# intellerce/controlanimate

Measured on AMD Instinct MI355X. Metric: frames_per_sec, higher is better.
Workload: dtype fp16

## Files before the change

controlanimate_amd/_capi.py:

```python
from __future__ import annotations

import ctypes as C
import os

_HERE = os.path.dirname(os.path.abspath(__file__))
LIB_PATH = os.environ.get("CA_HIP_LIB") or os.path.join(_HERE, "csrc", "libcontrolanimate_hip.so")

CA_BF16, CA_F16 = 0, 1
CA_F32 = 2
CA_ACT_NONE, CA_ACT_SILU = 0, 1
CA_ACT_RELU = 4
CA_ACT_RELU6 = 5
CA_MLSD_TOPK = 200
ABI_VERSION = 16


class CAHipUnavailable(RuntimeError):
    pass


class CAHipError(RuntimeError):
    pass


class GemmArgs(C.Structure):
    _fields_ = [
        ("a", C.c_void_p), ("a2", C.c_void_p), ("w", C.c_void_p), ("c", C.c_void_p),
        ("bias", C.c_void_p), ("rowbias", C.c_void_p), ("residual", C.c_void_p),
        ("lda", C.c_int64), ("lda2", C.c_int64), ("ldc", C.c_int64), ("ld_res", C.c_int64),
        ("ld_rowbias", C.c_int64),
        ("m", C.c_int32), ("n", C.c_int32), ("k1", C.c_int32), ("k2", C.c_int32),
        ("rows_per_group", C.c_int32),
        ("alpha", C.c_float), ("post_scale", C.c_float),
        ("act", C.c_int32), ("geglu", C.c_int32), ("out_f32", C.c_int32), ("dtype", C.c_int32),
        ("ln_stats", C.c_void_p), ("ln_colsum", C.c_void_p), ("ln_eps", C.c_float),
        ("workspace", C.c_void_p), ("workspace_bytes", C.c_int64),
        ("row_sums_out", C.c_void_p), ("ln_parts", C.c_int32),
        ("w_frag", C.c_void_p),
    ]


class FfArgs(C.Structure):
    _fields_ = [
        ("x", C.c_void_p), ("w1_frag", C.c_void_p), ("bias1", C.c_void_p), ("colsum1", C.c_void_p), ("ln_stats", C.c_void_p),
        ("w2_frag", C.c_void_p), ("bias2", C.c_void_p), ("residual", C.c_void_p), ("y", C.c_void_p),
        ("lda", C.c_int64), ("ldc", C.c_int64), ("ld_res", C.c_int64),
        ("m", C.c_int32), ("c", C.c_int32), ("inner", C.c_int32), ("ln_eps", C.c_float), ("dtype", C.c_int32),
        ("w_out_frag", C.c_void_p), ("bias_out", C.c_void_p), ("residual_out", C.c_void_p), ("ld_res_out", C.c_int64),
    ]


class TattnArgs(C.Structure):
    _fields_ = [
        ("x", C.c_void_p), ("w_frag", C.c_void_p), ("gamma", C.c_void_p), ("bias_pe", C.c_void_p), ("o", C.c_void_p),
        ("lda", C.c_int64), ("ldo", C.c_int64), ("ld_bias_pe", C.c_int64),
        ("batch", C.c_int32), ("frames", C.c_int32), ("tokens", C.c_int32), ("heads", C.c_int32), ("c", C.c_int32),
        ("ln_eps", C.c_float), ("scale", C.c_float), ("dtype", C.c_int32),
        ("w_out_frag", C.c_void_p), ("bias_out", C.c_void_p), ("residual", C.c_void_p), ("ld_res", C.c_int64),
    ]


ATTN_WOUT_FRAG_ELEMS = 102400
TATTN_W_FRAG_ELEMS = 368640


class XattnArgs(C.Structure):
    _fields_ = [
        ("x", C.c_void_p), ("wq_frag", C.c_void_p), ("bias", C.c_void_p), ("kv_frag", C.c_void_p), ("o", C.c_void_p),
        ("lda", C.c_int64), ("ldo", C.c_int64),
        ("m", C.c_int32), ("tokens", C.c_int32), ("frames_per_kv", C.c_int32), ("kv_mod", C.c_int32), ("kv_batches", C.c_int32),
        ("nk", C.c_int32), ("heads", C.c_int32), ("c", C.c_int32),
        ("ln_eps", C.c_float), ("dtype", C.c_int32),
        ("w_out_frag", C.c_void_p), ("bias_out", C.c_void_p), ("residual", C.c_void_p), ("ld_res", C.c_int64),
        ("kv_frag_ip", C.c_void_p), ("nk_ip", C.c_int32), ("ip_scale", C.c_float),
    ]


XATTN_W_FRAG_ELEMS = 122880
XATTN_KV_FRAG_ELEMS = 7680


class ConvArgs(C.Structure):
    _fields_ = [
        ("x", C.c_void_p), ("x2", C.c_void_p), ("w", C.c_void_p), ("y", C.c_void_p),
        ("bias", C.c_void_p), ("rowbias", C.c_void_p), ("residual", C.c_void_p),
        ("ld_res", C.c_int64), ("ld_rowbias", C.c_int64),
        ("images", C.c_int32), ("hin", C.c_int32), ("win", C.c_int32),
        ("cin1", C.c_int32), ("cin2", C.c_int32), ("cout", C.c_int32),
        ("stride", C.c_int32), ("upsample", C.c_int32), ("rows_per_group", C.c_int32),
        ("alpha", C.c_float), ("post_scale", C.c_float),
        ("act", C.c_int32), ("out_f32", C.c_int32), ("dtype", C.c_int32),
        ("workspace", C.c_void_p), ("workspace_bytes", C.c_int64), ("pad_asym", C.c_int32),
        ("w_wino", C.c_void_p), ("x_is_wino_v", C.c_int32),
    ]


class GroupNormArgs(C.Structure):
    _fields_ = [
        ("x", C.c_void_p), ("x2", C.c_void_p), ("y", C.c_void_p),
        ("gamma", C.c_void_p), ("beta", C.c_void_p), ("partials", C.c_void_p),
        ("images", C.c_int32), ("hw", C.c_int32), ("c1", C.c_int32), ("c2", C.c_int32),
        ("groups", C.c_int32), ("frames_per_stat", C.c_int32),
        ("eps", C.c_float), ("act", C.c_int32), ("dtype", C.c_int32),
        ("wino_v", C.c_void_p), ("wino_h", C.c_int32), ("wino_w", C.c_int32),
    ]


class LayerNormArgs(C.Structure):
    _fields_ = [
        ("x", C.c_void_p), ("y", C.c_void_p), ("gamma", C.c_void_p), ("beta", C.c_void_p),
        ("pos", C.c_void_p),
        ("rows", C.c_int64),
        ("c", C.c_int32), ("rows_per_frame", C.c_int32), ("frames", C.c_int32),
        ("eps", C.c_float), ("dtype", C.c_int32), ("stats", C.c_void_p),
    ]


class AttnArgs(C.Structure):
    _fields_ = [
        ("q", C.c_void_p), ("k", C.c_void_p), ("v", C.c_void_p), ("o", C.c_void_p),
        ("q_outer", C.c_int64), ("q_inner", C.c_int64), ("q_row", C.c_int64),
        ("o_outer", C.c_int64), ("o_inner", C.c_int64), ("o_row", C.c_int64),
# ... 51 lines not shown
    "ca_gemm_wants_finished_stats": (C.c_int, [C.POINTER(GemmArgs)]),
    "ca_ln_finish_sums": (C.c_int, [C.c_void_p, C.c_int, C.c_int64, C.c_int, C.c_float, C.c_void_p, C.c_void_p]),
    "ca_gemm_workspace_bytes": (C.c_int64, [C.POINTER(GemmArgs)]),
    "ca_gemm_row_sums_parts": (C.c_int, [C.POINTER(GemmArgs)]),
    "ca_gemm_plan_name": (C.c_int, [C.POINTER(GemmArgs), C.c_char_p, C.c_int32]),
    "ca_conv3x3_plan_name": (C.c_int, [C.POINTER(ConvArgs), C.c_char_p, C.c_int32]),
    "ca_conv3x3": (C.c_int, [C.POINTER(ConvArgs), C.c_void_p]),
    "ca_pack_w_wino": (C.c_int, [C.c_void_p, C.c_int32, C.c_int32, C.c_int32, C.c_void_p, C.c_void_p]),
    "ca_conv3x3_workspace_bytes": (C.c_int64, [C.POINTER(ConvArgs)]),
    "ca_softmax_rows": (C.c_int, [C.c_void_p, C.c_void_p, C.c_int64, C.c_int32, C.c_int64, C.c_int64, C.c_float, C.c_int32, C.c_void_p]),
    "ca_groupnorm_partials_floats": (C.c_int64, [C.c_int32, C.c_int32, C.c_int32, C.c_int32]),
    "ca_groupnorm_stats": (C.c_int, [C.POINTER(GroupNormArgs), C.c_void_p]),
    "ca_groupnorm_apply": (C.c_int, [C.POINTER(GroupNormArgs), C.c_void_p]),
    "ca_groupnorm": (C.c_int, [C.POINTER(GroupNormArgs), C.c_void_p]),
    "ca_groupnorm_wino_supported": (C.c_int, [C.POINTER(GroupNormArgs)]),
    "ca_layernorm": (C.c_int, [C.POINTER(LayerNormArgs), C.c_void_p]),
    "ca_attention": (C.c_int, [C.POINTER(AttnArgs), C.c_void_p]),
    "ca_attention_plan_name": (C.c_int, [C.POINTER(AttnArgs), C.c_char_p, C.c_int32]),
    "ca_add_bcast": (C.c_int, [C.c_void_p, C.c_void_p, C.c_void_p, C.c_int64, C.c_int64, C.c_int32, C.c_void_p]),
    "ca_repeat": (C.c_int, [C.c_void_p, C.c_void_p, C.c_int64, C.c_int32, C.c_void_p]),
    "ca_silu_f32": (C.c_int, [C.c_void_p, C.c_void_p, C.c_int64, C.c_void_p]),
    "ca_timestep_embedding": (C.c_int, [C.c_void_p, C.c_float, C.c_void_p, C.c_int32, C.c_int32, C.c_int32, C.c_void_p]),
    "ca_latents_to_nhwc": (C.c_int, [C.c_void_p, C.c_void_p, C.c_int32, C.c_int32, C.c_int32, C.c_int32, C.c_int32,
                                      C.c_int32, C.c_int32, C.c_float, C.c_int32, C.c_void_p]),
    "ca_nhwc_to_ncfhw_f32": (C.c_int, [C.c_void_p, C.c_void_p, C.c_int32, C.c_int32, C.c_int32, C.c_int32, C.c_int32,
                                        C.c_int32, C.c_int32, C.c_int32, C.c_void_p]),
    "ca_ncfhw_to_nhwc": (C.c_int, [C.c_void_p, C.c_int32, C.POINTER(C.c_int64), C.c_void_p, C.c_int32, C.c_int32,
                                    C.c_int32, C.c_int32, C.c_int32, C.c_int32, C.c_int32, C.c_void_p]),
    "ca_cfg_scheduler_step": (C.c_int, [C.c_void_p, C.c_int32, C.c_int32, C.c_float, C.c_void_p, C.c_void_p,
                                         C.c_void_p, C.c_void_p, C.c_int32, C.c_int32, C.c_int32, C.c_int32,
                                         C.POINTER(C.c_float), C.c_float, C.c_void_p]),
    "ca_lincomb": (C.c_int, [C.c_void_p, C.POINTER(C.c_void_p), C.POINTER(C.c_float), C.c_int32, C.c_int64, C.c_void_p]),
    "ca_conv3x3_narrow": (C.c_int, [C.POINTER(ConvNarrowArgs), C.c_void_p]),
    "ca_conv3x3_narrow_plan_name": (C.c_int, [C.POINTER(ConvNarrowArgs), C.c_char_p, C.c_int32]),
    "ca_rgb8_to_nhwc": (C.c_int, [C.c_void_p, C.c_void_p, C.c_int32, C.c_int32, C.c_int32, C.c_int32, C.c_void_p]),
    "ca_resize_lanczos4_u8": (C.c_int, [C.c_void_p, C.c_void_p, C.c_int32, C.c_int32, C.c_int32, C.c_int32, C.c_int32,
                                         C.c_void_p, C.c_void_p, C.c_void_p, C.c_void_p, C.c_void_p]),
    "ca_color_match_workspace_bytes": (C.c_int64, [C.c_int32, C.c_int64]),
    "ca_hist_u8x3": (C.c_int, [C.c_void_p, C.c_void_p, C.c_int32, C.c_int64, C.c_void_p]),
    "ca_color_moments_f64": (C.c_int, [C.c_void_p, C.c_void_p, C.c_void_p, C.c_void_p, C.c_int32, C.c_int64, C.c_void_p, C.c_int64, C.c_void_p]),
    "ca_color_transform_f64": (C.c_int, [C.c_void_p, C.c_void_p, C.c_void_p, C.c_void_p, C.c_void_p, C.c_void_p, C.c_int32, C.c_int64, C.c_void_p]),
    "ca_sort_f64_segments": (C.c_int, [C.c_void_p, C.c_void_p, C.c_int32, C.c_int64, C.c_void_p, C.c_int64, C.c_void_p]),
    "ca_color_rank_map_f64": (C.c_int, [C.c_void_p, C.c_void_p, C.c_void_p, C.c_void_p, C.c_void_p, C.c_void_p, C.c_int32, C.c_int64,
                                         C.c_void_p, C.c_int64, C.c_void_p]),
    "ca_color_finish_u8": (C.c_int, [C.c_void_p, C.c_void_p, C.c_int32, C.c_int64, C.c_int32, C.c_void_p, C.c_int64, C.c_void_p]),
    "ca_canny_workspace_bytes": (C.c_int64, [C.c_int32, C.c_int32, C.c_int32]),
    "ca_canny_tile_w": (C.c_int32, []),
    "ca_canny_tile_h": (C.c_int32, []),
    "ca_canny_classify": (C.c_int, [C.c_void_p, C.c_int32, C.c_int32, C.c_int32, C.c_int32, C.c_int32, C.c_int32, C.c_void_p, C.c_int64, C.c_void_p]),
    "ca_canny_link": (C.c_int, [C.c_int32, C.c_int32, C.c_int32, C.c_void_p, C.c_int64, C.c_void_p]),
    "ca_canny_link_stage": (C.c_int, [C.c_int32, C.c_int32, C.c_int32, C.c_void_p, C.c_int64, C.c_int32, C.c_void_p]),
    "ca_canny_emit": (C.c_int, [C.c_int32, C.c_int32, C.c_int32, C.c_void_p, C.c_int64, C.c_void_p, C.c_void_p, C.c_int32, C.c_int32, C.c_void_p]),
    "ca_conv_up2_phase_supported": (C.c_int, [C.POINTER(ConvArgs)]),
    "ca_conv_up2_phase": (C.c_int, [C.POINTER(ConvArgs), C.c_void_p]),
    "ca_conv_up2_phase_plan_name": (C.c_int, [C.POINTER(ConvArgs), C.c_char_p, C.c_int32]),
    "ca_perceiver_attn": (C.c_int, [C.POINTER(PerceiverAttnArgs), C.c_void_p]),
    "ca_hed_prep": (C.c_int, [C.c_void_p, C.c_void_p, C.c_void_p, C.c_int32, C.c_int32, C.c_int32, C.c_int32, C.c_void_p]),
    "ca_hed_pool_side": (C.c_int, [C.c_void_p, C.c_void_p, C.c_void_p, C.c_void_p, C.c_void_p, C.c_int32, C.c_int32, C.c_int32, C.c_int32, C.c_int32, C.c_void_p]),
    "ca_hed_fuse": (C.c_int, [C.c_void_p, C.c_void_p, C.c_void_p, C.c_void_p, C.c_void_p, C.c_int32, C.c_int32, C.c_int32, C.c_void_p, C.c_void_p, C.c_int32, C.c_int32, C.c_void_p]),
    "ca_lineart_conv_in": (C.c_int, [C.c_void_p, C.c_void_p, C.c_void_p, C.c_int32, C.c_int32, C.c_int32, C.c_int32, C.c_void_p]),
    "ca_instnorm_partials_floats": (C.c_int64, [C.c_int32, C.c_int32, C.c_int32, C.c_int32]),
    "ca_instnorm_stats": (C.c_int, [C.c_void_p, C.c_void_p, C.c_int32, C.c_int32, C.c_int32, C.c_int32, C.c_int32, C.c_int32, C.c_void_p]),
    "ca_instnorm_apply": (C.c_int, [C.c_void_p, C.c_void_p, C.c_void_p, C.c_void_p, C.c_int32, C.c_int32, C.c_int32, C.c_int32, C.c_int32, C.c_int32, C.c_int32,
                                    C.c_int32, C.c_float, C.c_int32, C.c_void_p]),
    "ca_convt3x3s2_gather": (C.c_int, [C.c_void_p, C.c_void_p, C.c_int32, C.c_int32, C.c_int32, C.c_int32, C.c_int32, C.c_void_p]),
    "ca_lineart_conv_out": (C.c_int, [C.c_void_p, C.c_void_p, C.c_void_p, C.c_void_p, C.c_int32, C.c_int32, C.c_int32, C.c_int32, C.c_void_p]),
    "ca_lineart_finish": (C.c_int, [C.c_void_p, C.c_int32, C.c_int32, C.c_int32, C.c_void_p, C.c_void_p, C.c_int32, C.c_int32, C.c_void_p]),
    "ca_mlsd_prep": (C.c_int, [C.c_void_p, C.c_void_p, C.c_int32, C.c_int32, C.c_int32, C.c_int32, C.c_void_p]),
    "ca_dwconv3x3": (C.c_int, [C.c_void_p, C.c_void_p, C.c_void_p, C.c_void_p, C.c_int32, C.c_int32, C.c_int32, C.c_int32, C.c_int32, C.c_int32, C.c_int32, C.c_void_p]),
    "ca_upsample2x_bilinear_ac": (C.c_int, [C.c_void_p, C.c_void_p, C.c_int32, C.c_int32, C.c_int32, C.c_int32, C.c_int64, C.c_int32, C.c_int32, C.c_void_p]),
    "ca_conv3x3_dil": (C.c_int, [C.c_void_p, C.c_void_p, C.c_void_p, C.c_void_p, C.c_int32, C.c_int32, C.c_int32, C.c_int32, C.c_int32, C.c_int32, C.c_int32, C.c_void_p]),
    "ca_mlsd_decode_workspace_bytes": (C.c_int64, [C.c_int32, C.c_int32, C.c_int32]),
    "ca_mlsd_decode": (C.c_int, [C.c_void_p, C.c_int32, C.c_int32, C.c_int32, C.c_float, C.c_float, C.c_void_p, C.c_int64, C.c_void_p, C.c_void_p, C.c_void_p]),
    "ca_mlsd_draw": (C.c_int, [C.c_void_p, C.c_void_p, C.c_int32, C.c_int32, C.c_int32, C.c_void_p, C.c_void_p, C.c_int32, C.c_int32, C.c_void_p]),
    "ca_softedge_prep": (C.c_int, [C.c_void_p, C.c_void_p, C.c_int32, C.c_int32, C.c_int32, C.c_int32, C.c_void_p]),
    "ca_relu": (C.c_int, [C.c_void_p, C.c_void_p, C.c_int64, C.c_int32, C.c_void_p]),
    "ca_dwconv_k": (C.c_int, [C.c_void_p, C.c_void_p, C.c_void_p, C.c_int32, C.c_int32, C.c_int32, C.c_int32, C.c_int32, C.c_int32, C.c_int32, C.c_void_p]),
    "ca_maxpool2x2": (C.c_int, [C.c_void_p, C.c_void_p, C.c_int32, C.c_int32, C.c_int32, C.c_int32, C.c_int32, C.c_void_p]),
    "ca_pdc_block_supported": (C.c_int, [C.c_int32, C.c_int32]),
    "ca_pdc_block": (C.c_int, [C.c_void_p, C.c_void_p, C.c_void_p, C.c_void_p, C.c_int32, C.c_int32, C.c_int32, C.c_int32, C.c_int32, C.c_int32, C.c_void_p]),
    "ca_cdcm_dil4": (C.c_int, [C.c_void_p, C.c_void_p, C.c_void_p, C.c_int32, C.c_int32, C.c_int32, C.c_int32, C.c_int32, C.c_void_p]),
    "ca_csam_reduce": (C.c_int, [C.c_void_p] * 9 + [C.c_int32] * 5 + [C.c_void_p]),
    "ca_softedge_fuse": (C.c_int, [C.c_void_p] * 5 + [C.c_int32] * 4 + [C.c_void_p] * 3 + [C.c_int32, C.c_int32, C.c_void_p]),
}

_lib = None


def lib() -> C.CDLL:
    global _lib
    if _lib is not None:
        return _lib
    import torch
    if not os.path.exists(LIB_PATH):
        raise CAHipUnavailable(
            f"{LIB_PATH} is missing: the HIP extension is not built. Run "
            "`python -m controlanimate_amd._build` (needs hipcc); there is no CPU fallback.")
    try:
        handle = C.CDLL(LIB_PATH)
    except OSError as e:
        raise CAHipUnavailable(f"cannot load {LIB_PATH}: {e}") from e
    for name, (res, args) in SYMBOLS.items():
        fn = getattr(handle, name)
        fn.restype = res
        fn.argtypes = args
    if handle.ca_abi_version() != ABI_VERSION:
        raise CAHipUnavailable(f"ABI mismatch: library {handle.ca_abi_version()} vs binding {ABI_VERSION}; rebuild")
    _lib = handle
    return handle


def check(rc: int, what: str) -> None:
    if rc != 0:
        msg = lib().ca_last_error()
        raise CAHipError(f"{what} failed with code {rc}: {msg.decode() if msg else ''}")
```

controlanimate_amd/attention.py:

```python
from __future__ import annotations

from typing import Optional

import torch
from torch import nn

from . import kernels as K
from .attention_processor import Attention, AttnProcessor2_0
from .context import ExecCtx, dispatch
from .layers import HipConv1x1, HipGroupNorm, HipLayerNorm, HipLinear, LnFold, WeightArena, _f32, geglu_interleave, ln_fold_enabled


class GEGLU(nn.Module):
    def __init__(self, dim_in: int, dim_out: int):
        super().__init__()
        self.dim_in, self.dim_out = dim_in, dim_out
        self.proj = HipLinear(dim_in, dim_out * 2)
        self.w = self.b = None

    def pack(self, arena: WeightArena, dtype):
        self.w = arena.add((2 * self.dim_out, self.dim_in), dtype, lambda: geglu_interleave(_f32(self.proj.weight)))
        self.b = arena.add((2 * self.dim_out,), torch.float32, lambda: geglu_interleave(_f32(self.proj.bias)))

    def run(self, x: torch.Tensor) -> torch.Tensor:
        return K.gemm(x, self.w.t, bias=self.b.t, geglu=True)


class FeedForward(nn.Module):
    def __init__(self, dim: int, dim_out: Optional[int] = None, mult: int = 4, dropout: float = 0.0,
                 activation_fn: str = "geglu", final_dropout: bool = False):
        super().__init__()
        if activation_fn != "geglu":
            raise NotImplementedError(activation_fn)
        inner = int(dim * mult)
        self.net = nn.ModuleList([GEGLU(dim, inner), nn.Identity(), HipLinear(inner, dim_out or dim)])

    def pack(self, arena, dtype, fold_ln=None):
        self.fold = None
        if fold_ln is not None and ln_fold_enabled():
            self.fold = LnFold(arena, dtype, fold_ln, [self.net[0].proj], geglu=True)
        else:
            self.net[0].pack(arena, dtype)
        self.net[2].pack(arena, dtype)
        self.w2f = None
        out = self.net[2]
        if self.fold is not None and self.fold.w.frag is not None and (out.out_features, out.in_features) == (320, 1280):
            from .layers import frag_order2
            self.w2f = arena.add((320, 1280), dtype, lambda: frag_order2(out.weight.detach().float()))

    def run_with_proj_out(self, x: torch.Tensor, residual: Optional[torch.Tensor], proj_frag, proj_bias, proj_residual) -> Optional[torch.Tensor]:
        fold = getattr(self, "fold", None)
        if fold is None or getattr(self, "w2f", None) is None or proj_frag is None or not dispatch.attn_out_fused:
            return None
        return K.ff_fused(x, fold.w.frag[0].t, fold.b.t, fold.cs.t, self.w2f.t, None if self.net[2].b is None else self.net[2].b.t,
                          fold.eps, residual=residual, w_out_frag=proj_frag.t, bias_out=None if proj_bias is None else proj_bias.t,
                          residual_out=proj_residual)

    def run(self, x: torch.Tensor, residual: Optional[torch.Tensor] = None, sums=None) -> torch.Tensor:
        fold = getattr(self, "fold", None)
        if fold is not None and getattr(self, "w2f", None) is not None and sums is None:
            y = K.ff_fused(x, fold.w.frag[0].t, fold.b.t, fold.cs.t, self.w2f.t, None if self.net[2].b is None else self.net[2].b.t,
                           fold.eps, residual=residual)
            if y is not None:
                return y
        if fold is not None:
            h = K.gemm(x, fold.w.t, bias=fold.b.t, geglu=True, ln=(K.RowStats(x, fold.eps, sums), fold.cs.t))
        else:
            h = self.net[0].run(x)
        return self.net[2].run(h, residual=residual)


class BasicTransformerBlock(nn.Module):
    def __init__(self, query_dim: int, num_attention_heads: int, attention_head_dim: int, dropout=0.0,
                 cross_attention_dim: Optional[int] = None, activation_fn: str = "geglu", attention_bias: bool = False,
                 upcast_attention: bool = False, unet_use_cross_frame_attention=False, unet_use_temporal_attention=False, **_):
        super().__init__()
        if unet_use_cross_frame_attention or unet_use_temporal_attention:
            raise NotImplementedError("both flags are false in configs/inference/inference-v{1,2}.yaml")
        self.processor = AttnProcessor2_0()
        self.attn1 = Attention(query_dim, heads=num_attention_heads, dim_head=attention_head_dim, bias=attention_bias)
        self.norm1 = HipLayerNorm(query_dim)
        self.attn2 = Attention(query_dim, cross_attention_dim=cross_attention_dim, heads=num_attention_heads,
                               dim_head=attention_head_dim, bias=attention_bias) if cross_attention_dim is not None else None
        self.norm2 = HipLayerNorm(query_dim) if cross_attention_dim is not None else None
        self.ff = FeedForward(query_dim, activation_fn=activation_fn)
        self.norm3 = HipLayerNorm(query_dim)

    def get_processor(self, return_deprecated_lora: bool = False):
        return self.processor

    def set_processor(self, processor, _remove_lora: bool = False):
        if isinstance(getattr(self, "processor", None), nn.Module) and not isinstance(processor, nn.Module):
            self._modules.pop("processor", None)
        self.processor = processor

    def pack(self, arena, dtype):
        self.attn1.pack(arena, dtype, fold_ln=self.norm1)
        self.norm1.pack(arena, dtype)
        if self.attn2 is not None:
            self.attn2.pack(arena, dtype, fold_ln=self.norm2)
            self.norm2.pack(arena, dtype)
        self.ff.pack(arena, dtype, fold_ln=self.norm3)
        self.norm3.pack(arena, dtype)

    def forward(self, x: torch.Tensor, ctx: ExecCtx, proj_out=None) -> torch.Tensor:
        return self.forward_rest(self.forward_self(x), ctx, proj_out=proj_out)

    def forward_self(self, x: torch.Tensor) -> torch.Tensor:
        B, N, C = x.shape
        next_folded = (self.attn2.fold if self.attn2 is not None else self.ff.fold) is not None
        if self.attn1.fold is not None:
            x = self.attn1(x, residual=x, ln=(K.RowStats(x.view(B * N, C), self.norm1.eps, K.row_sums_of(x)), self.attn1.fold),
                           row_sums=next_folded)
        else:
            x = self.attn1(self.norm1.run(x.view(B * N, C)).view(B, N, C), residual=x, row_sums=next_folded)
        return x

    def forward_rest(self, x: torch.Tensor, ctx: ExecCtx, proj_out=None) -> torch.Tensor:
        B, N, C = x.shape
        if self.attn2 is not None:
            kw = dict(encoder_hidden_states=ctx.ehs, residual=x, frames_per_kv=ctx.frames_per_kv, kv_mod=ctx.kv_mod, cache=ctx.cache,
                      row_sums=self.ff.fold is not None)
            if self.attn2.fold is not None:
                x = self.attn2(x, ln=(K.RowStats(x.view(B * N, C), self.norm2.eps, K.row_sums_of(x)), self.attn2.fold), **kw)
            else:
                x = self.attn2(self.norm2.run(x.view(B * N, C)).view(B, N, C), **kw)
        x2 = x.view(B * N, C)
        if self.ff.fold is None:
            return self.ff.run(self.norm3.run(x2), residual=x2).view(B, N, C)
        if proj_out is not None and K.row_sums_of(x) is None:
            y = self.ff.run_with_proj_out(x2, x2, *proj_out)
            if y is not None:
                y = y.view(B, N, C)
                y._proj_out_done = True
                return y
        return self.ff.run(x2, residual=x2, sums=K.row_sums_of(x)).view(B, N, C)


class Transformer3DModel(nn.Module):
    def __init__(self, num_attention_heads: int = 16, attention_head_dim: int = 88, in_channels: Optional[int] = None,
                 num_layers: int = 1, norm_num_groups: int = 32, cross_attention_dim: Optional[int] = None,
                 use_linear_projection: bool = False, **kw):
        super().__init__()
        if use_linear_projection:
            raise NotImplementedError("SD1.5 uses 1x1-conv projections")
        inner = num_attention_heads * attention_head_dim
        self.in_channels = in_channels
        self.norm = HipGroupNorm(norm_num_groups, in_channels, eps=1e-6)
        self.proj_in = HipConv1x1(in_channels, inner)
        self.transformer_blocks = nn.ModuleList([
            BasicTransformerBlock(inner, num_attention_heads, attention_head_dim, cross_attention_dim=cross_attention_dim, **kw)
            for _ in range(num_layers)])
        self.proj_out = HipConv1x1(inner, in_channels)

    def pack(self, arena, dtype):
        self.norm.pack(arena, dtype)
        self.proj_in.pack(arena, dtype)
        for b in self.transformer_blocks:
            b.pack(arena, dtype)
        self.proj_out.pack(arena, dtype)
        self.proj_out_frag = None
        po = self.proj_out
        if tuple(po.weight.shape[:2]) == (320, 320) and getattr(self.transformer_blocks[-1].ff, "w2f", None) is not None:
            from .layers import frag_order_wout
            self.proj_out_frag = arena.add((102400,), dtype, lambda: frag_order_wout(_f32(po.weight).reshape(320, 320)))

    def forward(self, x: torch.Tensor, ctx: ExecCtx, shared_half: bool = False) -> torch.Tensor:
        images, h, w, c = x.shape
        rows = images * h * w
        y = self.norm.run(x)
        y0 = self.proj_in.run(y.view(rows, c), row_sums=self.transformer_blocks[0].attn1.fold is not None)
        y = K.carry_row_sums(y0.view(images, h * w, -1), y0)
        nblk = len(self.transformer_blocks)
        pfrag = getattr(self, "proj_out_frag", None)

        def proj(k, x_rows):
            return (pfrag, self.proj_out.b, x_rows) if (k == nblk - 1 and pfrag is not None) else None
        if shared_half:
            y = self.transformer_blocks[0].forward_self(y)
            y, x = K.repeat_batch(y), K.repeat_batch(x)
            images, rows = 2 * images, 2 * rows
            y = self.transformer_blocks[0].forward_rest(y, ctx, proj_out=proj(0, x.view(rows, c)))
        for k in range(1 if shared_half else 0, nblk):
            y = self.transformer_blocks[k](y, ctx, proj_out=proj(k, x.view(rows, c)))
        if getattr(y, "_proj_out_done", False):
            return y.view(images, h, w, c)
        return self.proj_out.run(y.view(rows, -1), residual=x.view(rows, c)).view(images, h, w, c)
```

controlanimate_amd/context.py:

```python
from __future__ import annotations

from dataclasses import dataclass, field
from typing import Optional

import torch


@dataclass
class ExecCtx:
    b: int
    f: int
    dtype: torch.dtype
    temb: torch.Tensor
    emb_groups: int
    ehs: Optional[torch.Tensor] = None
    frames_per_kv: int = 1
    kv_mod: int = 0
    gn_frames_per_stat: int = 1
    cache: dict = field(default_factory=dict)

    @property
    def images(self) -> int:
        return self.b * self.f

    def rows_per_emb_group(self, h: int, w: int) -> int:
        return self.images // self.emb_groups * h * w


class Dispatch:
    gemm_ar = True
    ff_fused = True
    tattn_fused = True
    xattn_fused = True
    attn_out_fused = True
    xattn_ip_fused = True
    conv_winograd = True
    gn_winograd = True
    conv_up2_phase = True
    ln_row_sums = True
    repeat_kernel = True
    ln_fold = True
    cfg_shared = True
    cn_cfg_dedup = True
    pdc_block_fused = True
    controlnet_streams = 2


dispatch = Dispatch()
```

controlanimate_amd/csrc/ca_gemm.hip:

```cpp

#include "ca_gemm_plan.h"

namespace {
using namespace ca_gemm_detail;
#include "ca_conv_wino.h"

template <int DT, int BM, int BN, int WAVES_M, int WAVES_N, int MODE>
__global__ __launch_bounds__(256) void k_gemm(GemmKParams p) {
  constexpr int TM = BM / WAVES_M / 16;
  constexpr int TN = BN / WAVES_N / 16;
  constexpr int AI = BM / 32;
  constexpr int BI = BN / 32;
  static_assert(2 * (BM + BN) * BK >= BM * (BN + 8), "epilogue staging must fit");
  __shared__ __attribute__((aligned(16))) u16 smem[2 * (BM + BN) * BK];

  const int tid = threadIdx.x;
  const int lane = tid & 63;
  const int wid = tid >> 6;
  const int wm = wid / WAVES_N, wn = wid % WAVES_N;
  const int g = lane >> 4, l15 = lane & 15;

  const int tiles_n = (p.n + BN - 1) / BN;
  const unsigned bid = xcd_remap(blockIdx.x, gridDim.x);
  int tile_m, tile_n;
// ... 329 lines not shown
  if (p.bias) {
#pragma unroll
    for (int k = 0; k < 8; ++k) v[k] += p.bias[n + k];
  }
  if (p.rowbias) {
    const float* rbp = p.rowbias + (m / p.rows_per_group) * p.ld_rowbias + n;
#pragma unroll
    for (int k = 0; k < 8; ++k) v[k] += rbp[k];
  }
#pragma unroll
  for (int k = 0; k < 8; ++k) v[k] *= p.alpha;
  unpack8<DT>(pack8<DT>(v), v);
  if (p.res) {
    float r[8];
    unpack8<DT>(ld16(p.res + m * p.ld_res + n), r);
#pragma unroll
    for (int k = 0; k < 8; ++k) v[k] += r[k];
  }
#pragma unroll
  for (int k = 0; k < 8; ++k) v[k] *= p.post;
  if (p.act != CA_ACT_NONE) {
#pragma unroll
    for (int k = 0; k < 8; ++k) v[k] = act_f(v[k], p.act);
  }
  const int64_t off = m * p.ldc + n;
  if (p.out_f32) {
    float* cp = reinterpret_cast<float*>(p.c) + off;
    *reinterpret_cast<f32x4*>(cp) = (f32x4){v[0], v[1], v[2], v[3]};
    *reinterpret_cast<f32x4*>(cp + 4) = (f32x4){v[4], v[5], v[6], v[7]};
  } else {
    st16(reinterpret_cast<u16*>(p.c) + off, pack8<DT>(v));
  }
}

template <int DT, int MODE>
int launch_gemm(const GemmKParams& p, const GemmPlan& g, hipStream_t st) {
  const dim3 grid(ceil_div_i(p.m, g.bm) * ceil_div_i(p.n, g.bn));
  switch (g.kind) {
    case PK_WRES: return ca_launch_gemm_pp(p, DT, MODE, PK_WRES, 0u, st);
    case PK_AR: return ca_launch_gemm_ar(p, DT, st);
    case PK_PP2:
    case PK_PS:
    case PK_PQ: return ca_launch_gemm_pp(p, DT, MODE, g.kind, g.tiles, st);
    case PK_PP2_SPLITK: {
      GemmKParams q = p;
      q.splits = g.splits;
      const int rc = ca_launch_gemm_pp(q, DT, MODE, PK_PP2, g.tiles * (unsigned)g.splits, st);
      hipLaunchKernelGGL((k_splitk_reduce<DT>), dim3(ceil_div_i((int64_t)q.m * (q.n / 8), 256)), dim3(256), 0, st, q);
      return rc;
    }
    case PK_DMA_SPLITK:
      hipLaunchKernelGGL((k_gemm_dma<DT, 128, 128, 2, 2, MODE, 1>), dim3(g.tiles * (unsigned)p.splits), dim3(256), 0, st, p);
      hipLaunchKernelGGL((k_splitk_reduce<DT>), dim3(ceil_div_i((int64_t)p.m * (p.n / 8), 256)), dim3(256), 0, st, p);
      return CA_OK;
    case PK_DMA:
      if (g.bn == 160 && g.nbuf == 1) hipLaunchKernelGGL((k_gemm_dma<DT, 128, 160, 2, 2, MODE, 1>), grid, dim3(256), 0, st, p);
      else if (g.bn == 128 && g.nbuf == 1) hipLaunchKernelGGL((k_gemm_dma<DT, 128, 128, 2, 2, MODE, 1>), grid, dim3(256), 0, st, p);
      else if (g.bn == 64 && g.nbuf == 1) hipLaunchKernelGGL((k_gemm_dma<DT, 128, 64, 4, 1, MODE, 1>), grid, dim3(256), 0, st, p);
      else if (g.bn == 64 && g.nbuf == 3) hipLaunchKernelGGL((k_gemm_dma<DT, 128, 64, 4, 1, MODE, 3>), grid, dim3(256), 0, st, p);
      else break;
      return CA_OK;
    case PK_REG:
      if (g.bn == 128) hipLaunchKernelGGL((k_gemm<DT, 128, 128, 2, 2, MODE>), grid, dim3(256), 0, st, p);
      else if (g.bn == 64) hipLaunchKernelGGL((k_gemm<DT, 128, 64, 4, 1, MODE>), grid, dim3(256), 0, st, p);
      else break;
      return CA_OK;
  }
  CA_FAIL(CA_ERR_LAUNCH, "ca_gemm: no kernel for plan kind %d, tile %dx%d, %d stages", (int)g.kind, g.bm, g.bn, g.nbuf);
}

}

extern "C" int ca_gemm(const ca_gemm_args* a, void* stream) {
  DenseLaunch d;
  int rc = gemm_prepare(a, d);
  if (rc) return rc;
  hipStream_t st = (hipStream_t)stream;
  rc = a->dtype == CA_BF16 ? launch_gemm<CA_BF16, 0>(d.p, d.plan, st) : launch_gemm<CA_F16, 0>(d.p, d.plan, st);
  if (rc) return rc;
  CA_CHECK_LAUNCH("ca_gemm");
  return CA_OK;
}

extern "C" int64_t ca_gemm_workspace_bytes(const ca_gemm_args* a) {
  DenseLaunch d;
  return gemm_resolve(a, d) == CA_OK ? d.workspace : 0;
}

extern "C" int ca_gemm_row_sums_parts(const ca_gemm_args* a) {
  DenseLaunch d;
  DenseAsk ask{};
  ask.without_row_sums = true;
  return gemm_resolve(a, d, ask) == CA_OK ? row_sums_parts_of(d.p) : 0;
}

extern "C" int ca_gemm_ln_inline_supported(const ca_gemm_args* a) {
  DenseLaunch d;
  return a && a->ln_colsum && gemm_resolve(a, d) == CA_OK && wres_eligible(d.p) ? 1 : 0;
}

extern "C" int ca_gemm_wants_finished_stats(const ca_gemm_args* a) {
  if (!a || !a->ln_colsum || !a->ln_stats || a->ln_parts <= 0 || a->row_sums_out) return 0;
  DenseLaunch d;
  DenseAsk ask{};
  ask.stats_finished = true;
  return gemm_resolve(a, d, ask) == CA_OK && d.plan.kind == PK_PQ ? 1 : 0;
}

extern "C" int64_t ca_conv3x3_workspace_bytes(const ca_conv_args* a) { return conv_workspace_bytes(a); }

static int launch_conv_wino(const ca_conv_args* a, const GemmKParams& cp, hipStream_t st) {
  const int kc = a->cin1 + a->cin2;
  const ConvGeom g = conv_geom(a);
  const int64_t tiles = wino_tiles(a, g);
  WinoParams w{};
  w.x = (const u16*)a->x;
  w.x2 = (const u16*)a->x2;
  w.v = (u16*)a->workspace;
  u16* mm = (u16*)a->workspace + (a->x_is_wino_v ? 0 : 16 * tiles * kc);
  w.mm = mm;
  w.y = (u16*)a->y;
  w.bias = a->bias;
  w.rowbias = a->rowbias;
  w.res = (const u16*)a->residual;
  w.ld_res = a->ld_res;
  w.ld_rowbias = a->ld_rowbias;
  w.images = a->images, w.h = g.hl, w.w = g.wl, w.c1 = a->cin1, w.c2 = a->cin2, w.cout = a->cout;
  w.ups = a->upsample;
  w.rows_per_group = cp.rows_per_group;
  w.alpha = a->alpha, w.post = a->post_scale, w.act = a->act;
  const int64_t in_threads = tiles * (kc / 8), out_threads = tiles * (a->cout / 8);
  if (a->x_is_wino_v) w.v = (u16*)a->x;
  else if (a->dtype == CA_BF16) hipLaunchKernelGGL((k_wino_in<CA_BF16>), dim3((unsigned)((in_threads + 255) / 256)), dim3(256), 0, st, w);
  else hipLaunchKernelGGL((k_wino_in<CA_F16>), dim3((unsigned)((in_threads + 255) / 256)), dim3(256), 0, st, w);
  GemmKParams q{};
  q.a = w.v;
  q.w = (const u16*)a->w_wino;
  q.c = mm;
  q.lda = kc;
  q.ldc = a->cout;
  q.a_bytes = desc_bytes(16 * tiles * kc);
  q.w_bytes = desc_bytes((int64_t)16 * a->cout * kc);
  q.m = (int)(16 * tiles);
  q.n = a->cout;
  q.c1 = kc;
  q.taps = 1;
  q.kc_tiles = kc / BK;
  q.rows_per_group = 1;
  q.alpha = 1.f, q.post = 1.f;
  q.splits = 1;
  q.w_group_rows = (int)tiles;
  q.w_group_stride = (unsigned)((int64_t)a->cout * kc * 2);
  const unsigned gemm_tiles = (unsigned)((q.m / 256) * (q.n / 320));
  int rc = ca_launch_gemm_pp(q, a->dtype, 0, PK_PQ, gemm_tiles, st);
  if (rc) return rc;
  if (a->dtype == CA_BF16) hipLaunchKernelGGL((k_wino_out<CA_BF16>), dim3((unsigned)((out_threads + 255) / 256)), dim3(256), 0, st, w);
  else hipLaunchKernelGGL((k_wino_out<CA_F16>), dim3((unsigned)((out_threads + 255) / 256)), dim3(256), 0, st, w);
  return CA_OK;
}

extern "C" int ca_pack_w_wino(const void* w, int32_t cout, int32_t cin, int32_t dtype, void* dst, void* stream) {
  CA_REQUIRE(w && dst, "ca_pack_w_wino: null operand");
  CA_REQUIRE(cout > 0 && cin > 0 && (dtype == CA_BF16 || dtype == CA_F16), "ca_pack_w_wino: cout=%d cin=%d dtype=%d", cout, cin, dtype);
  const int64_t n = (int64_t)cout * cin;
  if (dtype == CA_BF16) hipLaunchKernelGGL((k_pack_w_wino<CA_BF16>), dim3((unsigned)((n + 255) / 256)), dim3(256), 0, (hipStream_t)stream, (const u16*)w, (u16*)dst, cout, cin);
  else hipLaunchKernelGGL((k_pack_w_wino<CA_F16>), dim3((unsigned)((n + 255) / 256)), dim3(256), 0, (hipStream_t)stream, (const u16*)w, (u16*)dst, cout, cin);
  CA_CHECK_LAUNCH("ca_pack_w_wino");
  return CA_OK;
}

extern "C" int ca_conv3x3(const ca_conv_args* a, void* stream) {
  GemmKParams p{};
  int rc = conv_prepare(a, p);
  if (rc) return rc;
  hipStream_t st = (hipStream_t)stream;
  if (wino_taken(a)) {
    rc = launch_conv_wino(a, p, st);
    if (rc) return rc;
    CA_CHECK_LAUNCH("ca_conv3x3(winograd)");
    return CA_OK;
  }
// ... 54 lines not shown
```

controlanimate_amd/csrc/ca_gemm_core.h:

```cpp
#pragma once
#include "ca_common.h"
#include <stdlib.h>

namespace ca_gemm_detail {


struct GemmKParams {
  const u16* a;
  const u16* a2;
  const u16* w;
  void* c;
  const float* bias;
  const float* rowbias;
  const float* ln_stats;
  const float* ln_colsum;
  const u16* res;
  int64_t lda, lda2, ldc, ld_res, ld_rowbias;
  unsigned a_bytes, a2_bytes, w_bytes;
  int m, n;
  int c1, c2;
  int taps;
  int kc_tiles;
  int hin, win, hout, wout, stride, ups, pad_lo;
  int rows_per_group;
  float alpha, post;
  int act, geglu, out_f32;
  int splits;
  float* partial;
  int dbg;
  int tap_inner;
  float* row_sums;
  int ln_parts;
  int ln_inline;
  float ln_eps;
  const u16* wf;
  int w_group_rows;
  unsigned w_group_stride;
  int up2_rows, up2_tiles;
  unsigned up2_mag_w, up2_mag_h;
};

constexpr int BK = 64;

constexpr int GROUP_M = 8;
__device__ __forceinline__ void tile_coords(unsigned bid, int tiles_m, int tiles_n, int& tile_m, int& tile_n) {
  const unsigned gsz = GROUP_M * tiles_n;
  const unsigned group = bid / gsz, in = bid - group * gsz;
  const int first_m = group * GROUP_M;
  const int gm = tiles_m - first_m < GROUP_M ? tiles_m - first_m : GROUP_M;
  tile_m = first_m + in % gm;
  tile_n = in / gm;
}

__device__ __forceinline__ void k_tile_split(const GemmKParams& p, int t, int kct, int& tap, int& cc) {
  if (p.taps == 1) {
    tap = 0;
    cc = t;
  } else if (p.tap_inner) {
    cc = t / p.taps;
    tap = t - cc * p.taps;
  } else {
    tap = t / kct;
    cc = t - tap * kct;
  }
}

__device__ __forceinline__ int lds_off(int row, int chunk) {
  return row * BK + ((chunk ^ ((row >> 1) & 7)) << 3);
}

template <int DT, int TM, int TN>
__device__ __forceinline__ void gemm_epilogue_direct(const GemmKParams& p, f32x4 (&acc)[TM][TN], int m0, int n0, int wm, int wn,
                                                     int l15, int g) {
#pragma unroll
  for (int i = 0; i < TM; ++i) {
    const int m = m0 + wm * TM * 16 + i * 16 + l15;
    if (m >= p.m) continue;
    const float* rbp = p.rowbias ? p.rowbias + (int64_t)(m / p.rows_per_group) * p.ld_rowbias : nullptr;
#pragma unroll
    for (int j = 0; j < TN; ++j) {
      const int n = n0 + wn * TN * 16 + j * 16 + g * 4;
      if (n >= p.n) continue;
      float v[4];
#pragma unroll
      for (int r = 0; r < 4; ++r) v[r] = acc[i][j][r];
      if (p.bias) {
        f32x4 b = *reinterpret_cast<const f32x4*>(p.bias + n);
#pragma unroll
        for (int r = 0; r < 4; ++r) v[r] += b[r];
      }
      if (rbp) {
        f32x4 b = *reinterpret_cast<const f32x4*>(rbp + n);
#pragma unroll
        for (int r = 0; r < 4; ++r) v[r] += b[r];
      }
#pragma unroll
      for (int r = 0; r < 4; ++r) v[r] *= p.alpha;
      if (p.res) {
        u32x2 rr = *reinterpret_cast<const u32x2*>(p.res + (int64_t)m * p.ld_res + n);
        v[0] += Elem<DT>::to_f((u16)(rr[0] & 0xffffu));
        v[1] += Elem<DT>::to_f((u16)(rr[0] >> 16));
        v[2] += Elem<DT>::to_f((u16)(rr[1] & 0xffffu));
        v[3] += Elem<DT>::to_f((u16)(rr[1] >> 16));
      }
#pragma unroll
      for (int r = 0; r < 4; ++r) v[r] *= p.post;
      if (p.act != CA_ACT_NONE) {
#pragma unroll
        for (int r = 0; r < 4; ++r) v[r] = act_f(v[r], p.act);
      }
      if (p.geglu) {
        const f32x2 gg = gelu_erf_f2((f32x2){v[1], v[3]});
        float o0 = v[0] * gg[0];
        float o1 = v[2] * gg[1];
        const int64_t off = (int64_t)m * p.ldc + (n >> 1);
        if (p.out_f32) {
          float* cp = reinterpret_cast<float*>(p.c) + off;
          cp[0] = o0;
          cp[1] = o1;
        } else {
          *reinterpret_cast<unsigned*>(reinterpret_cast<u16*>(p.c) + off) = pack2<DT>(o0, o1);
        }
// ... 256 lines not shown
```

controlanimate_amd/csrc/ca_gemm_plan.h:

```cpp
#pragma once
#include "ca_gemm_core.h"

namespace ca_gemm_detail {

inline unsigned desc_bytes(int64_t elems) {
  const int64_t b = elems * 2;
  return (b > 0 && b < (int64_t)0xFFFFFF00ll) ? (unsigned)b : 0u;
}

inline bool dma_shape_ok(const GemmKParams& p) { return (p.c1 + p.c2) % BK == 0 && (p.c2 == 0 || p.c1 % BK == 0); }
inline bool dma_sizes_ok(const GemmKParams& p) { return p.a_bytes != 0 && p.w_bytes != 0 && (p.c2 == 0 || p.a2_bytes != 0); }
inline bool dma_capable(const GemmKParams& p) { return dma_shape_ok(p) && dma_sizes_ok(p); }

inline bool wres_eligible(const GemmKParams& p) {
  static const int wres_env = CA_KNOB("CA_GEMM_WRES", -1);
  const int kc = p.c1 + p.c2;
  return wres_env != 0 && kc == 320 && p.taps == 1 && (p.c2 == 0 || p.c1 % 32 == 0) && p.n % 160 == 0 && p.n / 160 <= 32 && !p.out_f32 &&
         p.splits <= 1 && !p.ln_parts && dma_sizes_ok(p) &&
         (!p.rowbias || p.rows_per_group % 32 == 0) &&
         act_out_fit31(p) &&
         (wres_env == 1 || p.m >= 16384);
}

inline bool ar_eligible(const GemmKParams& p, bool scratch) {
// ... 62 lines not shown
      if (s_eff > p.splits) s_eff = p.splits;
      if (s_eff >= 2 && tiles320 * s_eff >= 128 && nt / s_eff >= 12) {
        return GemmPlan{PK_PP2_SPLITK, 128, 320, 0, s_eff, (unsigned)tiles320};
      }
    }
    return GemmPlan{PK_DMA_SPLITK, 128, 128, 1, p.splits, (unsigned)(ceil_div_i(p.m, 128) * (p.n / 128))};
  }
  static const int pp_env = CA_KNOB("CA_GEMM_PP", -1);
  static const int pq_env = CA_KNOB("CA_GEMM_PQ", -1);
  if (pq_env != 0 && pq_capable(p, mode)) {
    const int64_t tiles = (int64_t)ceil_div_i(p.m, 256) * (p.n / 320);
    const bool dflt = mode == 1 ? (tiles >= 256 && (p.n >= 640 || nt >= 64)) : (tiles >= 256 && (tiles % 256 == 0 || tiles >= 1024) && nt >= 8 && !wres_eligible(p));
    const bool epi1 = p.geglu || p.ln_colsum || p.ln_stats;
    const bool dflt2 = dflt && (mode == 1 || p.geglu), dflt3 = dflt && mode == 1, dflt4 = dflt && (mode == 1 || p.geglu || !epi1);
    if ((pq_env < 0 && dflt) || pq_env == 1 || (pq_env == 2 && dflt2) || (pq_env == 3 && dflt3) || (pq_env == 4 && dflt4) || (pq_env == 5 && dflt)) {
      return GemmPlan{PK_PQ, 256, 320, 0, 1, (unsigned)tiles};
    }
  }
  static const int ps_env = CA_KNOB("CA_GEMM_PS", -1);
  if (ps_env != 0 && ps_capable(p)) {
    const int64_t tiles = (int64_t)ceil_div_i(p.m, 128) * (p.n / 320);
    const bool dflt = mode == 0 && !wres_eligible(p) && nt <= 20 && tiles >= 256 && (p.geglu || p.n <= 1280);
    if ((ps_env < 0 && dflt) || ps_env == 1 || (ps_env == 2 && !(mode == 0 && wres_eligible(p)))) {
      return GemmPlan{PK_PS, 128, 320, 0, 1, (unsigned)tiles};
    }
  }
  if (mode == 0 && dma && ar_eligible(p, p.partial != nullptr)) return GemmPlan{PK_AR, 128, 64, 0, 1, 0u};
  if (mode == 0 && dma && wres_eligible(p)) return GemmPlan{PK_WRES, 256, 160, 0, 1, 0u};
  if (dma && pp_env != 0 && nt >= 2 && p.n % 320 == 0 && p.splits <= 1) {
    const int64_t tiles = (int64_t)ceil_div_i(p.m, 128) * (p.n / 320);
    if (p.row_sums || pp_env == 2 || (pp_env < 0 && tiles >= 128 && nt >= 10 && (tiles <= 256 || (tiles <= 512 && mode == 0)))) {
      return GemmPlan{PK_PP2, 128, 320, 0, 1, (unsigned)tiles};
    }
  }
  const bool wide = p.n % 128 == 0 && (int64_t)ceil_div_i(p.m, 128) * ceil_div_i(p.n, 128) >= 512;
  const int64_t blocks = (int64_t)ceil_div_i(p.m, 128) * ceil_div_i(p.n, wide ? 128 : 64);
  const int nbuf = blocks >= 512 ? 1 : 3;
  if (dma && !wide && p.n % 160 == 0 && (int64_t)ceil_div_i(p.m, 128) * (p.n / 160) >= 512) return GemmPlan{PK_DMA, 128, 160, 1, 1, 0u};
  return GemmPlan{dma ? PK_DMA : PK_REG, 128, wide ? 128 : 64, dma ? nbuf : 2, 1, 0u};
}

inline int row_sums_parts_of(GemmKParams p) {
  p.row_sums = nullptr;
  if (p.geglu || p.out_f32) return 0;
  const PlanKind k = plan_gemm(p, 0).kind;
  if (k == PK_PP2 || k == PK_PS) return p.n / 320;
  if (k == PK_PQ && !p.ln_colsum && !p.ln_stats) return 4 * (p.n / 320);
  return 0;
}
inline bool row_sums_capable(const GemmKParams& p) { return row_sums_parts_of(p) > 0; }

inline void plan_label(const GemmPlan& g, char* buf, int len) {
  switch (g.kind) {
    case PK_WRES: snprintf(buf, len, "wres160"); break;
    case PK_AR: snprintf(buf, len, "ar128x64"); break;
    case PK_PP2: snprintf(buf, len, "pp128x320"); break;
    case PK_PS: snprintf(buf, len, "ps128x320"); break;
    case PK_PQ: snprintf(buf, len, "pq256x320"); break;
    case PK_PP2_SPLITK: snprintf(buf, len, "pp128x320_splitk%d", g.splits); break;
    case PK_DMA: snprintf(buf, len, "%dx%d%s", g.bm, g.bn, g.nbuf == 3 ? "_r3" : ""); break;
    case PK_DMA_SPLITK: snprintf(buf, len, "128x128_splitk%d", g.splits); break;
    case PK_REG: snprintf(buf, len, "reg_%dx%d", g.bm, g.bn); break;
  }
}

inline int check_epilogue(const char* who, int n, int geglu, int64_t ldc, int64_t ld_res, const void* res) {
  CA_REQUIRE(n == 4 || (n >= 8 && n % 8 == 0), "%s: N=%d must be 4 or a multiple of 8", who, n);
  CA_REQUIRE(!geglu || n % 8 == 0, "%s: geglu needs N %% 8 == 0", who);
  if (n >= 8) {
    CA_REQUIRE(ldc % (geglu ? 4 : 8) == 0, "%s: ldc=%lld must be a multiple of %d", who, (long long)ldc, geglu ? 4 : 8);
    CA_REQUIRE(!res || ld_res % 8 == 0, "%s: ld_res=%lld must be a multiple of 8", who, (long long)ld_res);
  } else {
    CA_REQUIRE(ldc % 4 == 0, "%s: ldc=%lld misaligned", who, (long long)ldc);
    CA_REQUIRE(!res || ld_res % 4 == 0, "%s: ld_res=%lld misaligned", who, (long long)ld_res);
  }
  return CA_OK;
}

struct DenseAsk {
  bool without_row_sums;
  bool stats_finished;
};

inline int gemm_fill(const ca_gemm_args* a, GemmKParams& p, const DenseAsk& ask) {
  CA_REQUIRE(a != nullptr, "ca_gemm: null args");
  CA_REQUIRE(a->a && a->w && a->c, "ca_gemm: null operand");
  CA_REQUIRE(a->m > 0 && a->k1 > 0 && a->k2 >= 0, "ca_gemm: bad sizes m=%d k1=%d k2=%d", a->m, a->k1, a->k2);
  CA_REQUIRE(a->k1 % 8 == 0 && a->k2 % 8 == 0, "ca_gemm: k1=%d k2=%d must be multiples of 8", a->k1, a->k2);
  CA_REQUIRE(a->lda % 8 == 0 && (a->k2 == 0 || (a->a2 && a->lda2 % 8 == 0)), "ca_gemm: lda/lda2 misaligned or a2 missing");
  CA_REQUIRE(a->dtype == CA_BF16 || a->dtype == CA_F16, "ca_gemm: dtype %d", a->dtype);
  CA_REQUIRE(!a->rowbias || a->rows_per_group > 0, "ca_gemm: rows_per_group");
  CA_REQUIRE(!a->rowbias || a->ld_rowbias % 4 == 0, "ca_gemm: ld_rowbias misaligned");
  int rc = check_epilogue("ca_gemm", a->n, a->geglu, a->ldc, a->ld_res, a->residual);
  if (rc) return rc;
  p.a = (const u16*)a->a, p.a2 = (const u16*)a->a2, p.w = (const u16*)a->w, p.c = a->c;
  p.bias = a->bias, p.rowbias = a->rowbias, p.ln_stats = a->ln_stats, p.ln_colsum = a->ln_colsum;
  p.row_sums = ask.without_row_sums ? nullptr : a->row_sums_out;
  p.ln_parts = ask.stats_finished ? 0 : a->ln_parts;
  CA_REQUIRE(p.ln_parts >= 0 && p.ln_parts <= 16, "ca_gemm: ln_parts=%d", p.ln_parts);
  CA_REQUIRE(p.ln_parts == 0 || (a->ln_stats && a->ln_colsum && a->ln_eps > 0.f), "ca_gemm: ln_parts needs ln_stats (the partial sums), ln_colsum and ln_eps > 0");
  p.ln_inline = (a->ln_colsum && !a->ln_stats) ? 1 : 0;
  p.ln_eps = a->ln_eps;
  p.wf = (const u16*)a->w_frag;
  CA_REQUIRE(!a->ln_stats || a->ln_colsum, "ca_gemm: ln_stats without ln_colsum");
  CA_REQUIRE(!p.ln_inline || a->ln_eps > 0.f, "ca_gemm: ln_colsum without ln_stats asks for in-kernel statistics and needs ln_eps > 0");
  CA_REQUIRE(!a->ln_colsum || (a->n >= 8 && a->k2 == 0), "ca_gemm: the folded LayerNorm needs N >= 8 and a single A source");
  p.res = (const u16*)a->residual;
  p.lda = a->lda, p.lda2 = a->lda2, p.ldc = a->ldc, p.ld_res = a->ld_res, p.ld_rowbias = a->ld_rowbias;
  p.a_bytes = desc_bytes((int64_t)(a->m - 1) * a->lda + a->k1);
  p.a2_bytes = a->k2 ? desc_bytes((int64_t)(a->m - 1) * a->lda2 + a->k2) : 0u;
  p.w_bytes = desc_bytes((int64_t)a->n * (a->k1 + a->k2));
  p.m = a->m, p.n = a->n, p.c1 = a->k1, p.c2 = a->k2;
  p.taps = 1;
  p.kc_tiles = ceil_div_i(a->k1 + a->k2, BK);
  p.rows_per_group = a->rows_per_group > 0 ? a->rows_per_group : 1;
  p.alpha = a->alpha, p.post = a->post_scale, p.act = a->act, p.geglu = a->geglu, p.out_f32 = a->out_f32;
  p.splits = 1;
  return CA_OK;
}

struct DenseLaunch {
  GemmKParams p;
  GemmPlan plan;
  int64_t workspace;
};
inline int gemm_resolve(const ca_gemm_args* a, DenseLaunch& d, const DenseAsk& ask = DenseAsk{}) {
  d = DenseLaunch{};
  GemmKParams& p = d.p;
  int rc = gemm_fill(a, p, ask);
  if (rc) return rc;
  const SplitK k = splitk_decide(p, 0);
  splitk_apply(k, a->workspace, a->workspace_bytes, p);
  d.workspace = k.bytes;
  if (p.ln_inline && p.wf) {
    if (ar_eligible(p, true)) d.workspace = (int64_t)p.m * 8;
    if (a->workspace && a->workspace_bytes >= (int64_t)p.m * 8) p.partial = reinterpret_cast<float*>(a->workspace);
  }
  d.plan = plan_gemm(p, 0);
  return CA_OK;
}

inline int gemm_prepare(const ca_gemm_args* a, DenseLaunch& d) {
  int rc = gemm_resolve(a, d);
  if (rc) return rc;
  CA_REQUIRE(!d.p.row_sums || row_sums_capable(d.p), "ca_gemm: row_sums_out is not available for this launch: ask ca_gemm_row_sums_parts() first");
  CA_REQUIRE(!d.p.ln_inline || wres_eligible(d.p), "ca_gemm: in-kernel LayerNorm statistics (ln_stats NULL) are not available for this launch: "
             "ask ca_gemm_ln_inline_supported() first and pass ln_stats otherwise");
  return CA_OK;
}

struct ConvGeom { int hl, wl, hout, wout; int64_t m; };
inline ConvGeom conv_geom(const ca_conv_args* a) {
  ConvGeom g;
  g.hl = a->hin << a->upsample, g.wl = a->win << a->upsample;
  const int pad = a->pad_asym ? 1 : 2;
  g.hout = (g.hl + pad - 3) / a->stride + 1;
  g.wout = (g.wl + pad - 3) / a->stride + 1;
  g.m = (int64_t)a->images * g.hout * g.wout;
  return g;
}
inline int64_t wino_tiles(const ca_conv_args* a, const ConvGeom& g) { return (int64_t)a->images * (g.hl / 2) * (g.wl / 2); }

inline int64_t wino_workspace_bytes(const ca_conv_args* a) {
  if (!a || !a->w_wino || (a->dtype != CA_F16 && a->dtype != CA_BF16) || a->stride != 1 || a->pad_asym || a->out_f32) return 0;
  if (a->upsample != 0 && a->upsample != 1) return 0;
  if (a->x_is_wino_v && (a->cin2 != 0 || a->upsample)) return 0;
  const ConvGeom g = conv_geom(a);
  if (a->images <= 0 || g.hl < 2 || g.wl < 2 || (g.hl & 1) || (g.wl & 1)) return 0;
  const int kc = a->cin1 + a->cin2;
  static const int min_cin = CA_KNOB("CA_WINO_MIN_CIN", 1280);
  if (kc < 640 || kc % BK != 0 || a->cin1 % 8 != 0 || a->cin2 % 8 != 0 || a->cout % 320 != 0) return 0;
  const int64_t tiles = wino_tiles(a, g);
  if (kc < min_cin && !(min_cin == 1280 && tiles <= 4096)) return 0;
  static const int max_tiles = CA_KNOB("CA_WINO_MAX_TILES", 16384);
  if (tiles % 256 != 0 || tiles > max_tiles) return 0;
  if (16 * tiles * (int64_t)(kc > a->cout ? kc : a->cout) * 2 >= 0x7FFFFF00ll) return 0;
  return 16 * tiles * (int64_t)((a->x_is_wino_v ? 0 : kc) + a->cout) * 2;
}

inline bool wino_taken(const ca_conv_args* a) {
  const int64_t wb = wino_workspace_bytes(a);
  return wb > 0 && a->workspace && a->workspace_bytes >= wb && (((uintptr_t)a->workspace | (uintptr_t)a->w_wino) & 15) == 0;
}

inline void conv_fill_sizes(const ca_conv_args* a, const ConvGeom& g, GemmKParams& p) {
  p.a_bytes = desc_bytes((int64_t)a->images * a->hin * a->win * a->cin1);
  p.a2_bytes = a->cin2 ? desc_bytes((int64_t)a->images * a->hin * a->win * a->cin2) : 0u;
  p.w_bytes = desc_bytes((int64_t)a->cout * 9 * (a->cin1 + a->cin2));
  p.m = (int)g.m, p.n = a->cout, p.c1 = a->cin1, p.c2 = a->cin2;
  p.taps = 9;
  static const int tap_inner_env = CA_KNOB("CA_CONV_TAP_INNER", 1);
  p.tap_inner = tap_inner_env;
  p.kc_tiles = ceil_div_i(a->cin1 + a->cin2, BK);
  p.hin = a->hin, p.win = a->win, p.hout = g.hout, p.wout = g.wout;
  p.stride = a->stride, p.ups = a->upsample, p.pad_lo = a->pad_asym ? 0 : 1;
  p.geglu = 0, p.out_f32 = a->out_f32;
  p.splits = 1;
}

inline int conv_prepare(const ca_conv_args* a, GemmKParams& p) {
  CA_REQUIRE(a != nullptr, "ca_conv3x3: null args");
  CA_REQUIRE(a->x && a->w && a->y, "ca_conv3x3: null operand");
  CA_REQUIRE(a->images > 0 && a->hin > 0 && a->win > 0, "ca_conv3x3: bad geometry");
  CA_REQUIRE(a->cin1 > 0 && a->cin1 % 8 == 0 && a->cin2 >= 0 && a->cin2 % 8 == 0,
             "ca_conv3x3: cin1=%d cin2=%d must be multiples of 8", a->cin1, a->cin2);
  CA_REQUIRE(a->cin2 == 0 || a->x2, "ca_conv3x3: x2 missing");
  CA_REQUIRE(a->stride == 1 || a->stride == 2, "ca_conv3x3: stride %d", a->stride);
  CA_REQUIRE(a->upsample == 0 || a->upsample == 1, "ca_conv3x3: upsample %d", a->upsample);
  CA_REQUIRE(a->dtype == CA_BF16 || a->dtype == CA_F16, "ca_conv3x3: dtype %d", a->dtype);
  CA_REQUIRE(!a->rowbias || a->rows_per_group > 0, "ca_conv3x3: rows_per_group");
  int rc = check_epilogue("ca_conv3x3", a->cout, 0, a->cout, a->ld_res, a->residual);
  if (rc) return rc;
  CA_REQUIRE(a->pad_asym == 0 || a->pad_asym == 1, "ca_conv3x3: pad_asym %d", a->pad_asym);
  const ConvGeom g = conv_geom(a);
  CA_REQUIRE(g.m < (1ll << 31), "ca_conv3x3: too many output pixels");
  conv_fill_sizes(a, g, p);
  p.a = (const u16*)a->x, p.a2 = (const u16*)a->x2, p.w = (const u16*)a->w, p.c = a->y;
  p.bias = a->bias, p.rowbias = a->rowbias, p.res = (const u16*)a->residual;
  p.ldc = a->cout, p.ld_res = a->ld_res, p.ld_rowbias = a->ld_rowbias;
  p.rows_per_group = a->rows_per_group > 0 ? a->rows_per_group : 1;
  p.alpha = a->alpha, p.post = a->post_scale, p.act = a->act;
  splitk_apply(splitk_decide(p, 1), a->workspace, a->workspace_bytes, p);
  return CA_OK;
}

inline int64_t conv_workspace_bytes(const ca_conv_args* a) {
  if (!a || a->images <= 0 || a->hin <= 0 || a->win <= 0 || (a->stride != 1 && a->stride != 2)) return 0;
  const int64_t wb = wino_workspace_bytes(a);
  if (wb > 0) return wb;
  const ConvGeom g = conv_geom(a);
// ... 51 lines not shown
```

controlanimate_amd/csrc/ca_gemm_pp.hip:

```cpp
#include "ca_gemm_core.h"
#include <type_traits>

namespace {
using namespace ca_gemm_detail;
#include "ca_gemm_pp2.h"
#include "ca_gemm_wres.h"
#include "ca_gemm_ps.h"
#include "ca_gemm_pq.h"

int cu_count() {
  static int n = 0;
  if (!n) {
    int dev = 0;
    hipDeviceProp_t prop;
    if (hipGetDevice(&dev) == hipSuccess && hipGetDeviceProperties(&prop, dev) == hipSuccess) n = prop.multiProcessorCount;
    if (n <= 0) n = 256;
  }
  return n;
}

template <class Launch>
int launch_stamped(const GemmKParams& p, hipStream_t st, const char* label, unsigned sep, unsigned eol, Launch launch) {
  static unsigned long long* dbuf = nullptr;
  if (!dbuf && hipMalloc(&dbuf, 4096 * 8) != hipSuccess) return CA_ERR_LAUNCH;
  (void)hipMemsetAsync(dbuf, 0, 4096 * 8, st);
  GemmKParams q = p;
  q.partial = reinterpret_cast<float*>(dbuf);
  launch(q);
  (void)hipStreamSynchronize(st);
  static int printed = 0;
  if (printed++ < 1) {
    static unsigned long long host[4096];
    (void)hipMemcpy(host, dbuf, sizeof(host), hipMemcpyDeviceToHost);
    for (int g = 0; g < 2; ++g) {
      fprintf(stderr, "[%s stamps group %d, %dx%dx%d] tag:delta_cycles ...\n", label, g, p.m, p.n, (p.c1 + p.c2) * p.taps);
      unsigned long long prev = host[g * 2048];
      for (int i = 0; i < 1000 && host[g * 2048 + 2 * i]; ++i) {
        fprintf(stderr, "%llu:%llu ", host[g * 2048 + 2 * i + 1], host[g * 2048 + 2 * i] - prev);
        prev = host[g * 2048 + 2 * i];
        if (host[g * 2048 + 2 * i + 1] == sep) fprintf(stderr, "| ");
        if (host[g * 2048 + 2 * i + 1] == eol) fprintf(stderr, "\n");
      }
      fprintf(stderr, "\n");
    }
  }
  return CA_OK;
}

template <int DT, int MODE>
int launch_pp(const GemmKParams& p, PlanKind kind, unsigned tiles, hipStream_t st) {
  const unsigned c_bytes = (unsigned)c_extent_bytes(p), res_bytes = (unsigned)res_extent_bytes(p);
  const unsigned grid = tiles < (unsigned)cu_count() ? tiles : (unsigned)cu_count();
  switch (kind) {
    case PK_PQ: {
      auto launch = [&](const GemmKParams& q) {
        if (MODE == 0 && (q.geglu || q.ln_colsum || q.ln_stats)) hipLaunchKernelGGL((k_gemm_pq<DT, 0, 1>), dim3(grid), dim3(512), 0, st, q, (int)tiles, c_bytes, 0u);
        else if (MODE == 0 && q.row_sums) hipLaunchKernelGGL((k_gemm_pq<DT, 0, 2>), dim3(grid), dim3(512), 0, st, q, (int)tiles, c_bytes, res_bytes);
        else hipLaunchKernelGGL((k_gemm_pq<DT, MODE>), dim3(grid), dim3(512), 0, st, q, (int)tiles, c_bytes, res_bytes);
      };
#ifdef CA_STAMPS
      if (p.dbg == 9) return launch_stamped(p, st, "pq", 8, 10, launch);
#endif
      launch(p);
      return CA_OK;
    }
    case PK_PS: {
      auto launch = [&](const GemmKParams& q) { hipLaunchKernelGGL((k_gemm_ps<DT, MODE>), dim3(grid), dim3(512), 0, st, q, (int)tiles, c_bytes, res_bytes); };
#ifdef CA_STAMPS
      if (p.dbg == 9) return launch_stamped(p, st, "ps", 8, 10, launch);
#endif
      launch(p);
      return CA_OK;
    }
    case PK_WRES: {
      if (MODE != 0) return CA_ERR_LAUNCH;
      const int panels = p.n / 160;
      const int chunks = (p.m + 255) / 256;
      int per = (cu_count() / 8) / panels;
      if (per * 8 > chunks) per = chunks / 8;
      if (per < 1) per = 1;
      const unsigned rb_bytes = p.rowbias ? (unsigned)(((int64_t)((p.m - 1) / p.rows_per_group) * p.ld_rowbias + p.n) * 4) : 16u;
      hipLaunchKernelGGL((k_gemm_wres<DT>), dim3(8 * per * panels), dim3(512), 0, st, p, panels, 8 * per, chunks, rb_bytes, c_bytes, res_bytes);
      return CA_OK;
    }
    case PK_PP2:
      hipLaunchKernelGGL((k_gemm_pp2<DT, MODE>), dim3(tiles), dim3(512), 0, st, p);
      return CA_OK;
    default: return CA_ERR_LAUNCH;
  }
}

template <int DT>
int launch_up2(const GemmKParams& p, PlanKind kind, unsigned tiles, hipStream_t st) {
  if (kind != PK_PQ) return CA_ERR_LAUNCH;
  const unsigned grid = tiles < (unsigned)cu_count() ? tiles : (unsigned)cu_count();
  hipLaunchKernelGGL((k_gemm_pq<DT, 2>), dim3(grid), dim3(512), 0, st, p, (int)tiles, (unsigned)c_extent_bytes(p), (unsigned)res_extent_bytes(p));
  return CA_OK;
}
}

int ca_launch_gemm_pp(const ca_gemm_detail::GemmKParams& p0, int dtype, int mode, ca_gemm_detail::PlanKind kind, unsigned tiles, hipStream_t st) {
  static const int dbg = CA_KNOB("CA_PP_DBG", 0);
  ca_gemm_detail::GemmKParams p = p0;
  p.dbg = dbg;
  if (mode == 2) return dtype == CA_BF16 ? launch_up2<CA_BF16>(p, kind, tiles, st) : launch_up2<CA_F16>(p, kind, tiles, st);
  if (dtype == CA_BF16) return mode ? launch_pp<CA_BF16, 1>(p, kind, tiles, st) : launch_pp<CA_BF16, 0>(p, kind, tiles, st);
  return mode ? launch_pp<CA_F16, 1>(p, kind, tiles, st) : launch_pp<CA_F16, 0>(p, kind, tiles, st);
}
```

controlanimate_amd/csrc/ca_gemm_wres.h:

```cpp
#include "ca_gemm_seq.h"

__device__ __forceinline__ int ca_wres_col(int j, int i, bool geglu) {
  if (geglu) return 16 * j + i;
  return 32 * (j >> 1) + 8 * (i >> 2) + 4 * (j & 1) + (i & 3);
}

template <int DT>
__global__ __launch_bounds__(512, 1) void k_gemm_wres(GemmKParams p, int panels, int lanes, int chunks, unsigned rb_bytes, unsigned c_bytes, unsigned res_bytes) {
  constexpr int K = 320, PN = 160, TN = 10, KQ = 10;
  constexpr int WLD_B = 656;
  constexpr int W_BYTES = PN * WLD_B;
  constexpr int SLOT = 2048, RING = 3 * SLOT;
  constexpr int OFF_PAR = W_BYTES + 8 * RING;
  constexpr int OFF_RB = OFF_PAR + 1280;
  constexpr int OFF_FLAG = OFF_RB + 8 * 1024;
  __shared__ __attribute__((aligned(16))) unsigned char smem[OFF_FLAG + 8 * 16];
  static_assert(OFF_FLAG + 8 * 16 <= 160 * 1024, "LDS");

  const int tid = threadIdx.x;
  const int lane = tid & 63;
  const int wid = __builtin_amdgcn_readfirstlane(tid >> 6);
  const int g = lane >> 4, l15 = lane & 15;

  const int slot_b = blockIdx.x >> 3;
  const int panel = slot_b % panels;
  const int my_lane = (blockIdx.x & 7) + 8 * (slot_b / panels);
  if (my_lane >= lanes) return;
  const int n0 = panel * PN;

  const bool geglu = p.geglu != 0;
  for (int q = tid; q < PN * (K / 8); q += 512) {
    const int row = q / (K / 8), c = q - row * (K / 8);
    *reinterpret_cast<u32x4*>(smem + row * WLD_B + c * 16) = ld16(p.w + (int64_t)(n0 + ca_wres_col(row >> 4, row & 15, geglu)) * K + c * 8);
  }
  if (tid < 2 * PN) {
    const float* src = tid < PN ? p.bias : p.ln_colsum;
    const int n = tid < PN ? tid : tid - PN;
    reinterpret_cast<float*>(smem + OFF_PAR)[tid] = src ? src[n0 + n] : 0.f;
  }
  __syncthreads();

  const __amdgpu_buffer_rsrc_t rs_rb = __builtin_amdgcn_make_buffer_rsrc((void*)(p.rowbias ? (const void*)p.rowbias : (const void*)p.w), 0, rb_bytes, 0x00020000);
  unsigned char* rb_patch = smem + OFF_RB + wid * 1024;
  const __amdgpu_buffer_rsrc_t rs_c = __builtin_amdgcn_make_buffer_rsrc(p.c, 0, c_bytes, 0x00020000);
  const __amdgpu_buffer_rsrc_t rs_res = __builtin_amdgcn_make_buffer_rsrc((void*)(p.res ? (const void*)p.res : (const void*)p.c), 0, p.res ? res_bytes : 0u, 0x00020000);
  const __amdgpu_buffer_rsrc_t rs_a = __builtin_amdgcn_make_buffer_rsrc((void*)p.a, 0, p.a_bytes, 0x00020000);
  const __amdgpu_buffer_rsrc_t rs_a2 = __builtin_amdgcn_make_buffer_rsrc((void*)(p.a2 ? p.a2 : p.a), 0, p.a2 ? p.a2_bytes : p.a_bytes, 0x00020000);
  unsigned char* ring = smem + W_BYTES + wid * RING;
  const __amdgpu_buffer_rsrc_t rs_seq = __builtin_amdgcn_make_buffer_rsrc((void*)ca_seq_table.v, 0, 4096u, 0x00020000);
  unsigned char* const my_flags = smem + OFF_FLAG + wid * 16;
  const unsigned flag_addr0 = (unsigned)(size_t)(__attribute__((address_space(3))) unsigned char*)my_flags;
  if (lane < 4) {
    asm volatile("ds_write_b32 %0, %1\n\ts_waitcnt lgkmcnt(0)" ::"v"(flag_addr0 + (unsigned)lane * 4u), "v"(0xFFFFFFFFu) : "memory");
  }

  int d_c = my_lane, d_k = 0, d_s = 0;
  int d_n = 0;
  unsigned d_v1[2], d_v2[2];
  auto head_slab = [&]() {
    int lane_o = lane;
    asm volatile("" : "+v"(lane_o));
#pragma unroll
    for (int h = 0; h < 2; ++h) {
      const int m = d_c * 256 + wid * 32 + h * 16 + (lane_o >> 2);
      const bool ok = m < p.m;
      d_v1[h] = ok ? (unsigned)m * (unsigned)p.lda * 2u + (unsigned)(lane_o & 3) * 16u : DMA_OOB;
      d_v2[h] = ok ? (unsigned)m * (unsigned)p.lda2 * 2u + (unsigned)(lane_o & 3) * 16u : DMA_OOB;
    }
  };
  auto issue = [&]() {
    const int k0 = d_k * 32;
    unsigned char* dst = ring + d_s * SLOT;
    if (k0 >= p.c1) {
      const unsigned so = (unsigned)(k0 - p.c1) * 2u;
      __builtin_amdgcn_raw_ptr_buffer_load_lds(rs_a2, (__attribute__((address_space(3))) void*)dst, 16, d_v2[0], so, 0, 0);
      __builtin_amdgcn_raw_ptr_buffer_load_lds(rs_a2, (__attribute__((address_space(3))) void*)(dst + 1024), 16, d_v2[1], so, 0, 0);
    } else {
      const unsigned so = (unsigned)k0 * 2u;
      __builtin_amdgcn_raw_ptr_buffer_load_lds(rs_a, (__attribute__((address_space(3))) void*)dst, 16, d_v1[0], so, 0, 0);
      __builtin_amdgcn_raw_ptr_buffer_load_lds(rs_a, (__attribute__((address_space(3))) void*)(dst + 1024), 16, d_v1[1], so, 0, 0);
    }
    {
      int lane_f = lane;
      asm volatile("" : "+v"(lane_f));
      if (lane_f == 0)
        __builtin_amdgcn_raw_ptr_buffer_load_lds(rs_seq, (__attribute__((address_space(3))) void*)(my_flags + d_s * 4), 4, 0u, (unsigned)(d_n & 1023) * 4u, 0, 0);
    }
    ++d_n;
    d_s = d_s == 2 ? 0 : d_s + 1;
    if (++d_k == KQ) {
      d_k = 0;
      d_c += lanes;
      head_slab();
    }
  };

  auto chunk_wait = [&](int n, unsigned have) __attribute__((always_inline)) {
    const unsigned want = (unsigned)(n & 1023);
    if ((unsigned)__builtin_amdgcn_readfirstlane(have) == want) return;
    const unsigned addr = flag_addr0 + (unsigned)(n % 3) * 4u;
    for (unsigned spins = 0; spins < (1u << 22); ++spins) {
      unsigned v;
      asm volatile("ds_read_b32 %0, %1\n\ts_waitcnt lgkmcnt(0)" : "=v"(v) : "v"(addr) : "memory");
      if ((unsigned)__builtin_amdgcn_readfirstlane(v) == want) return;
      __builtin_amdgcn_s_sleep(1);
    }
    asm volatile("s_waitcnt vmcnt(0)" ::: "memory");
  };
  int r_n = 0;

  head_slab();
  issue();
  issue();
  chunk_wait(0, 0xFFFFFFFEu);

  const int fa_lane = l15 * 64 + g * 16;
  const unsigned char* wb = smem + l15 * WLD_B + g * 16;
  int r_s = 0;

  for (int c = my_lane; c < chunks; c += lanes) {
    const int m0 = c * 256 + wid * 32;
    f32x4 acc[2][TN];
#pragma unroll
    for (int i = 0; i < 2; ++i)
#pragma unroll
      for (int j = 0; j < TN; ++j) acc[i][j] = (f32x4){0.f, 0.f, 0.f, 0.f};

    float2 st[2] = {make_float2(0.f, 0.f), make_float2(0.f, 0.f)};
    float ln_s[2] = {0.f, 0.f}, ln_ss[2] = {0.f, 0.f};
    if (p.ln_stats) {
#pragma unroll
      for (int i = 0; i < 2; ++i) {
        const int m = m0 + i * 16 + l15;
        if (m < p.m) st[i] = *reinterpret_cast<const float2*>(p.ln_stats + (int64_t)m * 2);
      }
    }
    if (p.rowbias) {
      int lane_o = lane;
      asm volatile("" : "+v"(lane_o));
      const unsigned off = (lane_o < PN / 4 && m0 < p.m) ? ((unsigned)(m0 / p.rows_per_group) * (unsigned)p.ld_rowbias + (unsigned)n0) * 4u + (unsigned)lane_o * 16u : DMA_OOB;
      __builtin_amdgcn_raw_ptr_buffer_load_lds(rs_rb, (__attribute__((address_space(3))) void*)rb_patch, 16, off, 0, 0, 0);
    }
#pragma unroll
    for (int kq = 0; kq < KQ; ++kq) {
      issue();
      const unsigned char* as = ring + r_s * SLOT + fa_lane;
      __builtin_amdgcn_sched_barrier(0);
      const u32x4 fa0 = *reinterpret_cast<const u32x4*>(as);
      const u32x4 fa1 = *reinterpret_cast<const u32x4*>(as + 1024);
      u32x4 fb[TN];
#pragma unroll
      for (int j = 0; j < TN; ++j) {
        __builtin_amdgcn_sched_barrier(0);
        fb[j] = *reinterpret_cast<const u32x4*>(wb + j * 16 * WLD_B + kq * 64);
      }
      __builtin_amdgcn_sched_barrier(0);
#define CA_WRES_PAIR(J, CNT)                                        \
  asm volatile("s_waitcnt lgkmcnt(" #CNT ")" ::: "memory");         \
  __builtin_amdgcn_sched_barrier(0);                                \
  acc[0][J] = Elem<DT>::mfma(fb[J], fa0, acc[0][J]);                \
  acc[1][J] = Elem<DT>::mfma(fb[J], fa1, acc[1][J]);                \
  __builtin_amdgcn_sched_barrier(0);
      CA_WRES_PAIR(0, 9)
      if (p.ln_inline) {
#pragma unroll
        for (int q = 0; q < 4; ++q) {
          const float a0 = Elem<DT>::to_f((u16)(fa0[q] & 0xffffu)), a1 = Elem<DT>::to_f((u16)(fa0[q] >> 16));
          const float b0 = Elem<DT>::to_f((u16)(fa1[q] & 0xffffu)), b1 = Elem<DT>::to_f((u16)(fa1[q] >> 16));
          ln_s[0] += a0 + a1;
          ln_ss[0] = fmaf(a0, a0, fmaf(a1, a1, ln_ss[0]));
          ln_s[1] += b0 + b1;
          ln_ss[1] = fmaf(b0, b0, fmaf(b1, b1, ln_ss[1]));
        }
      }
      CA_WRES_PAIR(1, 8) CA_WRES_PAIR(2, 7) CA_WRES_PAIR(3, 6) CA_WRES_PAIR(4, 5)
      unsigned flag_next;
      asm volatile("ds_read_b32 %0, %1" : "=v"(flag_next) : "v"(flag_addr0 + (unsigned)((r_n + 1) % 3) * 4u) : "memory");
      __builtin_amdgcn_sched_barrier(0);
      CA_WRES_PAIR(5, 5) CA_WRES_PAIR(6, 4) CA_WRES_PAIR(7, 3) CA_WRES_PAIR(8, 2) CA_WRES_PAIR(9, 1)
#undef CA_WRES_PAIR
      asm volatile("s_waitcnt lgkmcnt(0)" : "+v"(flag_next)::"memory");
      r_s = r_s == 2 ? 0 : r_s + 1;
      ++r_n;
      chunk_wait(r_n, flag_next);
    }

    if (p.ln_inline) {
#pragma unroll
      for (int i = 0; i < 2; ++i) {
        float a = ln_s[i], b = ln_ss[i];
        a += __shfl_xor(a, 16);
        b += __shfl_xor(b, 16);
        a += __shfl_xor(a, 32);
        b += __shfl_xor(b, 32);
        const float mean = a * (1.f / K);
        st[i] = make_float2(mean, rsqrtf(fmaxf(b * (1.f / K) - mean * mean, 0.f) + p.ln_eps));
      }
    }
    if (p.dbg == 1) {
      if (acc[0][0][0] == 12345.678f) *reinterpret_cast<float*>(p.c) = acc[1][TN - 1][1];
      continue;
    }
    int lane_e = lane;
    asm volatile("" : "+v"(lane_e));
    const int g = lane_e >> 4, l15 = lane_e & 15;
    u32x4 rr[2][TN / 2];
    if (p.res) {
#pragma unroll
      for (int i = 0; i < 2; ++i)
#pragma unroll
        for (int q = 0; q < TN / 2; ++q) {
          const int m = m0 + i * 16 + l15;
          const unsigned off = m < p.m ? ((unsigned)m * (unsigned)p.ld_res + (unsigned)(n0 + g * 8)) * 2u : 0x80000000u;
          rr[i][q] = __builtin_bit_cast(u32x4, __builtin_amdgcn_raw_buffer_load_b128(rs_res, off, q * 64, 0));
        }
    }
    if (p.alpha == 1.f && p.post == 1.f && p.act == CA_ACT_NONE && !p.geglu) {
      unsigned off[2];
#pragma unroll
      for (int i = 0; i < 2; ++i) {
        const int m = m0 + i * 16 + l15;
        off[i] = m < p.m ? ((unsigned)m * (unsigned)p.ldc + (unsigned)(n0 + g * 8)) * 2u : 0x80000000u;
      }
#pragma unroll
      for (int q = 0; q < TN / 2; ++q) {
        f32x4 bb[2], cs[2];
#pragma unroll
        for (int u = 0; u < 2; ++u) {
          const int col = 32 * q + 8 * g + 4 * u;
          bb[u] = *reinterpret_cast<const f32x4*>(smem + OFF_PAR + col * 4);
          cs[u] = (f32x4){0.f, 0.f, 0.f, 0.f};
          if (p.ln_colsum) cs[u] = *reinterpret_cast<const f32x4*>(smem + OFF_PAR + (PN + col) * 4);
          if (p.rowbias) {
            const f32x4 rb = *reinterpret_cast<const f32x4*>(rb_patch + col * 4);
#pragma unroll
            for (int r = 0; r < 4; ++r) bb[u][r] += rb[r];
          }
        }
#pragma unroll
        for (int i = 0; i < 2; ++i) {
          u32x4 w;
#pragma unroll
          for (int u = 0; u < 2; ++u) {
            f32x4 v = acc[i][2 * q + u];
            if (p.ln_colsum) {
#pragma unroll
              for (int r = 0; r < 4; ++r) v[r] = st[i].y * (v[r] - st[i].x * cs[u][r]);
            }
            w[2 * u] = pack2<DT>(v[0] + bb[u][0], v[1] + bb[u][1]);
            w[2 * u + 1] = pack2<DT>(v[2] + bb[u][2], v[3] + bb[u][3]);
          }
          if (p.res) {
#pragma unroll
            for (int k = 0; k < 4; ++k) {
              if (DT == CA_F16) {
                unsigned s_;
                asm("v_pk_add_f16 %0, %1, %2" : "=v"(s_) : "v"(w[k]), "v"(rr[i][q][k]));
                w[k] = s_;
              } else {
                w[k] = pack2<DT>(Elem<DT>::to_f((u16)(w[k] & 0xffffu)) + Elem<DT>::to_f((u16)(rr[i][q][k] & 0xffffu)),
                                 Elem<DT>::to_f((u16)(w[k] >> 16)) + Elem<DT>::to_f((u16)(rr[i][q][k] >> 16)));
              }
            }
          }
          __builtin_amdgcn_raw_buffer_store_b128(w, rs_c, off[i] + (unsigned)(q * 64), 0, 0);
        }
      }
      continue;
    }
    if (p.geglu && !p.rowbias && !p.res && p.alpha == 1.f && p.post == 1.f && p.act == CA_ACT_NONE) {
      unsigned off[2];
#pragma unroll
      for (int i = 0; i < 2; ++i) {
        const int m = m0 + i * 16 + l15;
        off[i] = m < p.m ? ((unsigned)m * (unsigned)p.ldc + (unsigned)((n0 >> 1) + g * 2)) * 2u : DMA_OOB;
      }
#pragma unroll
      for (int j = 0; j < TN; ++j) {
        const f32x4 bi = *reinterpret_cast<const f32x4*>(smem + OFF_PAR + (j * 16 + g * 4) * 4);
        f32x4 cs = {0.f, 0.f, 0.f, 0.f};
        if (p.ln_colsum) cs = *reinterpret_cast<const f32x4*>(smem + OFF_PAR + (PN + j * 16 + g * 4) * 4);
#pragma unroll
        for (int i = 0; i < 2; ++i) {
          f32x4 v = acc[i][j];
          if (p.ln_colsum) {
#pragma unroll
            for (int r = 0; r < 4; ++r) v[r] = st[i].y * (v[r] - st[i].x * cs[r]);
          }
          float h[4];
#pragma unroll
          for (int r = 0; r < 4; ++r) h[r] = Elem<DT>::to_f(Elem<DT>::from_f(v[r] + bi[r]));
          const f32x2 gg = gelu_erf_f2((f32x2){h[1], h[3]});
          __builtin_amdgcn_raw_buffer_store_b32(pack2<DT>(h[0] * gg[0], h[2] * gg[1]), rs_c, off[i], j * 16, 0);
        }
      }
      continue;
    }
#pragma unroll
    for (int j = 0; j < TN; ++j) {
      const int nl = ca_wres_col(j, 4 * g, geglu);
      const f32x4 bi = *reinterpret_cast<const f32x4*>(smem + OFF_PAR + nl * 4);
      f32x4 cs = {0.f, 0.f, 0.f, 0.f}, rb = {0.f, 0.f, 0.f, 0.f};
      if (p.ln_colsum) cs = *reinterpret_cast<const f32x4*>(smem + OFF_PAR + (PN + nl) * 4);
      if (p.rowbias) rb = *reinterpret_cast<const f32x4*>(rb_patch + nl * 4);
#pragma unroll
      for (int i = 0; i < 2; ++i) {
        const int m = m0 + i * 16 + l15;
        float v[4];
#pragma unroll
        for (int r = 0; r < 4; ++r) v[r] = acc[i][j][r];
        if (p.ln_colsum) {
#pragma unroll
          for (int r = 0; r < 4; ++r) v[r] = st[i].y * (v[r] - st[i].x * cs[r]);
        }
#pragma unroll
        for (int r = 0; r < 4; ++r) v[r] = Elem<DT>::to_f(Elem<DT>::from_f((v[r] + bi[r] + rb[r]) * p.alpha));
        if (p.res) {
          const unsigned r0 = rr[i][j >> 1][2 * (j & 1)], r1 = rr[i][j >> 1][2 * (j & 1) + 1];
          v[0] += Elem<DT>::to_f((u16)(r0 & 0xffffu));
          v[1] += Elem<DT>::to_f((u16)(r0 >> 16));
          v[2] += Elem<DT>::to_f((u16)(r1 & 0xffffu));
          v[3] += Elem<DT>::to_f((u16)(r1 >> 16));
        }
#pragma unroll
        for (int r = 0; r < 4; ++r) v[r] *= p.post;
        if (p.act != CA_ACT_NONE) {
#pragma unroll
          for (int r = 0; r < 4; ++r) v[r] = act_f(v[r], p.act);
        }
        if (p.geglu) {
          const f32x2 gg = gelu_erf_f2((f32x2){v[1], v[3]});
          const unsigned w = pack2<DT>(v[0] * gg[0], v[2] * gg[1]);
          const unsigned off = m < p.m ? ((unsigned)m * (unsigned)p.ldc + (unsigned)((n0 >> 1) + (nl >> 1))) * 2u : 0x80000000u;
          __builtin_amdgcn_raw_buffer_store_b32(w, rs_c, off, 0, 0);
        } else {
          u32x2 w;
          w[0] = pack2<DT>(v[0], v[1]);
          w[1] = pack2<DT>(v[2], v[3]);
          const unsigned off = m < p.m ? ((unsigned)m * (unsigned)p.ldc + (unsigned)(n0 + nl)) * 2u : 0x80000000u;
          __builtin_amdgcn_raw_buffer_store_b64(w, rs_c, off, 0, 0);
        }
      }
    }
    asm volatile("s_waitcnt lgkmcnt(0)" ::: "memory");
  }
  asm volatile("s_waitcnt vmcnt(0)" ::: "memory");
}
```

controlanimate_amd/csrc/ca_norm.hip:

```cpp
#include "ca_common.h"
#include <stdlib.h>

namespace {

constexpr int GN_MAX_SLOTS = 5;
constexpr int GN_MAX_C = 64 * 8 * GN_MAX_SLOTS;

inline int gn_chunks_rows(int64_t rows_per_stat, int rows_per_chunk) {
  int64_t n = (rows_per_stat + rows_per_chunk - 1) / rows_per_chunk;
  if (n < 16) n = (rows_per_stat + 3) / 4 < 16 ? (rows_per_stat + 3) / 4 : 16;
  if (n < 1) n = 1;
  if (n > 256) n = 256;
  return (int)n;
}
inline int gn_chunks_host(int64_t rows_per_stat) { return gn_chunks_rows(rows_per_stat, 256); }

struct GnParams {
  const u16* x;
  const u16* x2;
  u16* y;
  const float* gamma;
  const float* beta;
  float* partials;
  int c1, c2, groups;
// ... 180 lines not shown
  {
    const int S = p.groups <= 32 ? 8 : 4;
    const int g = threadIdx.x % (256 / S), slot = threadIdx.x / (256 / S);
    if (g < p.groups) {
      double a = 0.0, b = 0.0;
      const float* part = p.partials + ((int64_t)sg * p.nchunks * p.groups + g) * 2;
      for (int k = slot; k < p.nchunks; k += S) {
        const float2 v = *reinterpret_cast<const float2*>(part + (int64_t)k * p.groups * 2);
        a += (double)v.x;
        b += (double)v.y;
      }
      red[slot][g][0] = a;
      red[slot][g][1] = b;
    }
    __syncthreads();
    if (threadIdx.x < p.groups) {
      double a = 0.0, b = 0.0;
      for (int q = 0; q < S; ++q) {
        a += red[q][threadIdx.x][0];
        b += red[q][threadIdx.x][1];
      }
      const double cnt = (double)p.rows_per_stat * (double)cpg;
      const double mean = a / cnt;
      double var = b / cnt - mean * mean;
      if (var < 0.0) var = 0.0;
      gm[threadIdx.x] = (float)mean;
      gr[threadIdx.x] = (float)(1.0 / sqrt(var + (double)p.eps));
    }
    __syncthreads();
  }
  float rs[SLOTS][8], rh[SLOTS][8];
#pragma unroll
  for (int k = 0; k < SLOTS; ++k) {
    const int c8 = tx + (k << txlog);
    if (c8 < C8) {
      const f32x4 g0 = *reinterpret_cast<const f32x4*>(p.gamma + (c8 << 3)), g1 = *reinterpret_cast<const f32x4*>(p.gamma + (c8 << 3) + 4);
      const f32x4 b0 = *reinterpret_cast<const f32x4*>(p.beta + (c8 << 3)), b1 = *reinterpret_cast<const f32x4*>(p.beta + (c8 << 3) + 4);
#pragma unroll
      for (int j = 0; j < 8; ++j) {
        const int gi = ((c8 << 3) + j) / cpg;
        const float scale = gr[gi] * (j < 4 ? g0[j & 3] : g1[j & 3]);
        rs[k][j] = scale;
        rh[k][j] = (j < 4 ? b0[j & 3] : b1[j & 3]) - gm[gi] * scale;
      }
    }
  }
  const int64_t r0 = (int64_t)chunk * p.rows_per_chunk;
  int64_t r1 = r0 + p.rows_per_chunk;
  if (r1 > p.rows_per_stat) r1 = p.rows_per_stat;
  const int64_t base_row = (int64_t)sg * p.rows_per_stat;
  for (int64_t piece = chunk;; piece += 2 * (int64_t)gridDim.x) {
    const int64_t ra = piece * TY + ty, rb = (piece + gridDim.x) * TY + ty;
    if (piece * TY >= p.rows_per_stat) break;
    const bool ok[2] = {ra < p.rows_per_stat, rb < p.rows_per_stat};
    const int64_t rows2[2] = {base_row + ra, base_row + rb};
    u32x4 raw[2][SLOTS];
#pragma unroll
    for (int h = 0; h < 2; ++h)
#pragma unroll
      for (int k = 0; k < SLOTS; ++k) {
        const int c8 = tx + (k << txlog);
        if (c8 < C8 && ok[h]) {
          const int ch = c8 << 3;
          const int64_t rr = rows2[h];
          raw[h][k] = ld16(ch < p.c1 ? p.x + rr * p.c1 + ch : p.x2 + rr * p.c2 + (ch - p.c1));
        }
      }
#pragma unroll
    for (int h = 0; h < 2; ++h)
#pragma unroll
      for (int k = 0; k < SLOTS; ++k) {
        const int c8 = tx + (k << txlog);
        if (c8 < C8 && ok[h]) {
          float f[8];
          unpack8<DT>(raw[h][k], f);
#pragma unroll
          for (int j = 0; j < 8; ++j) {
            const float v = f[j] * rs[k][j] + rh[k][j];
            f[j] = p.act == CA_ACT_SILU ? silu_f(v) : v;
          }
          st16(p.y + rows2[h] * C + (c8 << 3), pack8<DT>(f));
        }
      }
  }
}

constexpr int GNS_MAX = 12;
template <int DT, int NCH = GNS_MAX>
__global__ __launch_bounds__(256) void k_gn_small(GnParams p) {
  __shared__ double red[4][2];
  __shared__ float mr[2];
  const int C = p.c1 + p.c2;
  const int cpg = C / p.groups, q = cpg >> 3;
  const int g = blockIdx.x, sg = blockIdx.y;
  const int total = (int)p.rows_per_stat * q;
  const int64_t base_row = (int64_t)sg * p.rows_per_stat;
  const int lane = threadIdx.x & 63, wave = threadIdx.x >> 6;
  u32x4 raw[NCH];
  float s = 0.f, ss = 0.f;
#pragma unroll
  for (int k = 0; k < NCH; ++k) {
    const int id = threadIdx.x + k * 256;
    if (id < total) {
      const int row = id / q, ch = g * cpg + (id - row * q) * 8;
      const int64_t rr = base_row + row;
      raw[k] = ld16(ch < p.c1 ? p.x + rr * p.c1 + ch : p.x2 + rr * p.c2 + (ch - p.c1));
    }
  }
#pragma unroll
  for (int k = 0; k < NCH; ++k) {
    if (threadIdx.x + k * 256 < total) {
      float f[8];
      unpack8<DT>(raw[k], f);
#pragma unroll
      for (int j = 0; j < 8; ++j) {
        s += f[j];
        ss += f[j] * f[j];
      }
    }
  }
#pragma unroll
  for (int off = 1; off < 64; off <<= 1) {
    s += __shfl_xor(s, off);
    ss += __shfl_xor(ss, off);
  }
  if (lane == 0) {
    red[wave][0] = (double)s;
    red[wave][1] = (double)ss;
  }
  __syncthreads();
  if (threadIdx.x == 0) {
    const double a = red[0][0] + red[1][0] + red[2][0] + red[3][0], b = red[0][1] + red[1][1] + red[2][1] + red[3][1];
    const double cnt = (double)p.rows_per_stat * (double)cpg;
    const double mean = a / cnt;
    double var = b / cnt - mean * mean;
    if (var < 0.0) var = 0.0;
    mr[0] = (float)mean;
    mr[1] = (float)(1.0 / sqrt(var + (double)p.eps));
  }
  __syncthreads();
  const float mean = mr[0], rstd = mr[1];
#pragma unroll
  for (int k = 0; k < NCH; ++k) {
    const int id = threadIdx.x + k * 256;
    if (id < total) {
      const int row = id / q, ch = g * cpg + (id - row * q) * 8;
      const f32x4 g0 = *reinterpret_cast<const f32x4*>(p.gamma + ch), g1 = *reinterpret_cast<const f32x4*>(p.gamma + ch + 4);
      const f32x4 b0 = *reinterpret_cast<const f32x4*>(p.beta + ch), b1 = *reinterpret_cast<const f32x4*>(p.beta + ch + 4);
      float f[8];
      unpack8<DT>(raw[k], f);
#pragma unroll
      for (int j = 0; j < 8; ++j) {
        const float scale = rstd * (j < 4 ? g0[j & 3] : g1[j & 3]);
        const float v = f[j] * scale + ((j < 4 ? b0[j & 3] : b1[j & 3]) - mean * scale);
        f[j] = p.act == CA_ACT_SILU ? silu_f(v) : v;
      }
      st16(p.y + (base_row + row) * C + ch, pack8<DT>(f));
    }
  }
}

__device__ __forceinline__ unsigned gnw_pk_add(unsigned a, unsigned b) {
  unsigned r;
  asm("v_pk_add_f16 %0, %1, %2" : "=v"(r) : "v"(a), "v"(b));
  return r;
}
// ... 452 lines not shown
    const int txlog = gn_txlog(p.c >> 3);
    const int ty = 256 >> txlog;
    int64_t blocks = (p.rows + 2 * ty - 1) / (2 * ty);
    if (blocks > 8192) blocks = 8192;
    dim3 grid((unsigned)blocks), block(256);
    switch (txlog) {
      case 3: hipLaunchKernelGGL((k_ln_stats<DT, 3>), grid, block, 0, st, p); break;
      case 4: hipLaunchKernelGGL((k_ln_stats<DT, 4>), grid, block, 0, st, p); break;
      case 5: hipLaunchKernelGGL((k_ln_stats<DT, 5>), grid, block, 0, st, p); break;
      default: hipLaunchKernelGGL((k_ln_stats<DT, 6>), grid, block, 0, st, p); break;
    }
    return;
  }
  int64_t waves = (p.rows + LN_RPW - 1) / LN_RPW;
  int64_t blocks = (waves + 3) / 4;
  if (blocks > 16384) blocks = 16384;
  const int slots = (p.c / 8 + 63) / 64;
  dim3 grid((unsigned)blocks), block(256);
  switch (slots) {
    case 1: hipLaunchKernelGGL((k_layernorm<DT, 1>), grid, block, 0, st, p); break;
    case 2: hipLaunchKernelGGL((k_layernorm<DT, 2>), grid, block, 0, st, p); break;
    case 3: hipLaunchKernelGGL((k_layernorm<DT, 3>), grid, block, 0, st, p); break;
    default: hipLaunchKernelGGL((k_layernorm<DT, 4>), grid, block, 0, st, p); break;
  }
}

}

extern "C" int64_t ca_groupnorm_partials_floats(int32_t images, int32_t hw, int32_t frames_per_stat, int32_t groups) {
  if (images <= 0 || hw <= 0 || frames_per_stat <= 0 || groups <= 0) return 0;
  const int64_t nstat = images / frames_per_stat;
  return nstat * gn_chunks_host((int64_t)frames_per_stat * hw) * groups * 2;
}

template <int DT, int L>
void launch_gn_l(bool apply, int slots, const GnParams& p, dim3 grid, hipStream_t st) {
  if (slots <= 2) {
    if (apply) hipLaunchKernelGGL((k_gn_apply<DT, L, 2>), grid, dim3(256), 0, st, p);
    else hipLaunchKernelGGL((k_gn_stats<DT, L, 2>), grid, dim3(256), 0, st, p);
  } else if (slots <= 4) {
    if (apply) hipLaunchKernelGGL((k_gn_apply<DT, L, 4>), grid, dim3(256), 0, st, p);
    else hipLaunchKernelGGL((k_gn_stats<DT, L, 4>), grid, dim3(256), 0, st, p);
  } else {
    if (apply) hipLaunchKernelGGL((k_gn_apply<DT, L, 5>), grid, dim3(256), 0, st, p);
    else hipLaunchKernelGGL((k_gn_stats<DT, L, 5>), grid, dim3(256), 0, st, p);
  }
}

template <int DT>
void launch_gn(bool apply, const GnParams& p, dim3 grid, hipStream_t st) {
  const int c8 = (p.c1 + p.c2) >> 3;
  const int txlog = gn_txlog(c8);
  const int slots = (c8 + (1 << txlog) - 1) >> txlog;
  switch (txlog) {
    case 3: launch_gn_l<DT, 3>(apply, slots, p, grid, st); break;
    case 4: launch_gn_l<DT, 4>(apply, slots, p, grid, st); break;
    case 5: launch_gn_l<DT, 5>(apply, slots, p, grid, st); break;
    default: launch_gn_l<DT, 6>(apply, slots, p, grid, st);
  }
}

extern "C" int ca_groupnorm_stats(const ca_groupnorm_args* a, void* stream) {
  GnParams p{};
  int rc = gn_fill(a, p, "ca_groupnorm_stats");
  if (rc) return rc;
  dim3 grid(p.nchunks, a->images / a->frames_per_stat);
  if (a->dtype == CA_BF16) launch_gn<CA_BF16>(false, p, grid, (hipStream_t)stream);
  else launch_gn<CA_F16>(false, p, grid, (hipStream_t)stream);
  CA_CHECK_LAUNCH("ca_groupnorm_stats");
  return CA_OK;
}

extern "C" int ca_groupnorm_apply(const ca_groupnorm_args* a, void* stream) {
  GnParams p{};
  int rc = gn_fill(a, p, "ca_groupnorm_apply");
  if (rc) return rc;
  CA_REQUIRE(a->y && a->gamma && a->beta, "ca_groupnorm_apply: null operand");
  const int achunks = gn_chunks_rows(p.rows_per_stat, p.rows_per_stat >= 2048 ? 128 : 64);
  p.rows_per_chunk = (p.rows_per_stat + achunks - 1) / achunks;
  dim3 grid(achunks, a->images / a->frames_per_stat);
  if (a->dtype == CA_BF16) launch_gn<CA_BF16>(true, p, grid, (hipStream_t)stream);
  else launch_gn<CA_F16>(true, p, grid, (hipStream_t)stream);
  CA_CHECK_LAUNCH("ca_groupnorm_apply");
  return CA_OK;
}

extern "C" int ca_groupnorm_wino_supported(const ca_groupnorm_args* a) {
  if (!a || !a->x || !a->gamma || !a->beta || !a->wino_v || a->dtype != CA_F16 || a->frames_per_stat != 1) return 0;
  if (a->images <= 0 || a->c1 <= 0 || a->c1 % 8 || a->c2 < 0 || a->c2 % 8 || (a->c2 && !a->x2) || a->groups <= 0) return 0;
  const int C = a->c1 + a->c2;
  if (C % a->groups) return 0;
  const int cpg = C / a->groups;
  if (cpg % 8 || cpg > GNW_MAX_CPG || (a->c2 != 0 && a->c1 % cpg != 0)) return 0;
  if (a->wino_h < 2 || a->wino_w < 2 || (a->wino_h & 1) || (a->wino_w & 1) || a->wino_h * a->wino_w != a->hw || a->hw > GNW_MAX_ROWS) return 0;
  if ((int64_t)a->hw * (cpg >> 3) > 256 * GNS_MAX) return 0;
  if ((((uintptr_t)a->wino_v | (uintptr_t)a->x | (uintptr_t)a->x2) & 15) != 0) return 0;
  return 1;
}

extern "C" int ca_groupnorm(const ca_groupnorm_args* a, void* stream) {
  GnParams p{};
  if (a && a->wino_v) {
    CA_REQUIRE(ca_groupnorm_wino_supported(a), "ca_groupnorm: wino_v with arguments outside the fused form (fp16, per-image statistics, even image of <= 256 pixels, "
                                                "<= 80 channels per group in whole 8-channel chunks): ask ca_groupnorm_wino_supported() first");
    p.x = (const u16*)a->x;
    p.x2 = (const u16*)a->x2;
    p.gamma = a->gamma;
    p.beta = a->beta;
    p.c1 = a->c1, p.c2 = a->c2, p.groups = a->groups;
    p.rows_per_stat = a->hw;
    p.eps = a->eps;
    p.act = a->act;
    p.wino_v = (u16*)a->wino_v;
    p.wino_h = a->wino_h, p.wino_w = a->wino_w;
    {
      const int cpg_w = (a->c1 + a->c2) / a->groups;
      const int64_t per_thread = ((int64_t)a->hw * (cpg_w >> 3) + 255) / 256;
      const dim3 grid_w(a->groups, a->images);
      hipStream_t st_w = (hipStream_t)stream;
#define CA_GNW_CASE(N)                                                                                  \
  if (cpg_w <= 40) hipLaunchKernelGGL((k_gn_small_wino<N, 40>), grid_w, dim3(256), 0, st_w, p);         \
  else hipLaunchKernelGGL((k_gn_small_wino<N, GNW_MAX_CPG>), grid_w, dim3(256), 0, st_w, p);
      if (per_thread <= 2) { CA_GNW_CASE(2) }
      else if (per_thread <= 5) { CA_GNW_CASE(5) }
      else { CA_GNW_CASE(GNS_MAX) }
#undef CA_GNW_CASE
    }
    CA_CHECK_LAUNCH("ca_groupnorm(wino)");
    return CA_OK;
  }
  int rc = gn_fill(a, p, "ca_groupnorm");
  if (rc) return rc;
  CA_REQUIRE(a->y && a->gamma && a->beta, "ca_groupnorm: null operand");
  if (gn_small_ok(p)) {
    const dim3 grid(p.groups, a->images / a->frames_per_stat);
    const int64_t per_thread = (p.rows_per_stat * ((p.c1 + p.c2) / p.groups >> 3) + 255) / 256;
#define CA_GNS_CASE(N)                                                                                                     \
  if (a->dtype == CA_BF16) hipLaunchKernelGGL((k_gn_small<CA_BF16, N>), grid, dim3(256), 0, (hipStream_t)stream, p);       \
  else hipLaunchKernelGGL((k_gn_small<CA_F16, N>), grid, dim3(256), 0, (hipStream_t)stream, p);
    if (per_thread <= 2) { CA_GNS_CASE(2) }
    else if (per_thread <= 5) { CA_GNS_CASE(5) }
    else { CA_GNS_CASE(GNS_MAX) }
#undef CA_GNS_CASE
    CA_CHECK_LAUNCH("ca_groupnorm");
    return CA_OK;
  }
  if (const int uc = gn_unit_channels(p)) {
    const int units = (p.c1 + p.c2) / uc;
    const dim3 grid(units * (a->images / a->frames_per_stat));
    static const int gnu_small = CA_KNOB("CA_GN_UNIT_SMALL", 1);
    const bool few = gnu_small && (int64_t)p.rows_per_stat * (uc >> 3) <= 1024 * 5;
    if (a->dtype == CA_BF16) {
      if (few) hipLaunchKernelGGL((k_gn_unit<CA_BF16, 5>), grid, dim3(1024), 0, (hipStream_t)stream, p, uc, units);
      else hipLaunchKernelGGL((k_gn_unit<CA_BF16, GNU_MAX>), grid, dim3(1024), 0, (hipStream_t)stream, p, uc, units);
    } else {
      if (few) hipLaunchKernelGGL((k_gn_unit<CA_F16, 5>), grid, dim3(1024), 0, (hipStream_t)stream, p, uc, units);
      else hipLaunchKernelGGL((k_gn_unit<CA_F16, GNU_MAX>), grid, dim3(1024), 0, (hipStream_t)stream, p, uc, units);
    }
    CA_CHECK_LAUNCH("ca_groupnorm");
    return CA_OK;
  }
  rc = ca_groupnorm_stats(a, stream);
  if (rc) return rc;
  return ca_groupnorm_apply(a, stream);
}

// ... 49 lines not shown
```

controlanimate_amd/kernels.py:

```python
from __future__ import annotations

import ctypes as C
from typing import Optional

import torch

from . import _capi
from .context import dispatch
from ._capi import (AttnArgs, ConvArgs, ConvNarrowArgs, FfArgs, PerceiverAttnArgs, TattnArgs, XattnArgs, GemmArgs, GroupNormArgs, LayerNormArgs, CA_ACT_NONE,
                    CA_ACT_SILU, CA_BF16, CA_F16, check, lib)

ACT_NONE, ACT_SILU = CA_ACT_NONE, CA_ACT_SILU
ACT_QUICK_GELU, ACT_GELU = 2, 3
ACT_RELU = _capi.CA_ACT_RELU
ACT_RELU6 = _capi.CA_ACT_RELU6


def dt_code(dtype: torch.dtype) -> int:
    if dtype == torch.bfloat16:
        return CA_BF16
    if dtype == torch.float16:
        return CA_F16
    raise TypeError(f"activations must be bf16 or fp16, got {dtype}")


def _stream() -> int:
    return torch.cuda.current_stream().cuda_stream


def _p(t: Optional[torch.Tensor]) -> Optional[int]:
    return None if t is None else t.data_ptr()


def _req_cuda(*ts):
    for t in ts:
        if t is not None and not t.is_cuda:
            raise _capi.CAHipError("HIP kernels need device tensors (no CPU fallback)")


_plan_sink = None


def _record_plan(query, args) -> None:
    if _plan_sink is not None:
        buf = C.create_string_buffer(64)
        _plan_sink.append(buf.value.decode() if query(C.byref(args), buf, 64) == 0 else "?")


def gemm(a: torch.Tensor, w: torch.Tensor, *, a2: Optional[torch.Tensor] = None,
         bias: Optional[torch.Tensor] = None, rowbias: Optional[torch.Tensor] = None,
         rows_per_group: int = 0, residual: Optional[torch.Tensor] = None, alpha: float = 1.0,
         post_scale: float = 1.0, act: int = ACT_NONE, geglu: bool = False, out_f32: bool = False,
         out: Optional[torch.Tensor] = None, ln=None, row_sums: bool = False) -> torch.Tensor:
    _req_cuda(a, w, a2, bias, rowbias, residual, out)
    assert a.dim() == 2 and a.stride(1) == 1 and w.dim() == 2 and w.is_contiguous()
    m, k1 = a.shape
    k2 = 0
    if a2 is not None:
        assert a2.dim() == 2 and a2.stride(1) == 1 and a2.shape[0] == m and a2.dtype == a.dtype
        k2 = a2.shape[1]
    n = w.shape[0]
    assert w.shape[1] == k1 + k2 and w.dtype == a.dtype
    ncols = n // 2 if geglu else n
    if out is None:
        out = torch.empty((m, ncols), device=a.device, dtype=torch.float32 if out_f32 else a.dtype)
    assert out.shape == (m, ncols) and out.stride(1) == 1
    if residual is not None:
        assert residual.shape == (m, n) and residual.stride(1) == 1 and residual.dtype == a.dtype
    if bias is not None:
        assert bias.dtype == torch.float32 and bias.numel() == n
    if rowbias is not None:
        assert rowbias.dtype == torch.float32 and rowbias.dim() == 2 and rowbias.shape[1] == n and rows_per_group > 0
    args = GemmArgs(a=_p(a), a2=_p(a2), w=_p(w), c=_p(out), bias=_p(bias), rowbias=_p(rowbias),
                    residual=_p(residual), lda=a.stride(0), lda2=a2.stride(0) if a2 is not None else 0,
                    ldc=out.stride(0), ld_res=residual.stride(0) if residual is not None else 0,
                    ld_rowbias=rowbias.stride(0) if rowbias is not None else 0,
                    m=m, n=n, k1=k1, k2=k2, rows_per_group=rows_per_group, alpha=alpha,
                    post_scale=post_scale, act=act, geglu=int(geglu), out_f32=int(out_f32),
                    dtype=dt_code(a.dtype))
    frag = getattr(w, "_frag", None)
    if frag is not None and frag[1] == bool(geglu) and dispatch.gemm_ar:
        args.w_frag = _p(frag[0])
    if ln is not None:
        st, cs = ln
        assert cs.dtype == torch.float32 and cs.numel() == n
        args.ln_colsum = _p(cs)
        if isinstance(st, RowStats):
            assert st.x.data_ptr() == a.data_ptr() and st.x.shape == a.shape, "RowStats belongs to another tensor"
            args.ln_eps = st.eps
            if lib().ca_gemm_ln_inline_supported(C.byref(args)):
                pass
            elif st.sums is not None:
                rs, parts = st.sums
                assert rs.shape == (m, parts, 2) and rs.dtype == torch.float32 and rs.is_contiguous()
                args.ln_stats, args.ln_parts = _p(rs), min(parts, 4)
                if parts > 4 or lib().ca_gemm_wants_finished_stats(C.byref(args)):
                    fin = getattr(st, "_finished", None)
                    if fin is None:
                        fin = torch.empty((m, 2), device=a.device, dtype=torch.float32)
                        check(lib().ca_ln_finish_sums(_p(rs), parts, m, k1 + k2, st.eps, _p(fin), _stream()), "ca_ln_finish_sums")
                        st._finished = fin
                    args.ln_stats, args.ln_parts = _p(fin), 0
            else:
                st = st.tensor()
        if not isinstance(st, RowStats):
            assert st.dtype == torch.float32 and st.shape == (m, 2) and st.is_contiguous()
            args.ln_stats = _p(st)
    if hasattr(out, "_row_sums"):
        del out._row_sums
    if row_sums and dispatch.ln_row_sums and not geglu and not out_f32:
        parts = int(lib().ca_gemm_row_sums_parts(C.byref(args)))
        if parts > 0:
            rs = torch.empty((m, parts, 2), device=a.device, dtype=torch.float32)
            args.row_sums_out = _p(rs)
            out._row_sums = (rs, parts)
    wbytes = 0 if args.row_sums_out else int(lib().ca_gemm_workspace_bytes(C.byref(args)))
    if wbytes > 0:
        ws = torch.empty((wbytes,), device=a.device, dtype=torch.uint8)
        args.workspace, args.workspace_bytes = _p(ws), wbytes
    _record_plan(lib().ca_gemm_plan_name, args)
    check(lib().ca_gemm(C.byref(args), _stream()), "ca_gemm")
    return out


def attach_w_frag(w: torch.Tensor, geglu: bool = False) -> torch.Tensor:
    _req_cuda(w)
    if w.dim() != 2 or w.shape[1] != 320 or w.shape[0] % 320 != 0 or not w.is_contiguous() or w.dtype not in (torch.float16, torch.bfloat16):
        return w
    dst = torch.empty_like(w)
    check(lib().ca_pack_w_frag(w.data_ptr(), w.shape[0], w.shape[1], int(bool(geglu)), dst.data_ptr(), _stream()), "ca_pack_w_frag")
    w._frag = (dst, bool(geglu))
    return w


def ff_fused(x: torch.Tensor, w1_frag: torch.Tensor, bias1: torch.Tensor, colsum1: torch.Tensor, w2_frag: torch.Tensor,
             bias2: Optional[torch.Tensor], ln_eps: float, residual: Optional[torch.Tensor] = None,
             ln_stats: Optional[torch.Tensor] = None, *, w_out_frag: Optional[torch.Tensor] = None, bias_out: Optional[torch.Tensor] = None,
             residual_out: Optional[torch.Tensor] = None) -> Optional[torch.Tensor]:
    if not dispatch.ff_fused:
        return None
    _req_cuda(x, w1_frag, bias1, colsum1, w2_frag, bias2, residual, ln_stats, w_out_frag, bias_out, residual_out)
    if x.dim() != 2 or x.stride(1) != 1 or (residual is not None and (residual.shape != x.shape or residual.stride(1) != 1 or residual.dtype != x.dtype)):
        return None
    if w_out_frag is None and (bias_out is not None or residual_out is not None):
        return None
    if residual_out is not None and (residual_out.shape != x.shape or residual_out.stride(1) != 1 or residual_out.dtype != x.dtype):
        return None
    m, c = x.shape
    inner = w2_frag.shape[1]
    y = torch.empty((m, c), device=x.device, dtype=x.dtype)
    args = FfArgs(x=_p(x), w1_frag=_p(w1_frag), bias1=_p(bias1), colsum1=_p(colsum1), ln_stats=_p(ln_stats), w2_frag=_p(w2_frag),
                  bias2=_p(bias2), residual=_p(residual), y=_p(y), lda=x.stride(0), ldc=y.stride(0),
                  ld_res=residual.stride(0) if residual is not None else 0, m=m, c=c, inner=inner, ln_eps=float(ln_eps), dtype=dt_code(x.dtype),
                  w_out_frag=_p(w_out_frag), bias_out=_p(bias_out), residual_out=_p(residual_out),
                  ld_res_out=residual_out.stride(0) if residual_out is not None else 0)
    if not lib().ca_ff_fused_supported(C.byref(args)):
        return None
    if _plan_sink is not None:
        _plan_sink.append("ff_out128" if w_out_frag is not None else "ff_fused128")
    check(lib().ca_ff_fused(C.byref(args), _stream()), "ca_ff_fused")
    return y


def tattn_fused(x: torch.Tensor, w_frag: torch.Tensor, gamma: torch.Tensor, bias_pe: torch.Tensor, b: int, frames: int, tokens: int,
                heads: int, ln_eps: float, scale: float, *, w_out_frag: Optional[torch.Tensor] = None, bias_out: Optional[torch.Tensor] = None,
                residual: Optional[torch.Tensor] = None) -> Optional[torch.Tensor]:
    if not dispatch.tattn_fused:
        return None
    _req_cuda(x, w_frag, gamma, bias_pe, w_out_frag, bias_out, residual)
    if x.dim() != 2 or x.stride(1) != 1 or x.shape[0] != b * frames * tokens or bias_pe.shape[0] < frames or bias_pe.stride(1) != 1:
        return None
    if w_out_frag is None and (bias_out is not None or residual is not None):
        return None
    if residual is not None and (residual.shape != x.shape or residual.stride(1) != 1 or residual.dtype != x.dtype):
        return None
    c = x.shape[1]
    o = torch.empty((x.shape[0], c), device=x.device, dtype=x.dtype)
    args = TattnArgs(x=_p(x), w_frag=_p(w_frag), gamma=_p(gamma), bias_pe=_p(bias_pe), o=_p(o), lda=x.stride(0), ldo=o.stride(0),
                     ld_bias_pe=bias_pe.stride(0), batch=b, frames=frames, tokens=tokens, heads=heads, c=c, ln_eps=float(ln_eps),
                     scale=float(scale), dtype=dt_code(x.dtype), w_out_frag=_p(w_out_frag), bias_out=_p(bias_out), residual=_p(residual),
                     ld_res=residual.stride(0) if residual is not None else 0)
    if not lib().ca_tattn_fused_supported(C.byref(args)):
        return None
    if _plan_sink is not None:
        _plan_sink.append("tattn_out128" if w_out_frag is not None else "tattn_fused128")
    check(lib().ca_tattn_fused(C.byref(args), _stream()), "ca_tattn_fused")
    return o


def xattn_pack_kv(kv: torch.Tensor, kv_batches: int, rows_per_batch: int, nk: int, scale: float, row_offset: int = 0,
                  out: Optional[torch.Tensor] = None) -> Optional[torch.Tensor]:
    if (not dispatch.xattn_fused or kv.dim() != 2 or kv.shape[1] != 640 or kv.stride(1) != 1 or not (64 < nk <= 80 or 1 <= nk <= 16)
            or kv.dtype not in (torch.float16, torch.bfloat16)):
        return None
    _req_cuda(kv)
    dst = out if out is not None else torch.empty((kv_batches, 8, _capi.XATTN_KV_FRAG_ELEMS), device=kv.device, dtype=kv.dtype)
    assert dst.shape == (kv_batches, 8, _capi.XATTN_KV_FRAG_ELEMS) and dst.dtype == kv.dtype and dst.is_contiguous()
    check(lib().ca_xattn_pack_kv(kv.data_ptr(), kv.stride(0), kv_batches, rows_per_batch, row_offset, nk, float(scale), dt_code(kv.dtype),
                                 dst.data_ptr(), _stream()), "ca_xattn_pack_kv")
    return dst


def xattn_fused(x: torch.Tensor, wq_frag: torch.Tensor, bias: Optional[torch.Tensor], kv_frag: torch.Tensor, images: int, tokens: int,
                frames_per_kv: int, kv_mod: int, nk: int, ln_eps: float, *, w_out_frag: Optional[torch.Tensor] = None,
                bias_out: Optional[torch.Tensor] = None, residual: Optional[torch.Tensor] = None, kv_frag_ip: Optional[torch.Tensor] = None,
# ... 121 lines not shown
    cout = w_phase.shape[1]
    assert tuple(w_phase.shape) == (4, cout, 2, 2, cin)
    y = torch.empty((images, 2 * hin, 2 * win, cout), device=x.device, dtype=x.dtype)
    if residual is not None:
        assert residual.dtype == x.dtype and residual.is_contiguous() and residual.numel() == y.numel()
    if bias is not None:
        assert bias.dtype == torch.float32 and bias.numel() == cout
    args = _up2_args(x, w_phase, bias, residual, alpha, y)
    _record_plan(lib().ca_conv_up2_phase_plan_name, args)
    check(lib().ca_conv_up2_phase(C.byref(args), _stream()), "ca_conv_up2_phase")
    return y


_gn_wino_declined: dict = {}


def group_norm_conv3x3_wino(x: torch.Tensor, gamma: torch.Tensor, beta: torch.Tensor, w: torch.Tensor, w_wino: torch.Tensor, *,
                            x2: Optional[torch.Tensor] = None, groups: int = 32, eps: float = 1e-5, act: int = ACT_NONE,
                            bias: Optional[torch.Tensor] = None, rowbias: Optional[torch.Tensor] = None, rows_per_group: int = 0,
                            residual: Optional[torch.Tensor] = None, post_scale: float = 1.0) -> Optional[torch.Tensor]:
    if not (dispatch.conv_winograd and dispatch.gn_winograd):
        return None
    _req_cuda(x, gamma, beta, w, w_wino, x2, bias, rowbias, residual)
    if x.dim() != 4 or not x.is_contiguous() or x.dtype != torch.float16 or (x2 is not None and (not x2.is_contiguous() or x2.shape[:3] != x.shape[:3])):
        return None
    images, h, w_, c1 = x.shape
    c2 = 0 if x2 is None else x2.shape[3]
    c, cout = c1 + c2, w.shape[0]
    tiles = images * (h // 2) * (w_ // 2)
    key = (images, h, w_, c1, c2, cout, groups, act, rowbias is not None, residual is not None, rows_per_group)
    if _gn_wino_declined.get(key):
        return None
    cargs = ConvArgs(x=_p(x), x2=None, w=_p(w), y=_p(x), bias=_p(bias), rowbias=_p(rowbias), residual=_p(residual),
                     ld_res=cout if residual is not None else 0, ld_rowbias=rowbias.stride(0) if rowbias is not None else 0, images=images, hin=h,
                     win=w_, cin1=c, cin2=0, cout=cout, stride=1, upsample=0, rows_per_group=rows_per_group, alpha=1.0, post_scale=post_scale,
                     act=ACT_NONE, out_f32=0, dtype=dt_code(x.dtype), pad_asym=0, w_wino=_p(w_wino), x_is_wino_v=1)
    cargs.workspace, cargs.workspace_bytes = _p(x), 1 << 60
    buf = C.create_string_buffer(64)
    if lib().ca_conv3x3_plan_name(C.byref(cargs), buf, 64) != 0 or not buf.value.decode().startswith("wino"):
        _gn_wino_declined[key] = True
        return None
    wbytes = int(lib().ca_conv3x3_workspace_bytes(C.byref(cargs)))
    gargs = GroupNormArgs(x=_p(x), x2=_p(x2), y=None, gamma=_p(gamma), beta=_p(beta), partials=None, images=images, hw=h * w_, c1=c1, c2=c2,
                          groups=groups, frames_per_stat=1, eps=eps, act=act, dtype=dt_code(x.dtype), wino_v=_p(x), wino_h=h, wino_w=w_)
    if wbytes <= 0 or not lib().ca_groupnorm_wino_supported(C.byref(gargs)):
        _gn_wino_declined[key] = True
        return None
    y = torch.empty((images, h, w_, cout), device=x.device, dtype=x.dtype)
    v = torch.empty((16, tiles, c), device=x.device, dtype=x.dtype)
    if residual is not None:
        assert residual.dtype == x.dtype and residual.is_contiguous() and residual.numel() == y.numel()
    ws = torch.empty((wbytes,), device=x.device, dtype=torch.uint8)
    cargs.x, cargs.y, gargs.wino_v = _p(v), _p(y), _p(v)
    cargs.workspace, cargs.workspace_bytes = _p(ws), wbytes
    if _plan_sink is not None:
        buf = C.create_string_buffer(64)
        _plan_sink.append("gn_" + (buf.value.decode() if lib().ca_conv3x3_plan_name(C.byref(cargs), buf, 64) == 0 else "?"))
    check(lib().ca_groupnorm(C.byref(gargs), _stream()), "ca_groupnorm(wino)")
    check(lib().ca_conv3x3(C.byref(cargs), _stream()), "ca_conv3x3(wino, V given)")
    return y


def group_norm(x: torch.Tensor, gamma: torch.Tensor, beta: torch.Tensor, *, x2: Optional[torch.Tensor] = None,
               groups: int = 32, frames_per_stat: int = 1, eps: float = 1e-5, act: int = ACT_NONE) -> torch.Tensor:
    _req_cuda(x, gamma, beta, x2)
    assert x.dim() == 4 and x.is_contiguous()
    images, h, w_, c1 = x.shape
    c2 = 0
    if x2 is not None:
        assert x2.is_contiguous() and x2.shape[:3] == x.shape[:3] and x2.dtype == x.dtype
        c2 = x2.shape[3]
    c = c1 + c2
    assert gamma.dtype == torch.float32 and beta.dtype == torch.float32 and gamma.numel() == c and beta.numel() == c
    y = torch.empty((images, h, w_, c), device=x.device, dtype=x.dtype)
    nfl = lib().ca_groupnorm_partials_floats(images, h * w_, frames_per_stat, groups)
    partials = torch.empty((max(int(nfl), 1),), device=x.device, dtype=torch.float32)
    args = GroupNormArgs(x=_p(x), x2=_p(x2), y=_p(y), gamma=_p(gamma), beta=_p(beta), partials=_p(partials),
                         images=images, hw=h * w_, c1=c1, c2=c2, groups=groups,
                         frames_per_stat=frames_per_stat, eps=eps, act=act, dtype=dt_code(x.dtype))
    check(lib().ca_groupnorm(C.byref(args), _stream()), "ca_groupnorm")
    return y


def layer_norm(x: torch.Tensor, gamma: torch.Tensor, beta: torch.Tensor, *, pos: Optional[torch.Tensor] = None,
               rows_per_frame: int = 1, frames: int = 1, eps: float = 1e-5) -> torch.Tensor:
    _req_cuda(x, gamma, beta, pos)
    assert x.dim() == 2 and x.is_contiguous()
    rows, c = x.shape
    assert gamma.dtype == torch.float32 and beta.dtype == torch.float32
    if pos is not None:
        assert pos.dtype == torch.float32 and pos.is_contiguous() and pos.shape == (frames, c)
    y = torch.empty_like(x)
    args = LayerNormArgs(x=_p(x), y=_p(y), gamma=_p(gamma), beta=_p(beta), pos=_p(pos), rows=rows, c=c,
                         rows_per_frame=rows_per_frame, frames=frames, eps=eps, dtype=dt_code(x.dtype))
    check(lib().ca_layernorm(C.byref(args), _stream()), "ca_layernorm")
    return y


def row_stats(x: torch.Tensor, eps: float = 1e-5) -> torch.Tensor:
    _req_cuda(x)
    assert x.dim() == 2 and x.is_contiguous()
    rows, c = x.shape
    st = torch.empty((rows, 2), device=x.device, dtype=torch.float32)
    args = LayerNormArgs(x=_p(x), y=None, gamma=None, beta=None, pos=None, rows=rows, c=c, rows_per_frame=1, frames=1,
                         eps=eps, dtype=dt_code(x.dtype), stats=_p(st))
    check(lib().ca_layernorm(C.byref(args), _stream()), "ca_layernorm(stats)")
    return st


def attention_raw(q: torch.Tensor, k: torch.Tensor, v: torch.Tensor, o: torch.Tensor, *, q_off: int, k_off: int,
                  v_off: int, o_off: int, q_strides, o_strides, k_strides, inner_count: int, kv_inner_count: int,
                  kv_div: int, batches: int, heads: int, head_dim: int, nq: int, nk: int, scale: float,
                  out_scale: float = 1.0, accumulate: bool = False, kv_mod: int = 0, causal: bool = False,
                  key_mask: Optional[torch.Tensor] = None) -> None:
    _req_cuda(q, k, v, o, key_mask)
    if key_mask is not None:
        assert key_mask.dtype == torch.uint8 and key_mask.dim() == 2 and key_mask.shape == (batches, nk) and key_mask.stride(1) == 1
    es = q.element_size()
    args = AttnArgs(q=q.data_ptr() + q_off * es, k=k.data_ptr() + k_off * es, v=v.data_ptr() + v_off * es,
                    o=o.data_ptr() + o_off * es,
                    q_outer=q_strides[0], q_inner=q_strides[1], q_row=q_strides[2],
                    o_outer=o_strides[0], o_inner=o_strides[1], o_row=o_strides[2],
                    k_outer=k_strides[0], k_inner=k_strides[1], k_row=k_strides[2],
                    inner_count=inner_count, kv_inner_count=kv_inner_count, kv_div=kv_div,
                    kv_mod=kv_mod if kv_mod > 0 else batches, batches=batches, heads=heads, head_dim=head_dim, nq=nq, nk=nk, scale=scale, out_scale=out_scale,
                    accumulate=int(accumulate), dtype=dt_code(q.dtype), causal=int(causal),
                    key_mask=_p(key_mask), key_mask_stride=key_mask.stride(0) if key_mask is not None else 0)
    _record_plan(lib().ca_attention_plan_name, args)
    check(lib().ca_attention(C.byref(args), _stream()), "ca_attention")


def attention_spatial(qkv: torch.Tensor, images: int, tokens: int, heads: int, causal: bool = False,
                      key_mask: Optional[torch.Tensor] = None) -> torch.Tensor:
    c = qkv.shape[1] // 3
    d = c // heads
    o = torch.empty((images * tokens, c), device=qkv.device, dtype=qkv.dtype)
    ld = qkv.stride(0)
    attention_raw(qkv, qkv, qkv, o, q_off=0, k_off=c, v_off=2 * c, o_off=0,
                  q_strides=(tokens * ld, 0, ld), o_strides=(tokens * c, 0, c), k_strides=(tokens * ld, 0, ld),
                  inner_count=1, kv_inner_count=1, kv_div=1, batches=images, heads=heads, head_dim=d,
                  nq=tokens, nk=tokens, scale=d ** -0.5, causal=causal, key_mask=key_mask)
    return o


def attention_cross(q: torch.Tensor, kv: torch.Tensor, images: int, tokens: int, heads: int, kv_tokens: int,
                    kv_rows_per_batch: int, frames_per_kv: int, *, out: Optional[torch.Tensor] = None,
                    out_scale: float = 1.0, accumulate: bool = False, kv_row_offset: int = 0,
                    kv_mod: int = 0, key_mask: Optional[torch.Tensor] = None) -> torch.Tensor:
    c = q.shape[1]
    d = c // heads
    if out is None:
        out = torch.empty_like(q)
    ldk = kv.stride(0)
    attention_raw(q, kv, kv, out, q_off=0, k_off=kv_row_offset * ldk, v_off=kv_row_offset * ldk + c, o_off=0,
                  q_strides=(tokens * q.stride(0), 0, q.stride(0)), o_strides=(tokens * out.stride(0), 0, out.stride(0)),
                  k_strides=(kv_rows_per_batch * ldk, 0, ldk), inner_count=1, kv_inner_count=1,
                  kv_div=frames_per_kv, batches=images, heads=heads, head_dim=d, nq=tokens, nk=kv_tokens,
                  scale=d ** -0.5, out_scale=out_scale, accumulate=accumulate, kv_mod=kv_mod, key_mask=key_mask)
    return out


def attention_temporal(qkv: torch.Tensor, b: int, frames: int, tokens: int, heads: int) -> torch.Tensor:
    c = qkv.shape[1] // 3
    d = c // heads
    o = torch.empty((b * frames * tokens, c), device=qkv.device, dtype=qkv.dtype)
    ld = qkv.stride(0)
# ... 664 lines not shown
```

controlanimate_amd/layers.py:

```python
from __future__ import annotations

from typing import Callable, List, Optional, Sequence, Tuple

import torch
from torch import nn

from . import kernels as K
from .context import dispatch

ALIGN = 256


class Packed:

    __slots__ = ("shape", "dtype", "fill", "offset", "t", "frag")

    def __init__(self, shape, dtype, fill):
        self.shape = tuple(int(s) for s in shape)
        self.dtype = dtype
        self.fill = fill
        self.offset = -1
        self.t: Optional[torch.Tensor] = None
        self.frag = None

# ... 120 lines not shown
        super().__init__()
        self.in_channels, self.out_channels = in_channels, out_channels
        self.weight = nn.Parameter(torch.empty(out_channels, in_channels, 1, 1))
        self.bias = nn.Parameter(torch.zeros(out_channels))
        nn.init.normal_(self.weight, std=in_channels ** -0.5)
        self.w = self.b = None

    def pack(self, arena: WeightArena, dtype):
        self.w = arena.add((self.out_channels, self.in_channels), dtype, lambda: _f32(self.weight).reshape(self.out_channels, self.in_channels))
        self.b = arena.add((self.out_channels,), torch.float32, lambda: _f32(self.bias))

    def run(self, a: torch.Tensor, **kw) -> torch.Tensor:
        return K.gemm(a, self.w.t, bias=self.b.t, **kw)


def phase_weights(w: torch.Tensor) -> torch.Tensor:
    sel = torch.tensor([[[1.0, 0.0, 0.0], [0.0, 1.0, 1.0]], [[1.0, 1.0, 0.0], [0.0, 0.0, 1.0]]], dtype=w.dtype, device=w.device)
    wp = torch.einsum("ydk,xel,oikl->yxodei", sel, sel, w)
    return wp.reshape(4, w.shape[0], 2, 2, w.shape[1]).contiguous()


class HipConv3x3(nn.Module):

    def __init__(self, in_channels: int, out_channels: int, stride: int = 1):
        super().__init__()
        self.in_channels, self.out_channels, self.stride = in_channels, out_channels, stride
        self.cin_pad = (in_channels + 7) // 8 * 8
        self.weight = nn.Parameter(torch.empty(out_channels, in_channels, 3, 3))
        self.bias = nn.Parameter(torch.zeros(out_channels))
        nn.init.normal_(self.weight, std=(9 * in_channels) ** -0.5)
        self.w = self.b = None
        self.winograd = True
        self.up2_phase = False

    def _packed_weight(self) -> torch.Tensor:
        w = _f32(self.weight).permute(0, 2, 3, 1)
        if self.cin_pad != self.in_channels:
            w = torch.nn.functional.pad(w, (0, self.cin_pad - self.in_channels))
        return w.contiguous()

    def _winograd_weight(self) -> torch.Tensor:
        g = torch.tensor([[1.0, 0.0, 0.0], [0.5, 0.5, 0.5], [0.5, -0.5, 0.5], [0.0, 0.0, 1.0]], dtype=torch.float32, device=self.weight.device)
        u = torch.einsum("xk,oikl,yl->xyoi", g, _f32(self.weight), g)
        return u.reshape(16, self.out_channels, self.in_channels).contiguous()

    def pack(self, arena: WeightArena, dtype):
        self.w = arena.add((self.out_channels, 3, 3, self.cin_pad), dtype, self._packed_weight)
        self.b = arena.add((self.out_channels,), torch.float32, lambda: _f32(self.bias))
        self.u = None
        if (dispatch.conv_winograd and self.stride == 1 and self.winograd and self.in_channels >= 640 and self.in_channels % 64 == 0
                and self.out_channels % 320 == 0):
            self.u = arena.add((16, self.out_channels, self.in_channels), dtype, self._winograd_weight)
        self.wp = None
        if dispatch.conv_up2_phase and self.up2_phase and self.stride == 1 and self.in_channels % 64 == 0 and self.out_channels % 320 == 0:
            self.wp = arena.add((4, self.out_channels, 2, 2, self.in_channels), dtype, lambda: phase_weights(_f32(self.weight)))

    def run(self, x: torch.Tensor, **kw) -> torch.Tensor:
        wp = getattr(self, "wp", None)
        if wp is not None and dispatch.conv_up2_phase and kw.get("upsample") and set(kw) <= {"upsample", "residual", "alpha"}:
            ph = {k: v for k, v in kw.items() if k != "upsample"}
            if K.conv_up2_phase_supported(x, wp.t, bias=self.b.t, **ph):
                return K.conv_up2_phase(x, wp.t, bias=self.b.t, **ph)
        u = getattr(self, "u", None)
        return K.conv3x3(x, self.w.t, bias=self.b.t, stride=self.stride, w_wino=None if u is None else u.t, **kw)


class HipGroupNorm(nn.Module):
    def __init__(self, num_groups: int, num_channels: int, eps: float = 1e-5):
        super().__init__()
        self.num_groups, self.num_channels, self.eps = num_groups, num_channels, eps
        self.weight = nn.Parameter(torch.ones(num_channels))
        self.bias = nn.Parameter(torch.zeros(num_channels))
        self.g = self.b = None

    def pack(self, arena: WeightArena, dtype):
        self.g = arena.add((self.num_channels,), torch.float32, lambda: _f32(self.weight))
        self.b = arena.add((self.num_channels,), torch.float32, lambda: _f32(self.bias))

    def run(self, x: torch.Tensor, *, x2: Optional[torch.Tensor] = None, frames_per_stat: int = 1, act: int = K.ACT_NONE):
        return K.group_norm(x, self.g.t, self.b.t, x2=x2, groups=self.num_groups, frames_per_stat=frames_per_stat,
                            eps=self.eps, act=act)


class HipLayerNorm(nn.Module):
    def __init__(self, dim: int, eps: float = 1e-5):
        super().__init__()
        self.dim, self.eps = dim, eps
        self.weight = nn.Parameter(torch.ones(dim))
        self.bias = nn.Parameter(torch.zeros(dim))
        self.g = self.b = None

    def pack(self, arena: WeightArena, dtype):
        self.g = arena.add((self.dim,), torch.float32, lambda: _f32(self.weight))
        self.b = arena.add((self.dim,), torch.float32, lambda: _f32(self.bias))

    def run(self, x: torch.Tensor, *, pos: Optional[torch.Tensor] = None, rows_per_frame: int = 1, frames: int = 1):
        return K.layer_norm(x, self.g.t, self.b.t, pos=pos, rows_per_frame=rows_per_frame, frames=frames, eps=self.eps)


def pack_concat_rows(arena: WeightArena, dtype, mods: Sequence[nn.Module]) -> Packed:
    n = sum(m.weight.shape[0] for m in mods)
    k = mods[0].weight.shape[1]
    return arena.add((n, k), dtype, lambda: torch.cat([_f32(m.weight).reshape(m.weight.shape[0], -1) for m in mods], 0))


def pack_concat_bias(arena: WeightArena, mods: Sequence[nn.Module]) -> Packed:
    n = sum(m.weight.shape[0] for m in mods)
    return arena.add((n,), torch.float32, lambda: torch.cat([_f32(m.bias) for m in mods], 0))


def ln_fold_enabled() -> bool:
    from .context import dispatch
    return bool(dispatch.ln_fold)


class LnFold:

    def __init__(self, arena: WeightArena, dtype, ln: "HipLayerNorm", mods: Sequence[nn.Module], geglu: bool = False, pe=None):
        n = sum(m.weight.shape[0] for m in mods)
        k = mods[0].weight.shape[1]
        self.eps = ln.eps

        def w_cat():
            return torch.cat([_f32(m.weight).reshape(m.weight.shape[0], -1) for m in mods], 0)

        def w_fold():
            w = w_cat() * _f32(ln.weight)[None, :]
            return geglu_interleave(w) if geglu else w

        def bias():
            b = w_cat() @ _f32(ln.bias)
            b = b + torch.cat([_f32(m.bias) if getattr(m, "bias", None) is not None else torch.zeros(m.weight.shape[0], device=m.weight.device) for m in mods], 0)
            return geglu_interleave(b) if geglu else b

        self.w = arena.add((n, k), dtype, w_fold)
        self.w_fold = w_fold
        if frag_wanted(n, k):
            self.w.frag = (arena.add((n, k), dtype, lambda: frag_order(w_fold(), geglu)), geglu)
        self.cs = arena.add((n,), torch.float32, lambda: w_fold().to(dtype).float().sum(1))
        self.b = arena.add((n,), torch.float32, bias)
        self.pe = None
        if pe is not None:
            self.pe = arena.add((pe.shape[-2], n), torch.float32, lambda: _f32(pe).reshape(pe.shape[-2], k).to(mods[0].weight.device) @ w_cat().to(dtype).float().t())
        self._rb_cache = {}

    def rowbias(self, b: int, f: int) -> torch.Tensor:
        if f > self.pe.t.shape[0]:
            raise ValueError(f"video_length {f} exceeds temporal_position_encoding_max_len {self.pe.t.shape[0]}")
        key = (b, f, self.pe.t.data_ptr())
        rb = self._rb_cache.get(key)
        if rb is None:
            rb = self._rb_cache[key] = self.pe.t[:f].repeat(b, 1).contiguous()
        return rb


def geglu_interleave(w: torch.Tensor) -> torch.Tensor:
    d = w.shape[0] // 2
    return torch.stack([w[:d], w[d:]], dim=1).reshape(w.shape)
```

controlanimate_amd/motion_module.py:

```python
from __future__ import annotations

import math

import torch
from torch import nn

from . import kernels as K
from .attention import FeedForward
from .attention_processor import Attention
from .context import ExecCtx
from .layers import HipGroupNorm, HipLayerNorm, HipLinear, WeightArena, _f32


def get_motion_module(in_channels, motion_module_type: str, motion_module_kwargs: dict):
    if motion_module_type == "Vanilla":
        return VanillaTemporalModule(in_channels=in_channels, **motion_module_kwargs)
    raise ValueError(motion_module_type)


class PositionalEncoding(nn.Module):
    def __init__(self, d_model, dropout=0.0, max_len=24):
        super().__init__()
        position = torch.arange(max_len).unsqueeze(1)
        div_term = torch.exp(torch.arange(0, d_model, 2) * (-math.log(10000.0) / d_model))
        pe = torch.zeros(1, max_len, d_model)
        pe[0, :, 0::2] = torch.sin(position * div_term)
        pe[0, :, 1::2] = torch.cos(position * div_term)
        self.register_buffer("pe", pe)
        self.max_len = max_len
        self.table = None

    def pack(self, arena: WeightArena, dtype):
        self.table = arena.add((self.pe.shape[1], self.pe.shape[2]), torch.float32, lambda: _f32(self.pe)[0])


class VersatileAttention(Attention):
    def __init__(self, attention_mode=None, cross_frame_attention_mode=None, temporal_position_encoding=False,
                 temporal_position_encoding_max_len=24, *args, **kwargs):
        super().__init__(*args, **kwargs)
        assert attention_mode == "Temporal"
        self.attention_mode = attention_mode
        self.is_cross_attention = kwargs.get("cross_attention_dim") is not None
        if self.is_cross_attention:
            raise NotImplementedError("Temporal_Cross is not used by inference-v{1,2}.yaml")
        self.pos_encoder = PositionalEncoding(kwargs["query_dim"], max_len=temporal_position_encoding_max_len) \
            if temporal_position_encoding else None

    def pack(self, arena, dtype, fold_ln=None):
        pe = self.pos_encoder.pe if (fold_ln is not None and self.pos_encoder is not None) else None
        super().pack(arena, dtype, fold_ln=fold_ln, pe=pe)
        if self.pos_encoder is not None:
            self.pos_encoder.pack(arena, dtype)
        self.tfrag = self.tgamma = self.tbias_pe = None
        no_bias = all(getattr(m, "bias", None) is None for m in (self.to_q, self.to_k, self.to_v))
        if self.fold is not None and pe is not None and no_bias and (self.heads, self.inner_dim, self.query_dim) == (8, 320, 320):
            from .layers import _f32, frag_order_tattn
            self.tfrag = arena.add((368640,), dtype, lambda: frag_order_tattn(torch.cat([_f32(m.weight) for m in (self.to_q, self.to_k, self.to_v)], 0)))
            self.tgamma = arena.add((320,), torch.float32, lambda: _f32(fold_ln.weight))
            self.tbias_pe = arena.add((pe.shape[-2], 320), torch.float32,
                                      lambda: _f32(pe).reshape(pe.shape[-2], 320).to(fold_ln.bias.device) + _f32(fold_ln.bias)[None, :])
            self.tln_eps = fold_ln.eps

    def pos_table(self, frames: int):
        if self.pos_encoder is None:
            return None
        if frames > self.pos_encoder.max_len:
            raise ValueError(f"video_length {frames} exceeds temporal_position_encoding_max_len {self.pos_encoder.max_len}")
        return self.pos_encoder.table.t[:frames]


class TemporalTransformerBlock(nn.Module):
    def __init__(self, dim, num_attention_heads, attention_head_dim, attention_block_types=("Temporal_Self", "Temporal_Self"),
                 dropout=0.0, cross_attention_dim=768, activation_fn="geglu", attention_bias=False, upcast_attention=False,
                 cross_frame_attention_mode=None, temporal_position_encoding=False, temporal_position_encoding_max_len=24, **_):
        super().__init__()
        self.attention_blocks = nn.ModuleList([
            VersatileAttention(attention_mode=name.split("_")[0],
                               cross_attention_dim=cross_attention_dim if name.endswith("_Cross") else None,
                               query_dim=dim, heads=num_attention_heads, dim_head=attention_head_dim, bias=attention_bias,
                               temporal_position_encoding=temporal_position_encoding,
                               temporal_position_encoding_max_len=temporal_position_encoding_max_len)
            for name in attention_block_types])
        self.norms = nn.ModuleList([HipLayerNorm(dim) for _ in attention_block_types])
        self.ff = FeedForward(dim, activation_fn=activation_fn)
        self.ff_norm = HipLayerNorm(dim)

    def pack(self, arena, dtype):
        for attn, norm in zip(self.attention_blocks, self.norms):
            attn.pack(arena, dtype, fold_ln=norm)
            norm.pack(arena, dtype)
        self.ff.pack(arena, dtype, fold_ln=self.ff_norm)
        self.ff_norm.pack(arena, dtype)

    def forward(self, x: torch.Tensor, ctx: ExecCtx, tokens: int, proj_out=None) -> torch.Tensor:
        rows, C = x.shape
        nblk = len(self.attention_blocks)
        for i, (attn, norm) in enumerate(zip(self.attention_blocks, self.norms)):
            nxt = (self.attention_blocks[i + 1].fold if i + 1 < nblk else self.ff.fold) is not None
            if attn.fold is not None:
                o = attn(x.view(1, rows, C), residual=x.view(1, rows, C), temporal=(ctx.b, ctx.f, tokens),
                         ln=(K.RowStats(x, norm.eps, K.row_sums_of(x)), attn.fold), row_sums=nxt)
            else:
                n = norm.run(x, pos=attn.pos_table(ctx.f), rows_per_frame=tokens, frames=ctx.f)
                o = attn(n.view(1, rows, C), residual=x.view(1, rows, C), temporal=(ctx.b, ctx.f, tokens), row_sums=nxt)
            x = K.carry_row_sums(o.view(rows, C), o)
        if self.ff.fold is None:
            return self.ff.run(self.ff_norm.run(x), residual=x)
        if proj_out is not None and K.row_sums_of(x) is None:
            y = self.ff.run_with_proj_out(x, x, *proj_out)
            if y is not None:
                y._proj_out_done = True
                return y
        return self.ff.run(x, residual=x, sums=K.row_sums_of(x))


class TemporalTransformer3DModel(nn.Module):
    def __init__(self, in_channels, num_attention_heads, attention_head_dim, num_layers, norm_num_groups=32, **kw):
        super().__init__()
        inner = num_attention_heads * attention_head_dim
        self.norm = HipGroupNorm(norm_num_groups, in_channels, eps=1e-6)
        self.proj_in = HipLinear(in_channels, inner)
        self.transformer_blocks = nn.ModuleList([
            TemporalTransformerBlock(dim=inner, num_attention_heads=num_attention_heads,
                                     attention_head_dim=attention_head_dim, **kw) for _ in range(num_layers)])
        self.proj_out = HipLinear(inner, in_channels)

    def pack(self, arena, dtype):
        self.norm.pack(arena, dtype)
        self.proj_in.pack(arena, dtype)
        for b in self.transformer_blocks:
            b.pack(arena, dtype)
        self.proj_out.pack(arena, dtype)
        self.proj_out_frag = None
        po = self.proj_out
        if tuple(po.weight.shape) == (320, 320) and getattr(self.transformer_blocks[-1].ff, "w2f", None) is not None:
            from .layers import frag_order_wout
            self.proj_out_frag = arena.add((102400,), dtype, lambda: frag_order_wout(_f32(po.weight)))

    def forward(self, x: torch.Tensor, ctx: ExecCtx) -> torch.Tensor:
        images, h, w, c = x.shape
        rows = images * h * w
        y = self.norm.run(x)
        y = self.proj_in.run(y.view(rows, c), row_sums=self.transformer_blocks[0].attention_blocks[0].fold is not None)
        pfrag = getattr(self, "proj_out_frag", None)
        last = len(self.transformer_blocks) - 1
        for k, blk in enumerate(self.transformer_blocks):
            y = blk(y, ctx, h * w, proj_out=(pfrag, self.proj_out.b, x.view(rows, c)) if (k == last and pfrag is not None) else None)
        if getattr(y, "_proj_out_done", False):
            return y.view(images, h, w, c)
        return self.proj_out.run(y, residual=x.view(rows, c)).view(images, h, w, c)


class VanillaTemporalModule(nn.Module):
    def __init__(self, in_channels, num_attention_heads=8, num_transformer_block=2,
                 attention_block_types=("Temporal_Self", "Temporal_Self"), cross_frame_attention_mode=None,
                 temporal_position_encoding=False, temporal_position_encoding_max_len=24, temporal_attention_dim_div=1,
                 zero_initialize=True):
        super().__init__()
        self.temporal_transformer = TemporalTransformer3DModel(
            in_channels=in_channels, num_attention_heads=num_attention_heads,
            attention_head_dim=in_channels // num_attention_heads // temporal_attention_dim_div,
            num_layers=num_transformer_block, attention_block_types=attention_block_types,
            cross_frame_attention_mode=cross_frame_attention_mode, temporal_position_encoding=temporal_position_encoding,
            temporal_position_encoding_max_len=temporal_position_encoding_max_len)
        if zero_initialize:
            nn.init.zeros_(self.temporal_transformer.proj_out.weight)
            nn.init.zeros_(self.temporal_transformer.proj_out.bias)

    def pack(self, arena, dtype):
        self.temporal_transformer.pack(arena, dtype)

    def forward(self, x: torch.Tensor, ctx: ExecCtx) -> torch.Tensor:
        return self.temporal_transformer(x, ctx)
```

include/controlanimate_hip.h:

```cpp
#ifndef CONTROLANIMATE_HIP_H
#define CONTROLANIMATE_HIP_H

#include <stdint.h>

#ifdef __cplusplus
extern "C" {
#endif

#define CA_ABI_VERSION 16

#define CA_BF16 0
#define CA_F16 1
#define CA_F32 2

#define CA_OK 0
#define CA_ERR_INVALID_ARG (-1)
#define CA_ERR_UNSUPPORTED (-2)
#define CA_ERR_LAUNCH (-3)

#define CA_ACT_NONE 0
#define CA_ACT_SILU 1
#define CA_ACT_QUICK_GELU 2
#define CA_ACT_GELU 3
#define CA_ACT_RELU 4
// ... 20 lines not shown
  int32_t dtype;
  const float* ln_stats;
  const float* ln_colsum;
  float ln_eps;
  void* workspace;
  int64_t workspace_bytes;
  float* row_sums_out;
  int32_t ln_parts;
  const void* w_frag;
} ca_gemm_args;
int ca_gemm(const ca_gemm_args* args, void* stream);
int ca_pack_w_frag(const void* w, int32_t n, int32_t k, int32_t geglu, void* dst, void* stream);
typedef struct ca_ff_args {
  const void* x;
  const void* w1_frag;
  const float* bias1;
  const float* colsum1;
  const float* ln_stats;
  const void* w2_frag;
  const float* bias2;
  const void* residual;
  void* y;
  int64_t lda, ldc, ld_res;
  int32_t m, c, inner;
  float ln_eps;
  int32_t dtype;
  const void* w_out_frag;
  const float* bias_out;
  const void* residual_out;
  int64_t ld_res_out;
} ca_ff_args;
int ca_ff_fused(const ca_ff_args* args, void* stream);
int ca_ff_fused_supported(const ca_ff_args* args);
int ca_pack_w2_frag(const void* w, int32_t n, int32_t k, void* dst, void* stream);
#define CA_TATTN_W_FRAG_ELEMS 368640
typedef struct ca_tattn_args {
  const void* x;
  const void* w_frag;
  const float* gamma;
  const float* bias_pe;
  void* o;
  int64_t lda, ldo, ld_bias_pe;
  int32_t batch, frames, tokens, heads, c;
  float ln_eps, scale;
  int32_t dtype;
  const void* w_out_frag;
  const float* bias_out;
  const void* residual;
  int64_t ld_res;
} ca_tattn_args;
int ca_tattn_fused(const ca_tattn_args* args, void* stream);
int ca_tattn_fused_supported(const ca_tattn_args* args);
#define CA_ATTN_WOUT_FRAG_ELEMS 102400
int ca_pack_w_out(const void* w, int32_t n, int32_t k, void* dst, void* stream);
int ca_pack_w_tattn(const void* w, int32_t n, int32_t k, void* dst, void* stream);
#define CA_XATTN_W_FRAG_ELEMS 122880
#define CA_XATTN_KV_FRAG_ELEMS 7680
typedef struct ca_xattn_args {
  const void* x;
  const void* wq_frag;
  const float* bias;
  const void* kv_frag;
  void* o;
  int64_t lda, ldo;
  int32_t m, tokens, frames_per_kv, kv_mod, kv_batches, nk, heads, c;
  float ln_eps;
  int32_t dtype;
  const void* w_out_frag;
  const float* bias_out;
  const void* residual;
  int64_t ld_res;
  const void* kv_frag_ip;
  int32_t nk_ip;
  float ip_scale;
} ca_xattn_args;
int ca_xattn_fused(const ca_xattn_args* args, void* stream);
int ca_xattn_fused_supported(const ca_xattn_args* args);
int ca_xattn_pack_w(const void* w, int32_t n, int32_t k, void* dst, void* stream);
int ca_xattn_pack_kv(const void* kv, int64_t ld, int32_t kv_batches, int32_t rows_per_batch, int32_t row_offset, int32_t nk, float scale, int32_t dtype,
                     void* dst, void* stream);
int64_t ca_gemm_workspace_bytes(const ca_gemm_args* args);
int ca_gemm_row_sums_parts(const ca_gemm_args* args);
int ca_gemm_ln_inline_supported(const ca_gemm_args* args);
int ca_gemm_wants_finished_stats(const ca_gemm_args* args);
int ca_ln_finish_sums(const float* sums, int parts, int64_t rows, int k, float eps, float* mean_rstd, void* stream);
int ca_gemm_plan_name(const ca_gemm_args* args, char* buf, int32_t len);

typedef struct ca_conv_args {
  const void* x;
  const void* x2;
  const void* w;
  void* y;
  const float* bias;
  const float* rowbias;
  const void* residual;
  int64_t ld_res, ld_rowbias;
  int32_t images, hin, win, cin1, cin2, cout;
  int32_t stride;
  int32_t upsample;
  int32_t rows_per_group;
  float alpha, post_scale;
  int32_t act;
  int32_t out_f32;
  int32_t dtype;
  void* workspace;
  int64_t workspace_bytes;
  int32_t pad_asym;
  const void* w_wino;
  int32_t x_is_wino_v;
} ca_conv_args;
int ca_pack_w_wino(const void* w, int32_t cout, int32_t cin, int32_t dtype, void* dst, void* stream);
int64_t ca_conv3x3_workspace_bytes(const ca_conv_args* args);
int ca_conv3x3(const ca_conv_args* args, void* stream);
int ca_conv3x3_plan_name(const ca_conv_args* args, char* buf, int32_t len);
int ca_conv_up2_phase_supported(const ca_conv_args* args);
int ca_conv_up2_phase(const ca_conv_args* args, void* stream);
int ca_conv_up2_phase_plan_name(const ca_conv_args* args, char* buf, int32_t len);

typedef struct ca_groupnorm_args {
  const void* x;
  const void* x2;
  void* y;
  const float* gamma;
  const float* beta;
  float* partials;
  int32_t images, hw, c1, c2;
  int32_t groups;
  int32_t frames_per_stat;
  float eps;
  int32_t act;
  int32_t dtype;
  void* wino_v;
  int32_t wino_h, wino_w;
} ca_groupnorm_args;
int ca_groupnorm_wino_supported(const ca_groupnorm_args* args);
int64_t ca_groupnorm_partials_floats(int32_t images, int32_t hw, int32_t frames_per_stat, int32_t groups);
int ca_groupnorm_stats(const ca_groupnorm_args* args, void* stream);
int ca_groupnorm_apply(const ca_groupnorm_args* args, void* stream);
int ca_groupnorm(const ca_groupnorm_args* args, void* stream);

typedef struct ca_layernorm_args {
  const void* x; void* y;
  const float* gamma; const float* beta;
  const float* pos;
  int64_t rows;
  int32_t c;
  int32_t rows_per_frame, frames;
  float eps;
  int32_t dtype;
  float* stats;
} ca_layernorm_args;
int ca_layernorm(const ca_layernorm_args* args, void* stream);

typedef struct ca_attn_args {
  const void* q; const void* k; const void* v; void* o;
  int64_t q_outer, q_inner, q_row;
  int64_t o_outer, o_inner, o_row;
  int64_t k_outer, k_inner, k_row;
  int32_t inner_count, kv_inner_count, kv_div, kv_mod;
  int32_t batches, heads, head_dim;
  int32_t nq, nk;
  float scale;
  float out_scale;
  int32_t accumulate;
  int32_t dtype;
  int32_t causal;
  const uint8_t* key_mask;
  int64_t key_mask_stride;
} ca_attn_args;
int ca_attention(const ca_attn_args* args, void* stream);
int ca_attention_plan_name(const ca_attn_args* args, char* buf, int32_t len);


int ca_add_bcast(const void* a, const void* b, void* out, int64_t n, int64_t b_period,
                 int32_t dtype, void* stream);
int ca_repeat(const void* src, void* dst, int64_t bytes, int32_t times, void* stream);

int ca_softmax_rows(const float* x, void* y, int64_t rows, int32_t cols, int64_t ldx, int64_t ldy,
                    float scale, int32_t dtype, void* stream);

int ca_silu_f32(const float* x, float* y, int64_t n, void* stream);

int ca_timestep_embedding(const float* t_dev, float t_host, void* out, int32_t batch,
                          int32_t dim, int32_t dtype, void* stream);

int ca_latents_to_nhwc(const float* latents, void* out, int32_t b0, int32_t c, int32_t f,
                       int32_t h, int32_t w, int32_t cpad, int32_t rep, float in_scale,
                       int32_t dtype, void* stream);

int ca_nhwc_to_ncfhw_f32(const void* x, float* out, int32_t b, int32_t c, int32_t f, int32_t h,
                         int32_t w, int32_t ldx, int32_t x_is_f32, int32_t dtype, void* stream);

int ca_ncfhw_to_nhwc(const void* x, int32_t x_kind , const int64_t strides[5],
                     void* out, int32_t b, int32_t c, int32_t f, int32_t h, int32_t w, int32_t cpad,
                     int32_t dtype, void* stream);

int ca_cfg_scheduler_step(const float* eps, int32_t ld_eps, int32_t rep, float guidance,
                          const float* latents, const float* noise, float* prev, float* denoised,
                          int32_t c, int32_t f, int32_t h, int32_t w, const float coef[7],
                          float clip, void* stream);

int ca_lincomb(float* out, const float* const* x, const float* coef, int32_t n_terms, int64_t n, void* stream);

typedef struct ca_conv3x3_narrow_args {
  const void* x;
  const void* w;
  void* y;
  const float* bias;
  const void* r1;
  const void* r2;
  int64_t ldx, ldy, ld_r1, ld_r2;
  int32_t images, hin, win, cin, cout;
  int32_t channel_offset;
  int32_t upsample;
  int32_t leaky_relu;
  float s0, s1, s2;
  int32_t out_u8;
  int32_t dtype;
} ca_conv3x3_narrow_args;
int ca_conv3x3_narrow(const ca_conv3x3_narrow_args* args, void* stream);
int ca_conv3x3_narrow_plan_name(const ca_conv3x3_narrow_args* args, char* buf, int32_t len);

// ... 130 lines not shown
```

Before: 15.96.

## Fuse GroupNorm apply into proj_in GEMM using precomputed per-image moments

Adds a GroupNorm-moments kernel and a GEMM variant that normalizes A fragments in registers with per-channel scale/shift derived from the moments, gamma and beta. The transformer and motion module proj_in paths use it when shapes qualify (K=320, 10 channels per group). This removes the separate GroupNorm apply pass and the write and re-read of the normalized activation. The cost is extra VALU work interleaved with the MFMAs in the GEMM inner loop, plus added complexity.

Result: no change. 16.05, median of 6 (+0.6%).

```diff
diff --git a/controlanimate_amd/_capi.py b/controlanimate_amd/_capi.py
--- a/controlanimate_amd/_capi.py
+++ b/controlanimate_amd/_capi.py
@@ -38,6 +38,10 @@
         ("row_sums_out", C.c_void_p), ("ln_parts", C.c_int32),
         ("w_frag", C.c_void_p),
     ]
+
+
+class GemmGnArgs(C.Structure):
+    _fields_ = [("moments", C.c_void_p), ("gamma", C.c_void_p), ("beta", C.c_void_p), ("groups", C.c_int32), ("rows_per_image", C.c_int32)]
 
 
 class FfArgs(C.Structure):
@@ -255,6 +259,10 @@
     "ca_cdcm_dil4": (C.c_int, [C.c_void_p, C.c_void_p, C.c_void_p, C.c_int32, C.c_int32, C.c_int32, C.c_int32, C.c_int32, C.c_void_p]),
     "ca_csam_reduce": (C.c_int, [C.c_void_p] * 9 + [C.c_int32] * 5 + [C.c_void_p]),
     "ca_softedge_fuse": (C.c_int, [C.c_void_p] * 5 + [C.c_int32] * 4 + [C.c_void_p] * 3 + [C.c_int32, C.c_int32, C.c_void_p]),
+    "ca_gemm_gn_inline_supported": (C.c_int, [C.POINTER(GemmArgs), C.POINTER(GemmGnArgs)]),
+    "ca_gemm_gn": (C.c_int, [C.POINTER(GemmArgs), C.POINTER(GemmGnArgs), C.c_void_p]),
+    "ca_groupnorm_moments_partials_floats": (C.c_int64, [C.c_int32, C.c_int32, C.c_int32]),
+    "ca_groupnorm_moments": (C.c_int, [C.POINTER(GroupNormArgs), C.c_void_p, C.c_void_p]),
 }
 
 _lib = None
diff --git a/controlanimate_amd/attention.py b/controlanimate_amd/attention.py
--- a/controlanimate_amd/attention.py
+++ b/controlanimate_amd/attention.py
@@ -8,7 +8,7 @@
 from . import kernels as K
 from .attention_processor import Attention, AttnProcessor2_0
 from .context import ExecCtx, dispatch
-from .layers import HipConv1x1, HipGroupNorm, HipLayerNorm, HipLinear, LnFold, WeightArena, _f32, geglu_interleave, ln_fold_enabled
+from .layers import HipConv1x1, HipGroupNorm, HipLayerNorm, HipLinear, LnFold, WeightArena, _f32, geglu_interleave, group_norm_proj, ln_fold_enabled
 
 
 class GEGLU(nn.Module):
@@ -168,8 +168,7 @@
     def forward(self, x: torch.Tensor, ctx: ExecCtx, shared_half: bool = False) -> torch.Tensor:
         images, h, w, c = x.shape
         rows = images * h * w
-        y = self.norm.run(x)
-        y0 = self.proj_in.run(y.view(rows, c), row_sums=self.transformer_blocks[0].attn1.fold is not None)
+        y0 = group_norm_proj(self.norm, self.proj_in, x, row_sums=self.transformer_blocks[0].attn1.fold is not None)
         y = K.carry_row_sums(y0.view(images, h * w, -1), y0)
         nblk = len(self.transformer_blocks)
         pfrag = getattr(self, "proj_out_frag", None)
diff --git a/controlanimate_amd/context.py b/controlanimate_amd/context.py
--- a/controlanimate_amd/context.py
+++ b/controlanimate_amd/context.py
@@ -37,6 +37,7 @@
     conv_winograd = True
     gn_winograd = True
     conv_up2_phase = True
+    gn_proj_in = True
     ln_row_sums = True
     repeat_kernel = True
     ln_fold = True
diff --git a/controlanimate_amd/csrc/ca_gemm.hip b/controlanimate_amd/csrc/ca_gemm.hip
--- a/controlanimate_amd/csrc/ca_gemm.hip
+++ b/controlanimate_amd/csrc/ca_gemm.hip
@@ -435,6 +435,18 @@
   return CA_OK;
 }
 
+extern "C" int ca_gemm_gn(const ca_gemm_args* a, const ca_gemm_gn_args* gn, void* stream) {
+  CA_REQUIRE(gn != nullptr, "ca_gemm_gn: null gn args");
+  DenseLaunch d;
+  int rc = gemm_prepare(a, d, gn);
+  if (rc) return rc;
+  hipStream_t st = (hipStream_t)stream;
+  rc = a->dtype == CA_BF16 ? launch_gemm<CA_BF16, 0>(d.p, d.plan, st) : launch_gemm<CA_F16, 0>(d.p, d.plan, st);
+  if (rc) return rc;
+  CA_CHECK_LAUNCH("ca_gemm_gn");
+  return CA_OK;
+}
+
 extern "C" int64_t ca_gemm_workspace_bytes(const ca_gemm_args* a) {
   DenseLaunch d;
   return gemm_resolve(a, d) == CA_OK ? d.workspace : 0;
@@ -450,6 +462,11 @@
 extern "C" int ca_gemm_ln_inline_supported(const ca_gemm_args* a) {
   DenseLaunch d;
   return a && a->ln_colsum && gemm_resolve(a, d) == CA_OK && wres_eligible(d.p) ? 1 : 0;
+}
+
+extern "C" int ca_gemm_gn_inline_supported(const ca_gemm_args* a, const ca_gemm_gn_args* gn) {
+  DenseLaunch d;
+  return a && gn && gemm_resolve(a, d, DenseAsk{}, gn) == CA_OK && gn_inline_ok(d.p, d.plan) ? 1 : 0;
 }
 
 extern "C" int ca_gemm_wants_finished_stats(const ca_gemm_args* a) {
diff --git a/controlanimate_amd/csrc/ca_gemm_core.h b/controlanimate_amd/csrc/ca_gemm_core.h
--- a/controlanimate_amd/csrc/ca_gemm_core.h
+++ b/controlanimate_amd/csrc/ca_gemm_core.h
@@ -38,6 +38,10 @@
   unsigned w_group_stride;
   int up2_rows, up2_tiles;
   unsigned up2_mag_w, up2_mag_h;
+  const float* gn_moments;
+  const float* gn_gamma;
+  const float* gn_beta;
+  int gn_groups, gn_rows_per_image;
 };
 
 constexpr int BK = 64;
diff --git a/controlanimate_amd/csrc/ca_gemm_plan.h b/controlanimate_amd/csrc/ca_gemm_plan.h
--- a/controlanimate_amd/csrc/ca_gemm_plan.h
+++ b/controlanimate_amd/csrc/ca_gemm_plan.h
@@ -168,7 +168,7 @@
   bool stats_finished;
 };
 
-inline int gemm_fill(const ca_gemm_args* a, GemmKParams& p, const DenseAsk& ask) {
+inline int gemm_fill(const ca_gemm_args* a, GemmKParams& p, const DenseAsk& ask, const ca_gemm_gn_args* gn = nullptr) {
   CA_REQUIRE(a != nullptr, "ca_gemm: null args");
   CA_REQUIRE(a->a && a->w && a->c, "ca_gemm: null operand");
   CA_REQUIRE(a->m > 0 && a->k1 > 0 && a->k2 >= 0, "ca_gemm: bad sizes m=%d k1=%d k2=%d", a->m, a->k1, a->k2);
@@ -202,7 +202,19 @@
   p.rows_per_group = a->rows_per_group > 0 ? a->rows_per_group : 1;
   p.alpha = a->alpha, p.post = a->post_scale, p.act = a->act, p.geglu = a->geglu, p.out_f32 = a->out_f32;
   p.splits = 1;
-  return CA_OK;
+  if (gn) {
+    CA_REQUIRE(gn->moments && gn->gamma && gn->beta && gn->groups > 0 && gn->rows_per_image > 0, "ca_gemm_gn: null operand or bad sizes");
+    p.gn_moments = gn->moments, p.gn_gamma = gn->gamma, p.gn_beta = gn->beta;
+    p.gn_groups = gn->groups, p.gn_rows_per_image = gn->rows_per_image;
+  }
+  return CA_OK;
+}
+
+inline bool gn_inline_ok(const GemmKParams& p, const GemmPlan& plan) {
+  return plan.kind == PK_WRES && p.gn_moments && p.c2 == 0 && !p.ln_colsum && !p.ln_stats && !p.ln_inline && !p.rowbias && !p.geglu &&
+         p.alpha == 1.f && p.post == 1.f && p.act == CA_ACT_NONE &&
+         p.gn_rows_per_image % 256 == 0 && p.m % p.gn_rows_per_image == 0 && p.gn_groups > 0 && (p.c1 + p.c2) / p.gn_groups == 10 &&
+         (p.c1 + p.c2) % p.gn_groups == 0;
 }
 
 struct DenseLaunch {
@@ -210,10 +222,10 @@
   GemmPlan plan;
   int64_t workspace;
 };
-inline int gemm_resolve(const ca_gemm_args* a, DenseLaunch& d, const DenseAsk& ask = DenseAsk{}) {
+inline int gemm_resolve(const ca_gemm_args* a, DenseLaunch& d, const DenseAsk& ask = DenseAsk{}, const ca_gemm_gn_args* gn = nullptr) {
   d = DenseLaunch{};
   GemmKParams& p = d.p;
-  int rc = gemm_fill(a, p, ask);
+  int rc = gemm_fill(a, p, ask, gn);
   if (rc) return rc;
   const SplitK k = splitk_decide(p, 0);
   splitk_apply(k, a->workspace, a->workspace_bytes, p);
@@ -226,12 +238,14 @@
   return CA_OK;
 }
 
-inline int gemm_prepare(const ca_gemm_args* a, DenseLaunch& d) {
-  int rc = gemm_resolve(a, d);
+inline int gemm_prepare(const ca_gemm_args* a, DenseLaunch& d, const ca_gemm_gn_args* gn = nullptr) {
+  int rc = gemm_resolve(a, d, DenseAsk{}, gn);
   if (rc) return rc;
   CA_REQUIRE(!d.p.row_sums || row_sums_capable(d.p), "ca_gemm: row_sums_out is not available for this launch: ask ca_gemm_row_sums_parts() first");
   CA_REQUIRE(!d.p.ln_inline || wres_eligible(d.p), "ca_gemm: in-kernel LayerNorm statistics (ln_stats NULL) are not available for this launch: "
              "ask ca_gemm_ln_inline_supported() first and pass ln_stats otherwise");
+  CA_REQUIRE(!gn || gn_inline_ok(d.p, d.plan), "ca_gemm_gn: GroupNorm inside the GEMM is not available for this launch: "
+             "ask ca_gemm_gn_inline_supported() first and run ca_groupnorm + ca_gemm otherwise");
   return CA_OK;
 }
 
diff --git a/controlanimate_amd/csrc/ca_gemm_pp.hip b/controlanimate_amd/csrc/ca_gemm_pp.hip
--- a/controlanimate_amd/csrc/ca_gemm_pp.hip
+++ b/controlanimate_amd/csrc/ca_gemm_pp.hip
@@ -80,6 +80,11 @@
       if (per * 8 > chunks) per = chunks / 8;
       if (per < 1) per = 1;
       const unsigned rb_bytes = p.rowbias ? (unsigned)(((int64_t)((p.m - 1) / p.rows_per_group) * p.ld_rowbias + p.n) * 4) : 16u;
+      if (p.gn_moments) {
+        const unsigned mom_bytes = (unsigned)(p.m / p.gn_rows_per_image) * 256u;
+        hipLaunchKernelGGL((k_gemm_wres_gn<DT>), dim3(8 * per * panels), dim3(512), 0, st, p, panels, 8 * per, chunks, mom_bytes, c_bytes, res_bytes);
+        return CA_OK;
+      }
       hipLaunchKernelGGL((k_gemm_wres<DT>), dim3(8 * per * panels), dim3(512), 0, st, p, panels, 8 * per, chunks, rb_bytes, c_bytes, res_bytes);
       return CA_OK;
     }
diff --git a/controlanimate_amd/csrc/ca_gemm_wres.h b/controlanimate_amd/csrc/ca_gemm_wres.h
--- a/controlanimate_amd/csrc/ca_gemm_wres.h
+++ b/controlanimate_amd/csrc/ca_gemm_wres.h
@@ -5,8 +5,8 @@
   return 32 * (j >> 1) + 8 * (i >> 2) + 4 * (j & 1) + (i & 3);
 }
 
-template <int DT>
-__global__ __launch_bounds__(512, 1) void k_gemm_wres(GemmKParams p, int panels, int lanes, int chunks, unsigned rb_bytes, unsigned c_bytes, unsigned res_bytes) {
+template <int DT, bool GN>
+__device__ __forceinline__ void gemm_wres_body(const GemmKParams& p, int panels, int lanes, int chunks, unsigned rb_bytes, unsigned c_bytes, unsigned res_bytes) {
   constexpr int K = 320, PN = 160, TN = 10, KQ = 10;
   constexpr int WLD_B = 656;
   constexpr int W_BYTES = PN * WLD_B;
@@ -28,7 +28,8 @@
   if (my_lane >= lanes) return;
   const int n0 = panel * PN;
 
-  const bool geglu = p.geglu != 0;
+  const bool geglu = !GN && p.geglu != 0;
+  const bool ln_fold = !GN && p.ln_colsum != nullptr;
   for (int q = tid; q < PN * (K / 8); q += 512) {
     const int row = q / (K / 8), c = q - row * (K / 8);
     *reinterpret_cast<u32x4*>(smem + row * WLD_B + c * 16) = ld16(p.w + (int64_t)(n0 + ca_wres_col(row >> 4, row & 15, geglu)) * K + c * 8);
@@ -38,10 +39,13 @@
     const int n = tid < PN ? tid : tid - PN;
     reinterpret_cast<float*>(smem + OFF_PAR)[tid] = src ? src[n0 + n] : 0.f;
   }
+  if (GN) {
+    for (int q = tid; q < 2 * K; q += 512) reinterpret_cast<float*>(smem + OFF_RB)[q] = q < K ? p.gn_gamma[q] : p.gn_beta[q - K];
+  }
   __syncthreads();
 
-  const __amdgpu_buffer_rsrc_t rs_rb = __builtin_amdgcn_make_buffer_rsrc((void*)(p.rowbias ? (const void*)p.rowbias : (const void*)p.w), 0, rb_bytes, 0x00020000);
-  unsigned char* rb_patch = smem + OFF_RB + wid * 1024;
+  const __amdgpu_buffer_rsrc_t rs_rb = __builtin_amdgcn_make_buffer_rsrc((void*)(GN ? (const void*)p.gn_moments : p.rowbias ? (const void*)p.rowbias : (const void*)p.w), 0, rb_bytes, 0x00020000);
+  unsigned char* rb_patch = GN ? smem + OFF_RB + 4096 + wid * 512 : smem + OFF_RB + wid * 1024;
   const __amdgpu_buffer_rsrc_t rs_c = __builtin_amdgcn_make_buffer_rsrc(p.c, 0, c_bytes, 0x00020000);
   const __amdgpu_buffer_rsrc_t rs_res = __builtin_amdgcn_make_buffer_rsrc((void*)(p.res ? (const void*)p.res : (const void*)p.c), 0, p.res ? res_bytes : 0u, 0x00020000);
   const __amdgpu_buffer_rsrc_t rs_a = __builtin_amdgcn_make_buffer_rsrc((void*)p.a, 0, p.a_bytes, 0x00020000);
@@ -57,9 +61,16 @@
   int d_c = my_lane, d_k = 0, d_s = 0;
   int d_n = 0;
   unsigned d_v1[2], d_v2[2];
+  int d_i = 0;
   auto head_slab = [&]() {
     int lane_o = lane;
     asm volatile("" : "+v"(lane_o));
+    if (GN) {
+      const int m_first = d_c * 256;
+      const unsigned off = m_first < p.m ? (unsigned)(m_first / p.gn_rows_per_image) * 256u + (unsigned)lane_o * 4u : DMA_OOB;
+      __builtin_amdgcn_raw_ptr_buffer_load_lds(rs_rb, (__attribute__((address_space(3))) void*)(rb_patch + d_i * 256), 4, off, 0, 0, 0);
+      d_i ^= 1;
+    }
 #pragma unroll
     for (int h = 0; h < 2; ++h) {
       const int m = d_c * 256 + wid * 32 + h * 16 + (lane_o >> 2);
@@ -109,14 +120,31 @@
   };
   int r_n = 0;
 
+  float sc[8], sh[8];
+  auto gn_coeffs = [&](const unsigned char* mo, int kq) __attribute__((always_inline)) {
+    const int c0 = kq * 32 + (lane >> 4) * 8, ga = c0 / 10, na = (ga + 1) * 10 - c0;
+    const float2 mo_a = *reinterpret_cast<const float2*>(mo + ga * 8);
+    const float2 mo_b = *reinterpret_cast<const float2*>(mo + (ga < 31 ? ga + 1 : 31) * 8);
+    const f32x4 gm0 = *reinterpret_cast<const f32x4*>(smem + OFF_RB + c0 * 4), gm1 = *reinterpret_cast<const f32x4*>(smem + OFF_RB + c0 * 4 + 16);
+    const f32x4 bt0 = *reinterpret_cast<const f32x4*>(smem + OFF_RB + (K + c0) * 4), bt1 = *reinterpret_cast<const f32x4*>(smem + OFF_RB + (K + c0) * 4 + 16);
+#pragma unroll
+    for (int j = 0; j < 8; ++j) {
+      const float scale = (j < na ? mo_a.y : mo_b.y) * (j < 4 ? gm0[j & 3] : gm1[j & 3]);
+      sc[j] = scale;
+      sh[j] = (j < 4 ? bt0[j & 3] : bt1[j & 3]) - (j < na ? mo_a.x : mo_b.x) * scale;
+    }
+  };
+
   head_slab();
   issue();
   issue();
   chunk_wait(0, 0xFFFFFFFEu);
+  if (GN) gn_coeffs(rb_patch, 0);
 
   const int fa_lane = l15 * 64 + g * 16;
   const unsigned char* wb = smem + l15 * WLD_B + g * 16;
   int r_s = 0;
+  int r_i = 0;
 
   for (int c = my_lane; c < chunks; c += lanes) {
     const int m0 = c * 256 + wid * 32;
@@ -128,14 +156,16 @@
 
     float2 st[2] = {make_float2(0.f, 0.f), make_float2(0.f, 0.f)};
     float ln_s[2] = {0.f, 0.f}, ln_ss[2] = {0.f, 0.f};
-    if (p.ln_stats) {
+    if (!GN && p.ln_stats) {
 #pragma unroll
       for (int i = 0; i < 2; ++i) {
         const int m = m0 + i * 16 + l15;
         if (m < p.m) st[i] = *reinterpret_cast<const float2*>(p.ln_stats + (int64_t)m * 2);
       }
     }
-    if (p.rowbias) {
+    const unsigned char* const mom = rb_patch + r_i * 256;
+    r_i ^= 1;
+    if (!GN && p.rowbias) {
       int lane_o = lane;
       asm volatile("" : "+v"(lane_o));
       const unsigned off = (lane_o < PN / 4 && m0 < p.m) ? ((unsigned)(m0 / p.rows_per_group) * (unsigned)p.ld_rowbias + (unsigned)n0) * 4u + (unsigned)lane_o * 16u : DMA_OOB;
@@ -146,8 +176,8 @@
       issue();
       const unsigned char* as = ring + r_s * SLOT + fa_lane;
       __builtin_amdgcn_sched_barrier(0);
-      const u32x4 fa0 = *reinterpret_cast<const u32x4*>(as);
-      const u32x4 fa1 = *reinterpret_cast<const u32x4*>(as + 1024);
+      u32x4 fa0 = *reinterpret_cast<const u32x4*>(as);
+      u32x4 fa1 = *reinterpret_cast<const u32x4*>(as + 1024);
       u32x4 fb[TN];
 #pragma unroll
       for (int j = 0; j < TN; ++j) {
@@ -161,8 +191,43 @@
   acc[0][J] = Elem<DT>::mfma(fb[J], fa0, acc[0][J]);                \
   acc[1][J] = Elem<DT>::mfma(fb[J], fa1, acc[1][J]);                \
   __builtin_amdgcn_sched_barrier(0);
+      unsigned flag_next;
+      if (GN) {
+        float f0[8], f1[8];
+        unpack8<DT>(fa0, f0);
+#pragma unroll
+        for (int j = 0; j < 8; ++j) f0[j] = fmaf(f0[j], sc[j], sh[j]);
+        fa0 = pack8<DT>(f0);
+        __builtin_amdgcn_sched_barrier(0);
+#define CA_WRES_ROW0(J, CNT)                                        \
+  asm volatile("s_waitcnt lgkmcnt(" #CNT ")" ::: "memory");         \
+  __builtin_amdgcn_sched_barrier(0);                                \
+  acc[0][J] = Elem<DT>::mfma(fb[J], fa0, acc[0][J]);                \
+  __builtin_amdgcn_sched_barrier(0);
+#define CA_WRES_ELEM(J)                                                                                                       \
+  f1[J] = fmaf(Elem<DT>::to_f((u16)((J) & 1 ? fa1[(J) >> 1] >> 16 : fa1[(J) >> 1] & 0xffffu)), sc[J], sh[J]);                  \
+  __builtin_amdgcn_sched_barrier(0);
+        CA_WRES_ROW0(0, 9) CA_WRES_ELEM(0) CA_WRES_ROW0(1, 8) CA_WRES_ELEM(1) CA_WRES_ROW0(2, 7) CA_WRES_ELEM(2)
+        CA_WRES_ROW0(3, 6) CA_WRES_ELEM(3) CA_WRES_ROW0(4, 5) CA_WRES_ELEM(4)
+        asm volatile("ds_read_b32 %0, %1" : "=v"(flag_next) : "v"(flag_addr0 + (unsigned)((r_n + 1) % 3) * 4u) : "memory");
+        __builtin_amdgcn_sched_barrier(0);
+        CA_WRES_ROW0(5, 5) CA_WRES_ELEM(5) CA_WRES_ROW0(6, 4) CA_WRES_ELEM(6) CA_WRES_ROW0(7, 3) CA_WRES_ELEM(7)
+        CA_WRES_ROW0(8, 2)
+        fa1[0] = pack2<DT>(f1[0], f1[1]);
+        fa1[1] = pack2<DT>(f1[2], f1[3]);
+        __builtin_amdgcn_sched_barrier(0);
+        CA_WRES_ROW0(9, 1)
+        fa1[2] = pack2<DT>(f1[4], f1[5]);
+        fa1[3] = pack2<DT>(f1[6], f1[7]);
+        __builtin_amdgcn_sched_barrier(0);
+#undef CA_WRES_ROW0
+#undef CA_WRES_ELEM
+#pragma unroll
+        for (int j = 0; j < TN; ++j) acc[1][j] = Elem<DT>::mfma(fb[j], fa1, acc[1][j]);
+        __builtin_amdgcn_sched_barrier(0);
+      } else {
       CA_WRES_PAIR(0, 9)
-      if (p.ln_inline) {
+      if (!GN && p.ln_inline) {
 #pragma unroll
         for (int q = 0; q < 4; ++q) {
           const float a0 = Elem<DT>::to_f((u16)(fa0[q] & 0xffffu)), a1 = Elem<DT>::to_f((u16)(fa0[q] >> 16));
@@ -174,18 +239,19 @@
         }
       }
       CA_WRES_PAIR(1, 8) CA_WRES_PAIR(2, 7) CA_WRES_PAIR(3, 6) CA_WRES_PAIR(4, 5)
-      unsigned flag_next;
       asm volatile("ds_read_b32 %0, %1" : "=v"(flag_next) : "v"(flag_addr0 + (unsigned)((r_n + 1) % 3) * 4u) : "memory");
       __builtin_amdgcn_sched_barrier(0);
       CA_WRES_PAIR(5, 5) CA_WRES_PAIR(6, 4) CA_WRES_PAIR(7, 3) CA_WRES_PAIR(8, 2) CA_WRES_PAIR(9, 1)
+      }
 #undef CA_WRES_PAIR
       asm volatile("s_waitcnt lgkmcnt(0)" : "+v"(flag_next)::"memory");
       r_s = r_s == 2 ? 0 : r_s + 1;
       ++r_n;
       chunk_wait(r_n, flag_next);
-    }
-
-    if (p.ln_inline) {
+      if (GN) gn_coeffs(kq == KQ - 1 ? rb_patch + r_i * 256 : mom, kq == KQ - 1 ? 0 : kq + 1);
+    }
+
+    if (!GN && p.ln_inline) {
 #pragma unroll
       for (int i = 0; i < 2; ++i) {
         float a = ln_s[i], b = ln_ss[i];
@@ -215,7 +281,7 @@
           rr[i][q] = __builtin_bit_cast(u32x4, __builtin_amdgcn_raw_buffer_load_b128(rs_res, off, q * 64, 0));
         }
     }
-    if (p.alpha == 1.f && p.post == 1.f && p.act == CA_ACT_NONE && !p.geglu) {
+    if (GN || (p.alpha == 1.f && p.post == 1.f && p.act == CA_ACT_NONE && !geglu)) {
       unsigned off[2];
 #pragma unroll
       for (int i = 0; i < 2; ++i) {
@@ -230,8 +296,8 @@
           const int col = 32 * q + 8 * g + 4 * u;
           bb[u] = *reinterpret_cast<const f32x4*>(smem + OFF_PAR + col * 4);
           cs[u] = (f32x4){0.f, 0.f, 0.f, 0.f};
-          if (p.ln_colsum) cs[u] = *reinterpret_cast<const f32x4*>(smem + OFF_PAR + (PN + col) * 4);
-          if (p.rowbias) {
+          if (ln_fold) cs[u] = *reinterpret_cast<const f32x4*>(smem + OFF_PAR + (PN + col) * 4);
+          if (!GN && p.rowbias) {
             const f32x4 rb = *reinterpret_cast<const f32x4*>(rb_patch + col * 4);
 #pragma unroll
             for (int r = 0; r < 4; ++r) bb[u][r] += rb[r];
@@ -243,7 +309,7 @@
 #pragma unroll
           for (int u = 0; u < 2; ++u) {
             f32x4 v = acc[i][2 * q + u];
-            if (p.ln_colsum) {
+            if (ln_fold) {
 #pragma unroll
               for (int r = 0; r < 4; ++r) v[r] = st[i].y * (v[r] - st[i].x * cs[u][r]);
             }
@@ -268,7 +334,8 @@
       }
       continue;
     }
-    if (p.geglu && !p.rowbias && !p.res && p.alpha == 1.f && p.post == 1.f && p.act == CA_ACT_NONE) {
+    if (GN) continue;
+    if (geglu && !p.rowbias && !p.res && p.alpha == 1.f && p.post == 1.f && p.act == CA_ACT_NONE) {
       unsigned off[2];
 #pragma unroll
       for (int i = 0; i < 2; ++i) {
@@ -279,11 +346,11 @@
       for (int j = 0; j < TN; ++j) {
         const f32x4 bi = *reinterpret_cast<const f32x4*>(smem + OFF_PAR + (j * 16 + g * 4) * 4);
         f32x4 cs = {0.f, 0.f, 0.f, 0.f};
-        if (p.ln_colsum) cs = *reinterpret_cast<const f32x4*>(smem + OFF_PAR + (PN + j * 16 + g * 4) * 4);
+        if (ln_fold) cs = *reinterpret_cast<const f32x4*>(smem + OFF_PAR + (PN + j * 16 + g * 4) * 4);
 #pragma unroll
         for (int i = 0; i < 2; ++i) {
           f32x4 v = acc[i][j];
-          if (p.ln_colsum) {
+          if (ln_fold) {
 #pragma unroll
             for (int r = 0; r < 4; ++r) v[r] = st[i].y * (v[r] - st[i].x * cs[r]);
           }
@@ -301,15 +368,15 @@
       const int nl = ca_wres_col(j, 4 * g, geglu);
       const f32x4 bi = *reinterpret_cast<const f32x4*>(smem + OFF_PAR + nl * 4);
       f32x4 cs = {0.f, 0.f, 0.f, 0.f}, rb = {0.f, 0.f, 0.f, 0.f};
-      if (p.ln_colsum) cs = *reinterpret_cast<const f32x4*>(smem + OFF_PAR + (PN + nl) * 4);
-      if (p.rowbias) rb = *reinterpret_cast<const f32x4*>(rb_patch + nl * 4);
+      if (ln_fold) cs = *reinterpret_cast<const f32x4*>(smem + OFF_PAR + (PN + nl) * 4);
+      if (!GN && p.rowbias) rb = *reinterpret_cast<const f32x4*>(rb_patch + nl * 4);
 #pragma unroll
       for (int i = 0; i < 2; ++i) {
         const int m = m0 + i * 16 + l15;
         float v[4];
 #pragma unroll
         for (int r = 0; r < 4; ++r) v[r] = acc[i][j][r];
-        if (p.ln_colsum) {
+        if (ln_fold) {
 #pragma unroll
           for (int r = 0; r < 4; ++r) v[r] = st[i].y * (v[r] - st[i].x * cs[r]);
         }
@@ -328,7 +395,7 @@
 #pragma unroll
           for (int r = 0; r < 4; ++r) v[r] = act_f(v[r], p.act);
         }
-        if (p.geglu) {
+        if (geglu) {
           const f32x2 gg = gelu_erf_f2((f32x2){v[1], v[3]});
           const unsigned w = pack2<DT>(v[0] * gg[0], v[2] * gg[1]);
           const unsigned off = m < p.m ? ((unsigned)m * (unsigned)p.ldc + (unsigned)((n0 >> 1) + (nl >> 1))) * 2u : 0x80000000u;
@@ -346,3 +413,13 @@
   }
   asm volatile("s_waitcnt vmcnt(0)" ::: "memory");
 }
+
+template <int DT>
+__global__ __launch_bounds__(512, 1) void k_gemm_wres(GemmKParams p, int panels, int lanes, int chunks, unsigned rb_bytes, unsigned c_bytes, unsigned res_bytes) {
+  gemm_wres_body<DT, false>(p, panels, lanes, chunks, rb_bytes, c_bytes, res_bytes);
+}
+
+template <int DT>
+__global__ __launch_bounds__(512, 1) void k_gemm_wres_gn(GemmKParams p, int panels, int lanes, int chunks, unsigned rb_bytes, unsigned c_bytes, unsigned res_bytes) {
+  gemm_wres_body<DT, true>(p, panels, lanes, chunks, rb_bytes, c_bytes, res_bytes);
+}
diff --git a/controlanimate_amd/csrc/ca_norm.hip b/controlanimate_amd/csrc/ca_norm.hip
--- a/controlanimate_amd/csrc/ca_norm.hip
+++ b/controlanimate_amd/csrc/ca_norm.hip
@@ -286,6 +286,120 @@
           st16(p.y + rows2[h] * C + (c8 << 3), pack8<DT>(f));
         }
       }
+  }
+}
+
+template <int DT, int txlog, int SLOTS>
+__global__ __launch_bounds__(256) void k_gn_stats_pair(GnParams p) {
+  __shared__ float part[4][GN_MAX_C / 8][4];
+  const int C = p.c1, C8 = C >> 3;
+  constexpr int TX = 1 << txlog, TY = 256 >> txlog;
+  const int tx = threadIdx.x & (TX - 1), ty = threadIdx.x >> txlog;
+  const int lane = threadIdx.x & 63, wave = threadIdx.x >> 6;
+  const int chunk = blockIdx.x, sg = blockIdx.y;
+  const int64_t base_row = (int64_t)sg * p.rows_per_stat;
+  const int cpg = C / p.groups;
+  float v[SLOTS][4];
+  int n0[SLOTS];
+#pragma unroll
+  for (int k = 0; k < SLOTS; ++k) {
+    const int c8 = tx + (k << txlog);
+    n0[k] = ((c8 << 3) / cpg + 1) * cpg - (c8 << 3);
+    v[k][0] = v[k][1] = v[k][2] = v[k][3] = 0.f;
+  }
+  for (int64_t piece = chunk;; piece += 2 * (int64_t)gridDim.x) {
+    const int64_t ra = piece * TY + ty, rb = (piece + gridDim.x) * TY + ty;
+    if (piece * TY >= p.rows_per_stat) break;
+    const bool ok[2] = {ra < p.rows_per_stat, rb < p.rows_per_stat};
+    const int64_t rows2[2] = {base_row + ra, base_row + rb};
+    u32x4 raw[2][SLOTS];
+#pragma unroll
+    for (int h = 0; h < 2; ++h)
+#pragma unroll
+      for (int k = 0; k < SLOTS; ++k) {
+        const int c8 = tx + (k << txlog);
+        if (c8 < C8 && ok[h]) raw[h][k] = ld16(p.x + rows2[h] * C + (c8 << 3));
+      }
+#pragma unroll
+    for (int h = 0; h < 2; ++h)
+#pragma unroll
+      for (int k = 0; k < SLOTS; ++k) {
+        if (tx + (k << txlog) < C8 && ok[h]) {
+          float f[8];
+          unpack8<DT>(raw[h][k], f);
+#pragma unroll
+          for (int j = 0; j < 8; ++j) {
+            const float lo = j < n0[k] ? f[j] : 0.f, hi = j < n0[k] ? 0.f : f[j];
+            v[k][0] += lo;
+            v[k][1] = fmaf(lo, lo, v[k][1]);
+            v[k][2] += hi;
+            v[k][3] = fmaf(hi, hi, v[k][3]);
+          }
+        }
+      }
+  }
+#pragma unroll
+  for (int k = 0; k < SLOTS; ++k) {
+    const int c8 = tx + (k << txlog);
+    if ((k << txlog) < C8) {
+#pragma unroll
+      for (int q = 0; q < 4; ++q)
+#pragma unroll
+        for (int off = TX; off < 64; off <<= 1) v[k][q] += __shfl_xor(v[k][q], off);
+      if (lane < TX && c8 < C8) {
+#pragma unroll
+        for (int q = 0; q < 4; ++q) part[wave][c8][q] = v[k][q];
+      }
+    }
+  }
+  __syncthreads();
+  if (threadIdx.x < p.groups) {
+    const int g = threadIdx.x;
+    float a = 0.f, b = 0.f;
+    for (int c8 = (g * cpg) >> 3; c8 <= ((g + 1) * cpg - 1) >> 3; ++c8) {
+      const int q = (c8 << 3) / cpg == g ? 0 : 2;
+      for (int w = 0; w < 4; ++w) {
+        a += part[w][c8][q];
+        b += part[w][c8][q + 1];
+      }
+    }
+    float* out = p.partials + (((int64_t)sg * p.nchunks + chunk) * p.groups + g) * 2;
+    out[0] = a;
+    out[1] = b;
+  }
+}
+
+__global__ __launch_bounds__(256) void k_gn_moments(GnParams p, float* moments) {
+  __shared__ double red[8][64][2];
+  const int sg = blockIdx.x;
+  const int cpg = (p.c1 + p.c2) / p.groups;
+  const int S = p.groups <= 32 ? 8 : 4;
+  const int g = threadIdx.x % (256 / S), slot = threadIdx.x / (256 / S);
+  if (g < p.groups) {
+    double a = 0.0, b = 0.0;
+    const float* part = p.partials + ((int64_t)sg * p.nchunks * p.groups + g) * 2;
+    for (int k = slot; k < p.nchunks; k += S) {
+      const float2 v = *reinterpret_cast<const float2*>(part + (int64_t)k * p.groups * 2);
+      a += (double)v.x;
+      b += (double)v.y;
+    }
+    red[slot][g][0] = a;
+    red[slot][g][1] = b;
+  }
+  __syncthreads();
+  if (threadIdx.x < p.groups) {
+    double a = 0.0, b = 0.0;
+    for (int q = 0; q < S; ++q) {
+      a += red[q][threadIdx.x][0];
+      b += red[q][threadIdx.x][1];
+    }
+    const double cnt = (double)p.rows_per_stat * (double)cpg;
+    const double mean = a / cnt;
+    double var = b / cnt - mean * mean;
+    if (var < 0.0) var = 0.0;
+    float* out = moments + ((int64_t)sg * p.groups + threadIdx.x) * 2;
+    out[0] = (float)mean;
+    out[1] = (float)(1.0 / sqrt(var + (double)p.eps));
   }
 }
 
@@ -904,6 +1018,34 @@
   if (a->dtype == CA_BF16) launch_gn<CA_BF16>(true, p, grid, (hipStream_t)stream);
   else launch_gn<CA_F16>(true, p, grid, (hipStream_t)stream);
   CA_CHECK_LAUNCH("ca_groupnorm_apply");
+  return CA_OK;
+}
+
+inline int gn_moments_chunks(int64_t rows) { return gn_chunks_rows(rows, 128); }
+
+extern "C" int64_t ca_groupnorm_moments_partials_floats(int32_t images, int32_t hw, int32_t groups) {
+  if (images <= 0 || hw <= 0 || groups <= 0) return 0;
+  return (int64_t)images * gn_moments_chunks(hw) * groups * 2;
+}
+
+extern "C" int ca_groupnorm_moments(const ca_groupnorm_args* a, float* moments, void* stream) {
+  GnParams p{};
+  int rc = gn_fill(a, p, "ca_groupnorm_moments");
+  if (rc) return rc;
+  CA_REQUIRE(moments != nullptr, "ca_groupnorm_moments: null moments");
+  CA_REQUIRE(a->frames_per_stat == 1 && a->c2 == 0 && !a->x2, "ca_groupnorm_moments: per-image statistics of one source only");
+  p.nchunks = gn_moments_chunks(p.rows_per_stat);
+  p.rows_per_chunk = (p.rows_per_stat + p.nchunks - 1) / p.nchunks;
+  dim3 grid(p.nchunks, a->images);
+  const int c8 = p.c1 >> 3, txlog = gn_txlog(c8), slots = (c8 + (1 << txlog) - 1) >> txlog;
+  hipStream_t st = (hipStream_t)stream;
+  if (p.c1 / p.groups >= 8 && txlog == 3 && slots == 5) {
+    if (a->dtype == CA_BF16) hipLaunchKernelGGL((k_gn_stats_pair<CA_BF16, 3, 5>), grid, dim3(256), 0, st, p);
+    else hipLaunchKernelGGL((k_gn_stats_pair<CA_F16, 3, 5>), grid, dim3(256), 0, st, p);
+  } else if (a->dtype == CA_BF16) launch_gn<CA_BF16>(false, p, grid, st);
+  else launch_gn<CA_F16>(false, p, grid, st);
+  hipLaunchKernelGGL(k_gn_moments, dim3(a->images), dim3(256), 0, (hipStream_t)stream, p, moments);
+  CA_CHECK_LAUNCH("ca_groupnorm_moments");
   return CA_OK;
 }
 
diff --git a/controlanimate_amd/kernels.py b/controlanimate_amd/kernels.py
--- a/controlanimate_amd/kernels.py
+++ b/controlanimate_amd/kernels.py
@@ -7,7 +7,7 @@
 
 from . import _capi
 from .context import dispatch
-from ._capi import (AttnArgs, ConvArgs, ConvNarrowArgs, FfArgs, PerceiverAttnArgs, TattnArgs, XattnArgs, GemmArgs, GroupNormArgs, LayerNormArgs, CA_ACT_NONE,
+from ._capi import (AttnArgs, ConvArgs, ConvNarrowArgs, FfArgs, PerceiverAttnArgs, TattnArgs, XattnArgs, GemmArgs, GemmGnArgs, GroupNormArgs, LayerNormArgs, CA_ACT_NONE,
                     CA_ACT_SILU, CA_BF16, CA_F16, check, lib)
 
 ACT_NONE, ACT_SILU = CA_ACT_NONE, CA_ACT_SILU
@@ -51,7 +51,7 @@
          bias: Optional[torch.Tensor] = None, rowbias: Optional[torch.Tensor] = None,
          rows_per_group: int = 0, residual: Optional[torch.Tensor] = None, alpha: float = 1.0,
          post_scale: float = 1.0, act: int = ACT_NONE, geglu: bool = False, out_f32: bool = False,
-         out: Optional[torch.Tensor] = None, ln=None, row_sums: bool = False) -> torch.Tensor:
+         out: Optional[torch.Tensor] = None, ln=None, row_sums: bool = False, gn=None) -> torch.Tensor:
     _req_cuda(a, w, a2, bias, rowbias, residual, out)
     assert a.dim() == 2 and a.stride(1) == 1 and w.dim() == 2 and w.is_contiguous()
     m, k1 = a.shape
@@ -119,8 +119,30 @@
         ws = torch.empty((wbytes,), device=a.device, dtype=torch.uint8)
         args.workspace, args.workspace_bytes = _p(ws), wbytes
     _record_plan(lib().ca_gemm_plan_name, args)
+    if gn is not None:
+        mom, gamma, beta, groups, rows_per_image = gn
+        _req_cuda(mom, gamma, beta)
+        assert ln is None and mom.dtype == gamma.dtype == beta.dtype == torch.float32 and gamma.numel() == beta.numel() == k1 + k2
+        assert mom.is_contiguous() and mom.shape == (m // rows_per_image, groups, 2)
+        gargs = GemmGnArgs(moments=_p(mom), gamma=_p(gamma), beta=_p(beta), groups=groups, rows_per_image=rows_per_image)
+        check(lib().ca_gemm_gn(C.byref(args), C.byref(gargs), _stream()), "ca_gemm_gn")
+        return out
     check(lib().ca_gemm(C.byref(args), _stream()), "ca_gemm")
     return out
+
+
+_gn_gemm_answers: dict = {}
+
+
+def gn_gemm_supported(m: int, n: int, k: int, groups: int, rows_per_image: int, dtype: torch.dtype) -> bool:
+    key = (m, n, k, groups, rows_per_image, dtype)
+    ans = _gn_gemm_answers.get(key)
+    if ans is None:
+        fake = 0x1000
+        args = GemmArgs(a=fake, w=fake, c=fake, bias=fake, lda=k, ldc=n, m=m, n=n, k1=k, k2=0, alpha=1.0, post_scale=1.0, dtype=dt_code(dtype))
+        gargs = GemmGnArgs(moments=fake, gamma=fake, beta=fake, groups=groups, rows_per_image=rows_per_image)
+        ans = _gn_gemm_answers[key] = bool(lib().ca_gemm_gn_inline_supported(C.byref(args), C.byref(gargs)))
+    return ans
 
 
 def attach_w_frag(w: torch.Tensor, geglu: bool = False) -> torch.Tensor:
@@ -408,6 +430,19 @@
     return y
 
 
+def group_norm_moments(x: torch.Tensor, *, groups: int = 32, eps: float = 1e-5) -> torch.Tensor:
+    _req_cuda(x)
+    assert x.dim() == 4 and x.is_contiguous()
+    images, h, w_, c = x.shape
+    nfl = lib().ca_groupnorm_moments_partials_floats(images, h * w_, groups)
+    partials = torch.empty((max(int(nfl), 1),), device=x.device, dtype=torch.float32)
+    mom = torch.empty((images, groups, 2), device=x.device, dtype=torch.float32)
+    args = GroupNormArgs(x=_p(x), partials=_p(partials), images=images, hw=h * w_, c1=c, c2=0, groups=groups, frames_per_stat=1, eps=eps,
+                         act=ACT_NONE, dtype=dt_code(x.dtype))
+    check(lib().ca_groupnorm_moments(C.byref(args), _p(mom), _stream()), "ca_groupnorm_moments")
+    return mom
+
+
 def layer_norm(x: torch.Tensor, gamma: torch.Tensor, beta: torch.Tensor, *, pos: Optional[torch.Tensor] = None,
                rows_per_frame: int = 1, frames: int = 1, eps: float = 1e-5) -> torch.Tensor:
     _req_cuda(x, gamma, beta, pos)
diff --git a/controlanimate_amd/layers.py b/controlanimate_amd/layers.py
--- a/controlanimate_amd/layers.py
+++ b/controlanimate_amd/layers.py
@@ -226,6 +226,16 @@
                             eps=self.eps, act=act)
 
 
+def group_norm_proj(norm: HipGroupNorm, proj, x: torch.Tensor, **kw) -> torch.Tensor:
+    from .context import dispatch
+    images, h, w, c = x.shape
+    rows = images * h * w
+    if dispatch.gn_proj_in and K.gn_gemm_supported(rows, proj.w.t.shape[0], c, norm.num_groups, h * w, x.dtype):
+        mom = K.group_norm_moments(x, groups=norm.num_groups, eps=norm.eps)
+        return proj.run(x.view(rows, c), gn=(mom, norm.g.t, norm.b.t, norm.num_groups, h * w), **kw)
+    return proj.run(norm.run(x).view(rows, c), **kw)
+
+
 class HipLayerNorm(nn.Module):
     def __init__(self, dim: int, eps: float = 1e-5):
         super().__init__()
diff --git a/controlanimate_amd/motion_module.py b/controlanimate_amd/motion_module.py
--- a/controlanimate_amd/motion_module.py
+++ b/controlanimate_amd/motion_module.py
@@ -9,7 +9,7 @@
 from .attention import FeedForward
 from .attention_processor import Attention
 from .context import ExecCtx
-from .layers import HipGroupNorm, HipLayerNorm, HipLinear, WeightArena, _f32
+from .layers import HipGroupNorm, HipLayerNorm, HipLinear, WeightArena, _f32, group_norm_proj
 
 
 def get_motion_module(in_channels, motion_module_type: str, motion_module_kwargs: dict):
@@ -140,8 +140,7 @@
     def forward(self, x: torch.Tensor, ctx: ExecCtx) -> torch.Tensor:
         images, h, w, c = x.shape
         rows = images * h * w
-        y = self.norm.run(x)
-        y = self.proj_in.run(y.view(rows, c), row_sums=self.transformer_blocks[0].attention_blocks[0].fold is not None)
+        y = group_norm_proj(self.norm, self.proj_in, x, row_sums=self.transformer_blocks[0].attention_blocks[0].fold is not None)
         pfrag = getattr(self, "proj_out_frag", None)
         last = len(self.transformer_blocks) - 1
         for k, blk in enumerate(self.transformer_blocks):
diff --git a/include/controlanimate_hip.h b/include/controlanimate_hip.h
--- a/include/controlanimate_hip.h
+++ b/include/controlanimate_hip.h
@@ -126,6 +126,15 @@
 int64_t ca_gemm_workspace_bytes(const ca_gemm_args* args);
 int ca_gemm_row_sums_parts(const ca_gemm_args* args);
 int ca_gemm_ln_inline_supported(const ca_gemm_args* args);
+typedef struct ca_gemm_gn_args {
+  const float* moments;
+  const float* gamma;
+  const float* beta;
+  int32_t groups;
+  int32_t rows_per_image;
+} ca_gemm_gn_args;
+int ca_gemm_gn_inline_supported(const ca_gemm_args* args, const ca_gemm_gn_args* gn);
+int ca_gemm_gn(const ca_gemm_args* args, const ca_gemm_gn_args* gn, void* stream);
 int ca_gemm_wants_finished_stats(const ca_gemm_args* args);
 int ca_ln_finish_sums(const float* sums, int parts, int64_t rows, int k, float eps, float* mean_rstd, void* stream);
 int ca_gemm_plan_name(const ca_gemm_args* args, char* buf, int32_t len);
@@ -182,6 +191,8 @@
 int ca_groupnorm_stats(const ca_groupnorm_args* args, void* stream);
 int ca_groupnorm_apply(const ca_groupnorm_args* args, void* stream);
 int ca_groupnorm(const ca_groupnorm_args* args, void* stream);
+int64_t ca_groupnorm_moments_partials_floats(int32_t images, int32_t hw, int32_t groups);
+int ca_groupnorm_moments(const ca_groupnorm_args* args, float* moments, void* stream);
 
 typedef struct ca_layernorm_args {
   const void* x; void* y;
```
